# mpkuse/cerebro

Measured on AMD Instinct MI355X. Metric: loop-queries/sec (ticks of 3 descriptors vs 4096-D x 1M DB), higher is better.
Workload: dtype f64

## Files before the change

cerebro_amd/capi.py:

```python
from __future__ import annotations

import ctypes as C
import os
import sys
from pathlib import Path

import numpy as np

_HERE = Path(__file__).resolve().parent
PRODUCT_LIB_PATH = _HERE / "lib" / "libcerebro_hip.so"
HOOKS_LIB_PATH = _HERE / "lib" / "hooks" / "libcerebro_hip.so"


def _lib_path() -> Path:
    override = os.environ.get("CHIP_LIB")
    if override:
        if os.environ.get("CHIP_ALLOW_LIB_OVERRIDE") == "1":
            return Path(override).resolve()
        sys.stderr.write(f"[cerebro_amd] CHIP_LIB={override} IGNORED: set CHIP_ALLOW_LIB_OVERRIDE=1 to load another build of the library\n")
    return PRODUCT_LIB_PATH


LIB_PATH = _lib_path()

CHIP_OK = 0
CHIP_ERR_INVALID_ARG = -1
CHIP_ERR_NO_DEVICE = -2
CHIP_ERR_HIP = -3
CHIP_ERR_OOM = -4
CHIP_ERR_NOT_F32 = -5
CHIP_ERR_NONFINITE = -6
CHIP_ERR_RANGE = -7
CHIP_ERR_UNSUPPORTED = -8
CHIP_ERR_TOO_FEW_POINTS = -9
CHIP_ERR_BUSY = -10
CHIP_ERR_COMM = -11
CHIP_ERR_SHARD_FAILED = -12
CHIP_ERR_GROUP_BROKEN = -13

CHIP_MAX_TOPK = 16
CHIP_MAX_NQ = 4
CHIP_DEFAULT_TOPK = 8
CHIP_RING_ROWS = 4096
CHIP_MAX_INFLIGHT = 64
CHIP_APPEND_ALLOW_ROUNDING = 1
CHIP_CREATE_STORE_F32 = 1
CHIP_CREATE_STORE_F64 = 2
CHIP_MULTI_EXCHANGE_COPY = 4
CHIP_COMM_ID_BYTES = 128
CHIP_EXCHANGE_NONE, CHIP_EXCHANGE_RCCL, CHIP_EXCHANGE_COPY = 0, 1, 2
CHIP_SCAN_FORM_ONE_ROW, CHIP_SCAN_FORM_ROWS = 1, 2
CHIP_SAMPLER_FRESH, CHIP_SAMPLER_THEIA_PERSISTENT = 0, 1
CHIP_RANSAC_LEG_PNP, CHIP_RANSAC_LEG_ICP = 0, 1
CHIP_SCAN_FAMILY_NONE, CHIP_SCAN_FAMILY_ONE_ROW, CHIP_SCAN_FAMILY_WIDE, CHIP_SCAN_FAMILY_ROWS, CHIP_SCAN_FAMILY_MULTI = 0, 1, 2, 3, 4
CHIP_SCAN_CALL_QUERY, CHIP_SCAN_CALL_TICK, CHIP_SCAN_CALL_TICK_SYNC = 0, 1, 2
SCAN_FAMILY_NAMES = {0: "none", 1: "one_row", 2: "wide", 3: "rows", 4: "multi", 5: "prefilter", 6: "halfq"}

CHIP_TICK_SKIPPED, CHIP_TICK_TOO_SHORT, CHIP_TICK_SCANNED = 0, 1, 2
CHIP_MATCH_MAX_KEYPOINTS = 16384
CHIP_MATCH_MAX_BATCH = 16
CHIP_MATCH_MAX_PAIRS = CHIP_MATCH_MAX_BATCH
CHIP_ICP_MAX_BATCH = 16
CHIP_ORB_DESC_BYTES = 32
CHIP_SET_AB, CHIP_SET_BA = 0, 1
CHIP_DISP_S16, CHIP_DISP_F32 = 0, 1
CHIP_STEREO_BM_NUM_DISPARITIES, CHIP_STEREO_BM_BLOCK_SIZE, CHIP_STEREO_BM_PREFILTER_CAP = 64, 21, 31
CHIP_STEREO_BM_TEXTURE_THRESHOLD, CHIP_STEREO_BM_UNIQUENESS_RATIO = 10, 15
CHIP_ORB_MAX_LEVELS, CHIP_ORB_MAX_SIDE = 8, 4096
CHIP_ORB_BINS = 32
CHIP_ORB_N_FEATURES, CHIP_ORB_N_LEVELS, CHIP_ORB_FAST_THRESHOLD, CHIP_ORB_BORDER = 5000, 8, 0, 31
CHIP_RECTIFY_FRACTION_BITS, CHIP_RECTIFY_MAP_MIN, CHIP_RECTIFY_MAP_MAX, CHIP_RECTIFY_NAN_Q = 5, -2.0, 32768.0, -64
CHIP_PROJ_F32, CHIP_PROJ_F64, CHIP_PROJ_MAX_IN_DIM = 1, 2, 32768
CHIP_VLAD_NHWC, CHIP_VLAD_NCHW, CHIP_VLAD_BLOCK, CHIP_VLAD_MAX_POSITIONS = 1, 2, 64, 16384


class ChipError(RuntimeError):
    def __init__(self, status: int, where: str, detail: str = ""):
        self.status = status
        super().__init__(f"{where}: status {status} ({_strerror(status)}){' -- ' + detail if detail else ''}")


class DotParams(C.Structure):
    _fields_ = [("locality", C.c_int32), ("lag", C.c_int32), ("min_new", C.c_int32), ("min_k", C.c_int32),
                ("thresh", C.c_double)]


class TickResult(C.Structure):
    _fields_ = [("status", C.c_int32), ("found", C.c_int32), ("idx_curr", C.c_int64), ("idx_prev", C.c_int64),
                ("score", C.c_double), ("argmax", C.c_int64 * 3), ("maxv", C.c_double * 3)]

    def as_dict(self):
        return dict(status=self.status, found=self.found, idx_curr=self.idx_curr, idx_prev=self.idx_prev,
                    score=self.score, argmax=list(self.argmax), maxv=list(self.maxv))


class TopkEntry(C.Structure):
    _fields_ = [("score", C.c_double), ("idx", C.c_int64)]


class RansacParams(C.Structure):
    _fields_ = [("error_thresh", C.c_double), ("min_inlier_ratio", C.c_double), ("max_iterations", C.c_int32),
                ("min_iterations", C.c_int32), ("use_mle", C.c_int32), ("sample_size", C.c_int32),
                ("failure_probability", C.c_double), ("seed", C.c_uint64), ("n_hypotheses", C.c_int32),
                ("sampler", C.c_int32)]


class RansacSummary(C.Structure):
    _fields_ = [("n_iterations", C.c_int32), ("n_inliers", C.c_int32), ("best_hypothesis", C.c_int32),
                ("n_models", C.c_int32), ("best_cost", C.c_double)]


class StereoBmParams(C.Structure):
    _fields_ = [("num_disparities", C.c_int32), ("block_size", C.c_int32), ("prefilter_cap", C.c_int32),
                ("texture_threshold", C.c_int32), ("uniqueness_ratio", C.c_int32)]


class OrbParams(C.Structure):
    _fields_ = [("n_features", C.c_int32), ("n_levels", C.c_int32), ("fast_threshold", C.c_int32), ("border", C.c_int32)]


class OrbKeypoint(C.Structure):
    _fields_ = [("response", C.c_int64), ("x", C.c_float), ("y", C.c_float), ("m10", C.c_int32), ("m01", C.c_int32),
                ("x_level", C.c_uint16), ("y_level", C.c_uint16), ("level", C.c_uint16), ("zero", C.c_uint16)]


class OrbLevel(C.Structure):
    _fields_ = [("width", C.c_int32), ("height", C.c_int32), ("quota", C.c_int32), ("x0", C.c_int32), ("y0", C.c_int32),
                ("x1", C.c_int32), ("y1", C.c_int32), ("scale", C.c_double)]

    def as_dict(self):
        return {k: getattr(self, k) for k, _ in self._fields_}


ORB_KEYPOINT_DTYPE = np.dtype([("response", "<i8"), ("x", "<f4"), ("y", "<f4"), ("m10", "<i4"), ("m01", "<i4"), ("x_level", "<u2"),
                               ("y_level", "<u2"), ("level", "<u2"), ("zero", "<u2")])


class MatchFrame(C.Structure):
    _fields_ = [("desc", C.c_void_p), ("kp_xy", C.c_void_p), ("n", C.c_int32), ("width", C.c_int32), ("height", C.c_int32),
                ("xyz", C.c_void_p)]


class MatchSummary(C.Structure):
    _fields_ = [("n_matches_all", C.c_int32), ("n_matches_gms", C.c_int32), ("n_3d2d_ab", C.c_int32), ("n_3d2d_ba", C.c_int32),
                ("n_3d3d", C.c_int32), ("n_out_of_image", C.c_int32)]

    def as_dict(self):
        return {k: getattr(self, k) for k, _ in self._fields_}


CHIP_GMS_WITH_SCALE, CHIP_GMS_WITH_ROTATION = 1, 2


class GmsChoice(C.Structure):
    _fields_ = [("scale", C.c_int32), ("rotation", C.c_int32), ("n_inliers", C.c_int32), ("counts", (C.c_int32 * 8) * 5)]

    def as_dict(self):
        return dict(scale=self.scale, rotation=self.rotation, n_inliers=self.n_inliers,
                    counts=np.array([list(row) for row in self.counts], dtype=np.int32))


class MatchSetsOut(C.Structure):
    _fields_ = [(k, C.c_void_p) for k in ("uv", "uv_d", "X_ab", "uvn_ab", "X_ba", "uvn_ba", "A_3d3d", "B_3d3d",
                                          "match_query_idx", "match_train_idx")]


class ScanLaunch(C.Structure):
    _fields_ = [(n, C.c_int32) for n in ("family", "elem", "nq", "K", "U", "NT", "FULL", "NG", "R", "NTL", "ticks", "q64", "claimed", "fused",
                                         "grid", "block", "wg_per_cu", "lds_bytes")] + [("n_rows", C.c_int64), ("launches", C.c_int64)]

    def as_dict(self):
        d = {k: int(getattr(self, k)) for k, _ in self._fields_}
        d["family"] = SCAN_FAMILY_NAMES[d["family"]]
        return d


class PassInfo(C.Structure):
    _fields_ = [(n, C.c_int32) for n in ("family", "ticks", "grid", "wpb", "K", "e")] + [("k", C.c_int64 * 5), ("E", C.c_double)]


class RansacShape(C.Structure):
    _fields_ = [(n, C.c_int32) for n in ("P", "H", "N", "words", "S", "sampler")]


class Info(C.Structure):
    _fields_ = [("abi_version", C.c_int32), ("D", C.c_int32), ("device", C.c_int32), ("shard_rank", C.c_int32),
                ("shard_count", C.c_int32), ("n_cus", C.c_int32), ("rows_global", C.c_int64),
                ("rows_local", C.c_int64), ("capacity_local", C.c_int64), ("lossy_rows", C.c_int64),
                ("arch", C.c_char * 32), ("storage_bytes", C.c_int32), ("n_devices", C.c_int32), ("exchange", C.c_int32),
                ("comm_ranks", C.c_int32), ("comm_init_abandoned", C.c_int32), ("scan_forms", C.c_int32), ("test_hooks", C.c_int32),
                ("row_norm_max", C.c_double)]


_P = C.c_void_p
_SIGS = {
    "chip_strerror": (C.c_char_p, [C.c_int]),
    "chip_abi_version": (C.c_int, []),
    "chip_build_scan_forms": (C.c_int, []),
    "chip_build_test_hooks": (C.c_int, []),
    "chip_last_hip_error": (C.c_int, [_P, C.POINTER(C.c_char_p)]),
    "chip_last_comm_error": (C.c_int, [_P, C.POINTER(C.c_char_p)]),
    "chip_create": (C.c_int, [C.POINTER(_P), C.c_int32, C.c_int64, C.c_int32, C.c_int32, C.c_int32]),
    "chip_create_ex": (C.c_int, [C.POINTER(_P), C.c_int32, C.c_int64, C.c_int32, C.c_int32, C.c_int32, C.c_uint32]),
    "chip_create_multi": (C.c_int, [C.POINTER(_P), C.c_int32, C.c_int64, _P, C.c_int32, C.c_uint32]),
    "chip_comm_unique_id": (C.c_int, [_P]),
    "chip_comm_init_rank": (C.c_int, [_P, _P, C.c_int32, C.c_int32]),
    "chip_destroy": (None, [_P]),
    "chip_set_stream": (C.c_int, [_P, _P]),
    "chip_reset_stream": (C.c_int, [_P]),
    "chip_synchronize": (C.c_int, [_P]),
    "chip_db_append_f64": (C.c_int, [_P, _P, C.c_int64, C.c_uint32, C.POINTER(C.c_int64)]),
    "chip_db_append_f32": (C.c_int, [_P, _P, C.c_int64, C.POINTER(C.c_int64)]),
    "chip_db_size": (C.c_int64, [_P]),
    "chip_db_read_rows_f32": (C.c_int, [_P, _P, C.c_int64, _P]),
    "chip_db_read_rows_f64": (C.c_int, [_P, _P, C.c_int64, _P]),
    "chip_db_append_synthetic": (C.c_int, [_P, C.c_int64, C.c_uint64, _P, _P, _P, C.c_int64]),
    "chip_db_append_synthetic_unit": (C.c_int, [_P, C.c_int64, C.c_uint64, _P, _P, _P, C.c_int64]),
    "chip_query_rows": (C.c_int, [_P, C.c_int64, _P, C.c_int32, C.c_int32, _P, _P]),
    "chip_query_vectors_f32": (C.c_int, [_P, C.c_int64, _P, C.c_int32, C.c_int32, _P, _P]),
    "chip_query_vectors_f64": (C.c_int, [_P, C.c_int64, _P, C.c_int32, C.c_int32, _P, _P]),
    "chip_query_scores": (C.c_int, [_P, C.c_int64, C.c_int64, _P]),
    "chip_query_batch_f32": (C.c_int, [_P, C.c_int64, _P, C.c_int32, C.c_int32, _P, _P]),
    "chip_query_batch_cast_f32": (C.c_int, [_P, C.c_int64, _P, C.c_int32, C.c_int32, _P, _P]),
    "chip_build_has_query_prefix": (C.c_int, []),
    "chip_query_batch_rows_f32": (C.c_int, [_P, _P, _P, C.c_int32, C.c_int32, _P, _P]),
    "chip_query_batch_rows_cast_f32": (C.c_int, [_P, _P, _P, C.c_int32, C.c_int32, _P, _P]),
    "chip_query_batch_prefix_f32": (C.c_int, [_P, _P, _P, C.c_int32, C.c_int32, _P, _P]),
    "chip_query_batch_prefix_cast_f32": (C.c_int, [_P, _P, _P, C.c_int32, C.c_int32, _P, _P]),
    "chip_query_prefix_plan": (C.c_int, [_P, C.c_int32, C.c_int32, C.c_int32, _P, _P]),
    "chip_debug_query_prefix_last": (C.c_int, [_P, _P]),
    "chip_build_has_bulk_ticks": (C.c_int, []),
    "chip_loop_ticks_bulk": (C.c_int, [_P, _P, C.c_int32, _P, C.c_int64, C.c_int32, _P, _P, _P, _P]),
    "chip_bulk_ticks_plan": (C.c_int, [_P, C.c_int32, _P, C.c_int64, C.c_int64, _P, _P, _P]),
    "chip_debug_bulk_ticks_last": (C.c_int, [_P, _P]),
    "chip_dot_params_default": (None, [C.POINTER(DotParams)]),
    "chip_loop_tick": (C.c_int, [_P, C.c_int64, C.POINTER(DotParams), C.POINTER(TickResult)]),
    "chip_resident_pause": (C.c_int, [_P]),
    "chip_resident_resume": (C.c_int, [_P]),
    "chip_loop_tick_enqueue": (C.c_int, [_P, C.c_int64, C.POINTER(DotParams), C.c_int32]),
    "chip_loop_tick_collect": (C.c_int, [_P, C.c_int32, C.POINTER(TickResult)]),
    "chip_loop_last_l": (C.c_int64, [_P]),
    "chip_loop_reset": (None, [_P]),
    "chip_scan_local": (C.c_int, [_P, C.c_int64, C.POINTER(DotParams), C.c_int32, _P, C.POINTER(C.c_int32)]),
    "chip_merge_decide": (C.c_int, [_P, C.c_int64, C.POINTER(DotParams), _P, C.c_int32, C.c_int32, C.POINTER(TickResult)]),
    "chip_merge_decide_enqueue": (C.c_int, [_P, C.c_int64, C.POINTER(DotParams), _P, C.c_int32, C.c_int32, C.c_int32]),
    "chip_debug_merge_lists": (C.c_int, [_P, C.c_int32, _P, C.c_int32, C.c_int32, C.c_int32, _P, C.c_int64, C.POINTER(DotParams),
                                         C.POINTER(TickResult)]),
    "chip_debug_last_pass": (C.c_int, [_P, C.POINTER(PassInfo), _P, _P, _P]),
    "chip_ransac_params_default": (None, [C.POINTER(RansacParams)]),
    "chip_pnp_ransac": (C.c_int, [_P, _P, _P, C.c_int32, C.POINTER(RansacParams), _P, C.POINTER(C.c_float), _P,
                                  C.POINTER(RansacSummary)]),
    "chip_pnp_ransac_batch": (C.c_int, [_P, C.c_int32, _P, _P, _P, C.POINTER(RansacParams), _P, _P, _P, _P, _P]),
    "chip_icp_params_default": (None, [C.POINTER(RansacParams)]),
    "chip_icp_ransac": (C.c_int, [_P, _P, _P, C.c_int32, C.POINTER(RansacParams), _P, C.POINTER(C.c_float), _P,
                                  C.POINTER(RansacSummary)]),
    "chip_icp_ransac_enqueue": (C.c_int, [_P, _P, _P, C.c_int32, C.POINTER(RansacParams)]),
    "chip_icp_ransac_collect": (C.c_int, [_P, _P, C.POINTER(C.c_float), _P, C.POINTER(RansacSummary)]),
    "chip_build_has_icp_batch": (C.c_int, []),
    "chip_icp_ransac_batch": (C.c_int, [_P, C.c_int32, _P, _P, _P, C.POINTER(RansacParams), _P, _P, _P, _P, _P]),
    "chip_debug_ransac_record": (C.c_int, [_P, C.c_int32, C.c_int32, C.POINTER(RansacShape), _P, _P, _P, _P, _P, _P, _P]),
    "chip_debug_pnp_stage": (C.c_int, [_P, C.c_int32, _P, _P, _P]),
    "chip_debug_pnp_keep_stage": (C.c_int, [_P, C.c_int32]),
    "chip_build_has_match": (C.c_int, []),
    "chip_build_has_tick_coalesce": (C.c_int, []),
    "chip_debug_coalesce_stats": (C.c_int, [_P, C.POINTER(C.c_int64), C.POINTER(C.c_int64)]),
    "chip_debug_coalesce_force": (C.c_int, [_P, C.c_int32]),
    "chip_debug_coalesce_decide": (C.c_int, [C.c_int32, C.c_int32, C.c_int32]),
    "chip_debug_last_scan": (C.c_int, [_P, C.POINTER(ScanLaunch)]),
    "chip_debug_scan_plan": (C.c_int, [C.c_int32, C.c_int32, C.c_int32, C.c_int32, C.c_int64, C.c_int32, C.c_int32, C.POINTER(ScanLaunch)]),
    "chip_debug_multi_plan": (C.c_int, [C.c_int32, C.c_int32, C.c_int32, C.c_int32, C.c_int32, C.POINTER(ScanLaunch)]),
    "chip_debug_prefilter_plan": (C.c_int, [C.c_int32, C.c_int32, C.c_int32, C.c_int32, C.POINTER(ScanLaunch)]),
    "chip_debug_halfq_plan": (C.c_int, [C.c_int32, C.c_int32, C.c_int32, C.c_int32, C.POINTER(ScanLaunch)]),
    "chip_debug_halfq_bound": (C.c_int, [C.c_int32, C.c_double, C.POINTER(C.c_int32), C.POINTER(C.c_double)]),
    "chip_debug_prefilter_stats": (C.c_int, [_P, C.POINTER(C.c_int64), C.POINTER(C.c_int64), C.POINTER(C.c_int64)]),
    "chip_orb_match": (C.c_int, [_P, _P, C.c_int32, _P, C.c_int32, _P, _P]),
    "chip_gms_filter": (C.c_int, [_P, _P, C.c_int32, C.c_int32, C.c_int32, _P, C.c_int32, C.c_int32, C.c_int32, _P, _P, C.c_int32, _P,
                                  C.POINTER(C.c_int32)]),
    "chip_match_pair": (C.c_int, [_P, C.POINTER(MatchFrame), C.POINTER(MatchFrame), _P, C.POINTER(MatchSummary)]),
    "chip_match_read_sets": (C.c_int, [_P, C.POINTER(MatchSetsOut)]),
    "chip_pnp_ransac_matched": (C.c_int, [_P, C.c_int32, C.POINTER(RansacParams), _P, C.POINTER(C.c_float), _P, C.POINTER(RansacSummary)]),
    "chip_icp_ransac_matched": (C.c_int, [_P, C.POINTER(RansacParams), _P, C.POINTER(C.c_float), _P, C.POINTER(RansacSummary)]),
    "chip_build_has_gms_modes": (C.c_int, []),
    "chip_gms_filter_modes": (C.c_int, [_P, _P, C.c_int32, C.c_int32, C.c_int32, _P, C.c_int32, C.c_int32, C.c_int32, _P, _P, C.c_int32,
                                        C.c_uint32, _P, C.POINTER(C.c_int32), C.POINTER(GmsChoice)]),
    "chip_match_batch_modes": (C.c_int, [_P, C.POINTER(MatchFrame), C.POINTER(MatchFrame), C.c_int32, _P, C.c_uint32, C.POINTER(MatchSummary),
                                         C.POINTER(GmsChoice)]),
    "chip_match_batch_stored_modes": (C.c_int, [_P, C.c_int64, _P, C.c_int32, _P, C.c_uint32, C.POINTER(MatchSummary), C.POINTER(GmsChoice)]),
    "chip_build_has_match_batch": (C.c_int, []),
    "chip_match_batch": (C.c_int, [_P, C.POINTER(MatchFrame), C.POINTER(MatchFrame), C.c_int32, _P, C.POINTER(MatchSummary)]),
    "chip_match_select": (C.c_int, [_P, C.c_int32]),
    "chip_match_batch_read_matches": (C.c_int, [_P, C.c_int32, _P, _P]),
    "chip_pnp_ransac_matched_batch": (C.c_int, [_P, C.c_int32, _P, _P, C.POINTER(RansacParams), _P, _P, _P, _P, _P, _P]),
    "chip_icp_ransac_matched_batch_enqueue": (C.c_int, [_P, C.c_int32, _P, C.POINTER(RansacParams), _P, _P]),
    "chip_icp_ransac_matched_batch_collect": (C.c_int, [_P, _P, _P, _P, _P]),
    "chip_icp_ransac_matched_batch": (C.c_int, [_P, C.c_int32, _P, C.POINTER(RansacParams), _P, _P, _P, _P, _P, _P]),
    "chip_build_has_frame_store": (C.c_int, []),
    "chip_frame_store_reserve": (C.c_int, [_P, C.c_int32, C.c_int32]),
    "chip_frame_store_info": (C.c_int, [_P, C.POINTER(C.c_int32), C.POINTER(C.c_int32), C.POINTER(C.c_int32)]),
    "chip_frame_put": (C.c_int, [_P, C.c_int64, C.POINTER(MatchFrame)]),
    "chip_frame_drop": (C.c_int, [_P, C.c_int64]),
    "chip_frame_read": (C.c_int, [_P, C.c_int64, C.POINTER(C.c_int32), C.POINTER(C.c_int32), C.POINTER(C.c_int32), _P, _P, _P]),
    "chip_match_batch_stored": (C.c_int, [_P, C.c_int64, _P, C.c_int32, _P, C.POINTER(MatchSummary)]),
    "chip_build_has_match_pairs": (C.c_int, []),
    "chip_match_pairs_stored": (C.c_int, [_P, _P, _P, C.c_int32, _P, C.c_uint32, C.POINTER(MatchSummary), C.POINTER(GmsChoice)]),
    "chip_build_has_disparity": (C.c_int, []),
    "chip_frame_put_disparity": (C.c_int, [_P, C.c_int64, _P, _P, C.c_int32, C.c_int32, C.c_int32, _P, C.c_int32, _P]),
    "chip_disparity_to_xyz": (C.c_int, [_P, _P, C.c_int32, C.c_int32, C.c_int32, _P, _P]),
    "chip_stereo_bm_params_default": (None, [C.POINTER(StereoBmParams)]),
    "chip_build_has_stereo_bm": (C.c_int, []),
    "chip_stereo_bm": (C.c_int, [_P, _P, _P, C.c_int32, C.c_int32, C.POINTER(StereoBmParams), _P]),
    "chip_frame_put_stereo": (C.c_int, [_P, C.c_int64, _P, _P, C.c_int32, C.c_int32, C.c_int32, _P, _P, C.POINTER(StereoBmParams), _P]),
    "chip_orb_params_default": (None, [C.POINTER(OrbParams)]),
    "chip_build_has_orb_detect": (C.c_int, []),
    "chip_orb_plan": (C.c_int, [C.c_int32, C.c_int32, C.POINTER(OrbParams), C.POINTER(OrbLevel)]),
    "chip_orb_detect": (C.c_int, [_P, _P, C.c_int32, C.c_int32, C.POINTER(OrbParams), _P, C.c_int32, C.POINTER(C.c_int32), C.POINTER(C.c_int32)]),
    "chip_debug_orb_level": (C.c_int, [_P, C.c_int32, _P, _P]),
    "chip_build_has_orb_describe": (C.c_int, []),
    "chip_orb_bin": (C.c_int, [C.c_int32, C.c_int32]),
    "chip_orb_pattern": (C.c_int, [_P, _P]),
    "chip_orb_detect_describe": (C.c_int, [_P, _P, C.c_int32, C.c_int32, C.POINTER(OrbParams), _P, C.c_int32, C.POINTER(C.c_int32), C.POINTER(C.c_int32),
                                           _P]),
    "chip_debug_orb_blur": (C.c_int, [_P, C.c_int32, _P]),
    "chip_frame_put_orb_stereo": (C.c_int, [_P, C.c_int64, C.c_int32, C.c_int32, _P, _P, C.POINTER(OrbParams), C.POINTER(StereoBmParams), _P,
                                            C.POINTER(C.c_int32)]),
    "chip_build_has_rectify": (C.c_int, []),
    "chip_rectify_quantize": (C.c_int, [_P, C.c_int64, _P]),
    "chip_remap": (C.c_int, [_P, _P, C.c_int32, C.c_int32, _P, _P, _P]),
    "chip_rectify_set_maps": (C.c_int, [_P, C.c_int32, C.c_int32, _P, _P, _P, _P, _P, _P, _P, _P]),
    "chip_rectify_pair": (C.c_int, [_P, _P, _P, C.c_int32, C.c_int32, _P, _P]),
    "chip_frame_put_raw_orb_stereo": (C.c_int, [_P, C.c_int64, C.c_int32, C.c_int32, _P, _P, C.POINTER(OrbParams), C.POINTER(StereoBmParams), _P,
                                                C.POINTER(C.c_int32)]),
    "chip_build_has_frame_put_batch": (C.c_int, []),
    "chip_frame_put_plan": (C.c_int, [C.c_int32, C.c_int32, C.POINTER(OrbParams), C.c_int32, C.c_int32, C.POINTER(C.c_int32), C.POINTER(C.c_int32)]),
    "chip_frame_put_orb_stereo_batch": (C.c_int, [_P, _P, C.c_int32, C.c_int32, C.c_int32, _P, _P, C.POINTER(OrbParams), C.POINTER(StereoBmParams), _P,
                                                  _P]),
    "chip_frame_put_raw_orb_stereo_batch": (C.c_int, [_P, _P, C.c_int32, C.c_int32, C.c_int32, _P, _P, C.POINTER(OrbParams),
                                                      C.POINTER(StereoBmParams), _P, _P]),
    "chip_frame_put_records": (C.c_int, [_P, C.c_int64, _P, _P, _P, C.c_int32, C.c_int32, C.c_int32]),
    "chip_debug_frame_put_last": (C.c_int, [_P, C.POINTER(C.c_int32), C.POINTER(C.c_int32), C.POINTER(C.c_int32)]),
    "chip_build_has_project": (C.c_int, []),
    "chip_project_set": (C.c_int, [_P, C.c_int32, _P, C.c_int32, _P]),
    "chip_project_clear": (C.c_int, [_P]),
    "chip_project_info": (C.c_int, [_P, C.POINTER(C.c_int32), C.POINTER(C.c_int32), C.POINTER(C.c_int32)]),
    "chip_project": (C.c_int, [_P, _P, C.c_int64, _P]),
    "chip_db_append_projected_f32": (C.c_int, [_P, _P, C.c_int64, C.c_uint32, C.POINTER(C.c_int64)]),
    "chip_build_has_vlad": (C.c_int, []),
    "chip_vlad_set": (C.c_int, [_P, C.c_int32, C.c_int32, C.c_int32, _P, _P, _P]),
    "chip_vlad_clear": (C.c_int, [_P]),
    "chip_vlad_info": (C.c_int, [_P, C.POINTER(C.c_int32), C.POINTER(C.c_int32), C.POINTER(C.c_int32)]),
    "chip_vlad": (C.c_int, [_P, _P, C.c_int32, C.c_int32, _P]),
    "chip_db_append_vlad_f32": (C.c_int, [_P, _P, C.c_int32, C.c_int32, C.c_uint32, C.POINTER(C.c_int64)]),
    "chip_debug_vlad_stage": (C.c_int, [_P, _P, _P, _P]),
    "chip_project_plan": (C.c_int, [C.c_int32, C.c_int32, C.c_int64, _P]),
    "chip_debug_project_last": (C.c_int, [_P, C.POINTER(C.c_int64), C.POINTER(C.c_int64), C.POINTER(C.c_int32)]),
    "chip_vlad_batch": (C.c_int, [_P, _P, C.c_int32, C.c_int32, C.c_int32, _P]),
    "chip_db_append_vlad_batch_f32": (C.c_int, [_P, _P, C.c_int32, C.c_int32, C.c_int32, C.c_uint32, C.POINTER(C.c_int64)]),
    "chip_get_info": (C.c_int, [_P, C.POINTER(Info)]),
    "chip_profile_enable": (C.c_int, [_P, C.c_int32]),
    "chip_profile_reset": (C.c_int, [_P]),
    "chip_profile_scan": (C.c_int, [_P, C.POINTER(C.c_double), C.POINTER(C.c_int64), C.POINTER(C.c_double), C.POINTER(C.c_double)]),
}

_lib = None


def load_library(path: os.PathLike | None = None) -> C.CDLL:
    global _lib
    if _lib is not None and path is None:
        return _lib
    p = Path(path) if path else LIB_PATH
    if p.exists() and "torch" not in sys.modules:
        try:
            import torch
        except Exception:
            pass
    if not p.exists():
        raise FileNotFoundError(
            f"{p} not found: the HIP extension is not built. Run `make lib` (or __graft_entry__.build()). "
            "cerebro_amd has no CPU fallback.")
    lib = C.CDLL(str(p))
    for name, (res, args) in _SIGS.items():
        fn = getattr(lib, name)
        fn.restype = res
        fn.argtypes = args
    if path is None:
        _lib = lib
    return lib


class use_hooks_library:

    def __enter__(self):
        global _lib
        self.saved = _lib
        lib = load_library(HOOKS_LIB_PATH)
        if lib.chip_build_test_hooks() != 1:
            raise RuntimeError(f"{HOOKS_LIB_PATH} is not a -DCHIP_TEST_HOOKS build")
        _lib = lib
        return lib

    def __exit__(self, *exc):
        global _lib
        _lib = self.saved
        return False


def declared_symbols():
    return sorted(_SIGS)


def _strerror(status: int) -> str:
    try:
        return load_library().chip_strerror(status).decode()
    except Exception:
        return "?"


def _ptr(a: np.ndarray):
    return a.ctypes.data_as(C.c_void_p)

# ... 39 lines not shown
        raise ChipError(rc, "chip_orb_pattern")
    return pattern, steered


def rectify_quantize(map) -> np.ndarray:
    m = np.ascontiguousarray(map, dtype=np.float32)
    q = np.zeros(m.shape, dtype=np.int32)
    rc = load_library().chip_rectify_quantize(_ptr(m), m.size, _ptr(q))
    if rc != CHIP_OK:
        raise ChipError(rc, "chip_rectify_quantize")
    return q


def frame_put_plan(width: int, height: int, F: int, params=None, raw: bool = False) -> dict:
    _, o = _orb_params(params)
    g, n = C.c_int32(), C.c_int32()
    rc = load_library().chip_frame_put_plan(width, height, o, int(raw), F, C.byref(g), C.byref(n))
    if rc != CHIP_OK:
        raise ChipError(rc, "chip_frame_put_plan")
    return dict(group=g.value, n_groups=n.value)


def orb_plan(width: int, height: int, params=None) -> list:
    params, p = _orb_params(params)
    lv = (OrbLevel * CHIP_ORB_MAX_LEVELS)()
    rc = load_library().chip_orb_plan(width, height, p, lv)
    if rc != CHIP_OK:
        raise ChipError(rc, "chip_orb_plan")
    n = CHIP_ORB_N_LEVELS if params is None else params.n_levels
    return [lv[l].as_dict() for l in range(n)]


class ProjectPlan(C.Structure):
    _fields_ = [("width", C.c_int32), ("slab", C.c_int32), ("lds_bytes", C.c_int32), ("single_lds_bytes", C.c_int32), ("block", C.c_int32),
                ("reserved", C.c_int32), ("passes", C.c_int64), ("shared_passes", C.c_int64), ("single_launches", C.c_int64)]


def project_plan(in_dim: int, matrix_type: int, n: int) -> dict:
    out = ProjectPlan()
    rc = load_library().chip_project_plan(in_dim, matrix_type, n, C.byref(out))
    if rc != CHIP_OK:
        raise ChipError(rc, "chip_project_plan")
    return {name: getattr(out, name) for name, _ in ProjectPlan._fields_ if name != "reserved"}


CHIP_QUERY_PREFIX_GROUP = 4096


class QueryPrefixPlan(C.Structure):
    _fields_ = [("group_size", C.c_int32), ("groups", C.c_int32), ("tile_full", C.c_int32), ("tile_last", C.c_int32),
                ("qtiles", C.c_int64), ("units", C.c_int64), ("units_rect", C.c_int64)]


class QueryPrefixLast(C.Structure):
    _fields_ = [("groups", C.c_int32), ("launches", C.c_int32), ("waits", C.c_int32), ("reserved", C.c_int32),
                ("units_claimed", C.c_int64), ("units_planned", C.c_int64)]


def query_prefix_plan(k, elem: int = 4, topk: int = 5) -> dict:
    k = np.ascontiguousarray(k, dtype=np.int64).reshape(-1)
    order = np.empty(k.shape[0], dtype=np.int32)
    out = QueryPrefixPlan()
    rc = load_library().chip_query_prefix_plan(_ptr(k), k.shape[0], elem, topk, _ptr(order), C.byref(out))
    if rc != CHIP_OK:
        raise ChipError(rc, "chip_query_prefix_plan")
    d = {name: getattr(out, name) for name, _ in QueryPrefixPlan._fields_}
    d["order"] = order
    return d


CHIP_BULK_TICKS_GROUP, CHIP_BULK_TICKS_MAX_TOPK = 1365, 8


class BulkTicksPlan(C.Structure):
    _fields_ = [("group_ticks", C.c_int32), ("groups", C.c_int32), ("tile_full", C.c_int32), ("tile_last", C.c_int32),
                ("ticks_scanned", C.c_int64), ("ticks_skipped", C.c_int64), ("ticks_too_short", C.c_int64),
                ("units", C.c_int64), ("units_rect", C.c_int64), ("last_l", C.c_int64)]


class BulkTicksLast(C.Structure):
    _fields_ = [("groups", C.c_int32), ("launches", C.c_int32), ("waits", C.c_int32), ("list_len", C.c_int32),
                ("certified", C.c_int64), ("uncertified", C.c_int64), ("rescored_rows", C.c_int64),
                ("exact_reruns", C.c_int64), ("E", C.c_double)]


def bulk_ticks_plan(ls, n_rows: int, params: DotParams | None = None, last_l: int = 0) -> dict:
    ls = np.ascontiguousarray(ls, dtype=np.int64).reshape(-1)
    T = ls.shape[0]
    status = np.empty(T, dtype=np.int32)
    k = np.empty(T, dtype=np.int64)
    out = BulkTicksPlan()
    rc = load_library().chip_bulk_ticks_plan(_ptr(ls) if T else None, T, C.byref(params) if params is not None else None, last_l, n_rows,
                                             _ptr(status), _ptr(k), C.byref(out))
    if rc != CHIP_OK:
        raise ChipError(rc, "chip_bulk_ticks_plan")
    d = {name: getattr(out, name) for name, _ in BulkTicksPlan._fields_}
    d["status"] = status
    d["k"] = k
    return d


def default_ransac_params() -> RansacParams:
    p = RansacParams()
    load_library().chip_ransac_params_default(C.byref(p))
    return p


def default_icp_params() -> RansacParams:
    p = RansacParams()
    load_library().chip_icp_params_default(C.byref(p))
    return p


def scan_plan(D: int, elem: int, nq: int, K: int, n_rows: int, call: int = CHIP_SCAN_CALL_QUERY, n_cus: int = 256, check: bool = True):
    out = ScanLaunch()
    rc = load_library().chip_debug_scan_plan(D, elem, nq, K, n_rows, call, n_cus, C.byref(out))
    if not check:
        return rc, out.as_dict()
    if rc != CHIP_OK:
        raise ChipError(rc, "chip_debug_scan_plan")
    return out.as_dict()


def multi_plan(D: int, elem: int, n_ticks: int, K: int = CHIP_DEFAULT_TOPK, n_cus: int = 256, check: bool = True):
    out = ScanLaunch()
    rc = load_library().chip_debug_multi_plan(D, elem, n_ticks, K, n_cus, C.byref(out))
    if not check:
        return rc, out.as_dict()
    if rc != CHIP_OK:
        raise ChipError(rc, "chip_debug_multi_plan")
    return out.as_dict()


def prefilter_plan(D: int, elem: int = 4, K: int = CHIP_DEFAULT_TOPK, n_cus: int = 256, check: bool = True):
    out = ScanLaunch()
    rc = load_library().chip_debug_prefilter_plan(D, elem, K, n_cus, C.byref(out))
    if not check:
        return rc, out.as_dict()
    if rc != CHIP_OK:
        raise ChipError(rc, "chip_debug_prefilter_plan")
    return out.as_dict()


def halfq_plan(D: int, elem: int = 4, K: int = CHIP_DEFAULT_TOPK, n_cus: int = 256, check: bool = True):
    out = ScanLaunch()
    rc = load_library().chip_debug_halfq_plan(D, elem, K, n_cus, C.byref(out))
    if not check:
        return rc, out.as_dict()
    if rc != CHIP_OK:
        raise ChipError(rc, "chip_debug_halfq_plan")
    return out.as_dict()


def halfq_bound(D: int, row_norm_max: float) -> tuple[int, float]:
    e, E = C.c_int32(), C.c_double()
    rc = load_library().chip_debug_halfq_bound(D, row_norm_max, C.byref(e), C.byref(E))
    if rc != CHIP_OK:
        raise ChipError(rc, "chip_debug_halfq_bound")
    return e.value, E.value


def comm_unique_id() -> bytes:
    buf = C.create_string_buffer(CHIP_COMM_ID_BYTES)
    st = load_library().chip_comm_unique_id(buf)
    if st != CHIP_OK:
        raise ChipError(st, "chip_comm_unique_id")
    return buf.raw


class Chip:

    def __init__(self, D: int, capacity_hint: int = 0, device: int = 0, shard_rank: int = 0, shard_count: int = 1,
                 storage: str | None = None, devices=None, copy_exchange: bool = False):
        self.lib = load_library()
        self.D = int(D)
        self.shard_rank, self.shard_count = shard_rank, shard_count
        flags = {None: 0, "f32": CHIP_CREATE_STORE_F32, "f64": CHIP_CREATE_STORE_F64}[storage]
        h = C.c_void_p()
        if devices is not None:
            dev = np.ascontiguousarray(devices, dtype=np.int32)
            st = self.lib.chip_create_multi(C.byref(h), D, capacity_hint, _ptr(dev), dev.size,
                                            flags | (CHIP_MULTI_EXCHANGE_COPY if copy_exchange else 0))
            where = "chip_create_multi"
        elif flags:
            st = self.lib.chip_create_ex(C.byref(h), D, capacity_hint, device, shard_rank, shard_count, flags)
            where = "chip_create_ex"
        else:
            st = self.lib.chip_create(C.byref(h), D, capacity_hint, device, shard_rank, shard_count)
            where = "chip_create"
        if st != CHIP_OK:
            raise ChipError(st, where)
        self.h = h

    def comm_init_rank(self, unique_id: bytes, n_ranks: int, rank: int):
        assert len(unique_id) == CHIP_COMM_ID_BYTES
        self._chk(self.lib.chip_comm_init_rank(self.h, C.c_char_p(unique_id), n_ranks, rank), "chip_comm_init_rank")

    def close(self):
        if getattr(self, "h", None):
            self.lib.chip_destroy(self.h)
            self.h = None

    def __del__(self):
        try:
            self.close()
        except Exception:
            pass

    def __enter__(self):
        return self

    def __exit__(self, *a):
        self.close()

    def _chk(self, st: int, where: str):
        if st != CHIP_OK:
            txt = C.c_char_p()
            if st == CHIP_ERR_COMM:
                r = self.lib.chip_last_comm_error(self.h, C.byref(txt))
                raise ChipError(st, where, f"ncclResult {r}: {txt.value.decode() if txt.value else ''}")
            hip = self.lib.chip_last_hip_error(self.h, C.byref(txt)) if st in (CHIP_ERR_HIP, CHIP_ERR_OOM) else 0
            raise ChipError(st, where, f"hipError {hip}: {txt.value.decode() if txt.value else ''}" if hip else "")

    def last_comm_error(self) -> str:
        txt = C.c_char_p()
        r = self.lib.chip_last_comm_error(self.h, C.byref(txt))
        return f"{r}: {txt.value.decode() if txt.value else ''}"

    def set_stream(self, stream_ptr: int | None):
        if stream_ptr is None:
            self._chk(self.lib.chip_reset_stream(self.h), "chip_reset_stream")
        else:
            self._chk(self.lib.chip_set_stream(self.h, C.c_void_p(stream_ptr)), "chip_set_stream")

    def synchronize(self):
        self._chk(self.lib.chip_synchronize(self.h), "chip_synchronize")

    def append_f64(self, desc: np.ndarray, allow_rounding: bool = False) -> int:
        desc = np.ascontiguousarray(desc, dtype=np.float64).reshape(-1, self.D)
        first = C.c_int64()
        self._chk(self.lib.chip_db_append_f64(self.h, _ptr(desc), desc.shape[0],
                                              CHIP_APPEND_ALLOW_ROUNDING if allow_rounding else 0, C.byref(first)),
                  "chip_db_append_f64")
        return first.value

    def append_f32(self, desc: np.ndarray) -> int:
        desc = np.ascontiguousarray(desc, dtype=np.float32).reshape(-1, self.D)
        first = C.c_int64()
        self._chk(self.lib.chip_db_append_f32(self.h, _ptr(desc), desc.shape[0], C.byref(first)), "chip_db_append_f32")
        return first.value

    def project_set(self, Mt: np.ndarray, bias=None):
        Mt = np.asarray(Mt)
        if Mt.dtype not in (np.float32, np.float64) or Mt.ndim != 2 or Mt.shape[0] != self.D:
            raise ValueError("project_set: Mt must be a (D, in_dim) float32 or float64 array")
        Mt = np.ascontiguousarray(Mt)
        b = None if bias is None else np.ascontiguousarray(bias, dtype=np.float64).reshape(self.D)
        self._chk(self.lib.chip_project_set(self.h, Mt.shape[1], _ptr(Mt), CHIP_PROJ_F32 if Mt.dtype == np.float32 else CHIP_PROJ_F64,
                                            None if b is None else _ptr(b)), "chip_project_set")

    def project_clear(self):
        self._chk(self.lib.chip_project_clear(self.h), "chip_project_clear")

    def project_info(self) -> dict:
        v = [C.c_int32(), C.c_int32(), C.c_int32()]
        self._chk(self.lib.chip_project_info(self.h, *(C.byref(x) for x in v)), "chip_project_info")
        return dict(in_dim=v[0].value, matrix_type=v[1].value, has_bias=bool(v[2].value))

    def _raw_descriptors(self, x, n):
        if isinstance(x, (int, np.integer)):
            if n is None:
                raise ValueError("a device address needs n")
            return C.c_void_p(int(x)), int(n), None
        in_dim = self.project_info()["in_dim"]
        a = np.ascontiguousarray(x, dtype=np.float32)
        a = a.reshape(-1, in_dim) if in_dim else a.reshape(1, -1)
        return _ptr(a), a.shape[0], a

    def project(self, x, n: int | None = None) -> np.ndarray:
        p, n, keep = self._raw_descriptors(x, n)
        z = np.empty((n, self.D), dtype=np.float64)
        self._chk(self.lib.chip_project(self.h, p, n, _ptr(z)), "chip_project")
        return z

    def append_projected(self, x, flags: int = 0, n: int | None = None) -> int:
        p, n, keep = self._raw_descriptors(x, n)
        first = C.c_int64()
        self._chk(self.lib.chip_db_append_projected_f32(self.h, p, n, flags, C.byref(first)), "chip_db_append_projected_f32")
        return first.value

    def debug_project_last(self) -> dict:
        passes, descs, width = (C.c_int64 * 2)(), (C.c_int64 * 2)(), C.c_int32()
        self._chk(self.lib.chip_debug_project_last(self.h, passes, descs, C.byref(width)), "chip_debug_project_last")
        return dict(shared_passes=passes[0], single_launches=passes[1], shared_descriptors=descs[0], single_descriptors=descs[1],
                    width=width.value)

    def vlad_set(self, Wt, bias, centres):
        Wt = np.ascontiguousarray(Wt, dtype=np.float32)
        centres = np.ascontiguousarray(centres, dtype=np.float32)
        bias = np.ascontiguousarray(bias, dtype=np.float32).reshape(-1)
        if Wt.ndim != 2 or centres.ndim != 2 or centres.shape[1] != Wt.shape[1] or bias.size != Wt.shape[0] or centres.shape[0] > Wt.shape[0]:
            raise ValueError("vlad_set: Wt (K+G, C), bias (K+G), centres (K, C)")
        K, G = centres.shape[0], Wt.shape[0] - centres.shape[0]
        self._chk(self.lib.chip_vlad_set(self.h, Wt.shape[1], K, G, _ptr(Wt), _ptr(bias), _ptr(centres)), "chip_vlad_set")

    def vlad_clear(self):
# ... 86 lines not shown
        return out

    def read_rows_f64(self, rows) -> np.ndarray:
        rows = np.ascontiguousarray(rows, dtype=np.int64)
        out = np.empty((rows.size, self.D), dtype=np.float64)
        self._chk(self.lib.chip_db_read_rows_f64(self.h, _ptr(rows), rows.size, _ptr(out)), "chip_db_read_rows_f64")
        return out

    def query_scores(self, k: int, row: int) -> np.ndarray:
        u = np.full(max(k, 1), np.nan, dtype=np.float64)
        self._chk(self.lib.chip_query_scores(self.h, k, row, _ptr(u)), "chip_query_scores")
        return u[:k]

    def query_vectors_f64(self, k: int, q: np.ndarray, topk: int = CHIP_DEFAULT_TOPK):
        q = np.ascontiguousarray(q, dtype=np.float64).reshape(-1, self.D)
        nq = q.shape[0]
        sc = np.empty((nq, topk), dtype=np.float64)
        ix = np.empty((nq, topk), dtype=np.int64)
        self._chk(self.lib.chip_query_vectors_f64(self.h, k, _ptr(q), nq, topk, _ptr(sc), _ptr(ix)), "chip_query_vectors_f64")
        return sc, ix

    def query_rows(self, k: int, rows, topk: int = CHIP_DEFAULT_TOPK):
        rows = np.ascontiguousarray(rows, dtype=np.int64)
        nq = rows.size
        sc = np.empty((nq, topk), dtype=np.float64)
        ix = np.empty((nq, topk), dtype=np.int64)
        self._chk(self.lib.chip_query_rows(self.h, k, _ptr(rows), nq, topk, _ptr(sc), _ptr(ix)), "chip_query_rows")
        return sc, ix

    def query_vectors(self, k: int, q: np.ndarray, topk: int = CHIP_DEFAULT_TOPK):
        q = np.ascontiguousarray(q, dtype=np.float32).reshape(-1, self.D)
        nq = q.shape[0]
        sc = np.empty((nq, topk), dtype=np.float64)
        ix = np.empty((nq, topk), dtype=np.int64)
        self._chk(self.lib.chip_query_vectors_f32(self.h, k, _ptr(q), nq, topk, _ptr(sc), _ptr(ix)),
                  "chip_query_vectors_f32")
        return sc, ix

    def query_batch(self, k: int, q: np.ndarray, topk: int = CHIP_DEFAULT_TOPK, cast_rows: bool = False):
        q = np.ascontiguousarray(q, dtype=np.float32).reshape(-1, self.D)
        Q = q.shape[0]
        sc = np.empty((Q, topk), dtype=np.float32)
        ix = np.empty((Q, topk), dtype=np.int64)
        name = "chip_query_batch_cast_f32" if cast_rows else "chip_query_batch_f32"
        self._chk(getattr(self.lib, name)(self.h, k, _ptr(q), Q, topk, _ptr(sc), _ptr(ix)), name)
        return sc, ix

    def query_batch_rows(self, rows, k, topk: int = CHIP_DEFAULT_TOPK, cast_rows: bool = False):
        rows = np.ascontiguousarray(rows, dtype=np.int64).reshape(-1)
        k = np.ascontiguousarray(k, dtype=np.int64).reshape(-1)
        if rows.shape != k.shape:
            raise ValueError("rows and k must have the same length")
        Q = rows.shape[0]
        sc = np.empty((Q, topk), dtype=np.float32)
        ix = np.empty((Q, topk), dtype=np.int64)
        name = "chip_query_batch_rows_cast_f32" if cast_rows else "chip_query_batch_rows_f32"
        self._chk(getattr(self.lib, name)(self.h, _ptr(rows), _ptr(k), Q, topk, _ptr(sc), _ptr(ix)), name)
        return sc, ix

    def query_batch_prefix(self, k, q: np.ndarray, topk: int = CHIP_DEFAULT_TOPK, cast_rows: bool = False):
        q = np.ascontiguousarray(q, dtype=np.float32).reshape(-1, self.D)
        k = np.ascontiguousarray(k, dtype=np.int64).reshape(-1)
        Q = q.shape[0]
        if k.shape[0] != Q:
            raise ValueError("k must have one entry per query")
        sc = np.empty((Q, topk), dtype=np.float32)
        ix = np.empty((Q, topk), dtype=np.int64)
        name = "chip_query_batch_prefix_cast_f32" if cast_rows else "chip_query_batch_prefix_f32"
        self._chk(getattr(self.lib, name)(self.h, _ptr(k), _ptr(q), Q, topk, _ptr(sc), _ptr(ix)), name)
        return sc, ix

    def self_join(self, first: int, count: int, lag: int, topk: int = CHIP_DEFAULT_TOPK, cast_rows: bool = False):
        rows = first + np.arange(count, dtype=np.int64)
        return self.query_batch_rows(rows, np.maximum(0, rows - lag), topk, cast_rows)

    def debug_query_prefix_last(self) -> dict:
        out = QueryPrefixLast()
        self._chk(self.lib.chip_debug_query_prefix_last(self.h, C.byref(out)), "chip_debug_query_prefix_last")
        return {name: getattr(out, name) for name, _ in QueryPrefixLast._fields_ if name != "reserved"}

    def loop_tick(self, l: int, params: DotParams | None = None) -> TickResult:
        p = params or default_dot_params()
        r = TickResult()
        self._chk(self.lib.chip_loop_tick(self.h, l, C.byref(p), C.byref(r)), "chip_loop_tick")
        return r

    def loop_ticks_bulk(self, ls, params: DotParams | None = None, last_l: int = 0, topk: int = 1):
        ls = np.ascontiguousarray(ls, dtype=np.int64).reshape(-1)
        T = ls.shape[0]
        recs = (TickResult * max(T, 1))()
        sc = np.empty((T, 3, topk), dtype=np.float64)
        ix = np.empty((T, 3, topk), dtype=np.int64)
        last = C.c_int64(last_l)
        self._chk(self.lib.chip_loop_ticks_bulk(self.h, _ptr(ls) if T else None, T, C.byref(params) if params is not None else None, last_l, topk,
                                                C.byref(recs), _ptr(sc), _ptr(ix), C.byref(last)), "chip_loop_ticks_bulk")
        return [recs[t] for t in range(T)], sc, ix, last.value

    def debug_bulk_ticks_last(self) -> dict:
        out = BulkTicksLast()
        self._chk(self.lib.chip_debug_bulk_ticks_last(self.h, C.byref(out)), "chip_debug_bulk_ticks_last")
        return {name: getattr(out, name) for name, _ in BulkTicksLast._fields_}

    def resident_pause(self):
        self._chk(self.lib.chip_resident_pause(self.h), "chip_resident_pause")

    def resident_resume(self):
        self._chk(self.lib.chip_resident_resume(self.h), "chip_resident_resume")

    def loop_tick_enqueue(self, l: int, slot: int, params: DotParams | None = None):
        p = params or default_dot_params()
        self._chk(self.lib.chip_loop_tick_enqueue(self.h, l, C.byref(p), slot), "chip_loop_tick_enqueue")

    def loop_tick_collect(self, slot: int) -> TickResult:
        r = TickResult()
        self._chk(self.lib.chip_loop_tick_collect(self.h, slot, C.byref(r)), "chip_loop_tick_collect")
        return r

    def loop_reset(self):
        self.lib.chip_loop_reset(self.h)

    def last_l(self) -> int:
        return int(self.lib.chip_loop_last_l(self.h))

    def coalesce_stats(self) -> tuple[int, int]:
        passes, ticks = C.c_int64(), C.c_int64()
        self._chk(self.lib.chip_debug_coalesce_stats(self.h, C.byref(passes), C.byref(ticks)), "chip_debug_coalesce_stats")
        return passes.value, ticks.value

    def prefilter_stats(self) -> tuple[int, int, int]:
        passes, ticks, unc = C.c_int64(), C.c_int64(), C.c_int64()
        self._chk(self.lib.chip_debug_prefilter_stats(self.h, C.byref(passes), C.byref(ticks), C.byref(unc)), "chip_debug_prefilter_stats")
        return passes.value, ticks.value, unc.value

    def coalesce_force(self, on: bool):
        self._chk(self.lib.chip_debug_coalesce_force(self.h, 1 if on else 0), "chip_debug_coalesce_force")

    def last_scan(self) -> dict:
        out = ScanLaunch()
        self._chk(self.lib.chip_debug_last_scan(self.h, C.byref(out)), "chip_debug_last_scan")
        return out.as_dict()

    def last_pass(self) -> dict:
        info = PassInfo()
        self._chk(self.lib.chip_debug_last_pass(self.h, C.byref(info), None, None, None), "chip_debug_last_pass")
        T, grid, K = info.ticks, info.grid, info.K
        cand = np.empty((T, grid, 3, K, 2), dtype=np.float64)
        exact = np.empty((T, 3, K, 2), dtype=np.float64)
        cert = np.zeros((T, 3), dtype=np.uint32)
        self._chk(self.lib.chip_debug_last_pass(self.h, C.byref(info), _ptr(cand), _ptr(exact), _ptr(cert)), "chip_debug_last_pass")
        return dict(family=SCAN_FAMILY_NAMES[info.family], ticks=T, grid=grid, wpb=int(info.wpb), K=K, k=[int(x) for x in info.k[:T]],
                    E=float(info.E), e=int(info.e), cand_s=cand[..., 0].copy(), cand_i=cand[..., 1].copy().view(np.int64),
                    exact_s=exact[..., 0].copy(), exact_i=exact[..., 1].copy().view(np.int64), cert=cert)

    def scan_local(self, l: int, dev_out_ptr: int, topk: int = CHIP_DEFAULT_TOPK, params: DotParams | None = None) -> int:
        p = params or default_dot_params()
        status = C.c_int32()
        self._chk(self.lib.chip_scan_local(self.h, l, C.byref(p), topk, C.c_void_p(dev_out_ptr), C.byref(status)),
                  "chip_scan_local")
        return status.value

    def merge_decide(self, l: int, dev_gathered_ptr: int, n_lists: int, topk: int = CHIP_DEFAULT_TOPK,
                     params: DotParams | None = None) -> TickResult:
        p = params or default_dot_params()
        r = TickResult()
        self._chk(self.lib.chip_merge_decide(self.h, l, C.byref(p), C.c_void_p(dev_gathered_ptr), n_lists, topk,
                                             C.byref(r)), "chip_merge_decide")
        return r

    def merge_decide_enqueue(self, l: int, dev_gathered_ptr: int, n_lists: int, slot: int, topk: int = CHIP_DEFAULT_TOPK,
                             params: DotParams | None = None):
        p = params or default_dot_params()
        self._chk(self.lib.chip_merge_decide_enqueue(self.h, l, C.byref(p), C.c_void_p(dev_gathered_ptr), n_lists, topk, slot),
                  "chip_merge_decide_enqueue")

    def debug_merge_lists(self, form: int, scores: np.ndarray, idx: np.ndarray, l: int = 0, params: DotParams | None = None,
                          record: bool = False):
        scores = np.ascontiguousarray(scores, dtype=np.float64)
        idx = np.ascontiguousarray(idx, dtype=np.int64)
        assert scores.ndim == 3 and scores.shape == idx.shape
        n_lists, nq, K = scores.shape
        lists = np.empty((n_lists, nq, K, 2), dtype=np.float64)
        lists[..., 0] = scores
        lists[..., 1] = idx.view(np.float64)
        out = np.empty((nq, K, 2), dtype=np.float64)
        r = TickResult() if record else None
        p = params or default_dot_params()
        self._chk(self.lib.chip_debug_merge_lists(self.h, form, _ptr(lists), n_lists, nq, K, _ptr(out), l, C.byref(p),
                                                  C.byref(r) if record else None), "chip_debug_merge_lists")
        return out[..., 0].copy(), out[..., 1].copy().view(np.int64), r

    def pnp_ransac(self, X: np.ndarray, uv: np.ndarray, params: RansacParams | None = None):
        X = np.ascontiguousarray(X, dtype=np.float64).reshape(-1, 3)
        uv = np.ascontiguousarray(uv, dtype=np.float64).reshape(-1, 2)
        N = X.shape[0]
        assert uv.shape[0] == N
        p = params or default_ransac_params()
        T = np.empty(16, dtype=np.float64)
        conf = C.c_float()
        mask = np.zeros(max(N, 1), dtype=np.uint8)
        summ = RansacSummary()
        st = self.lib.chip_pnp_ransac(self.h, _ptr(X), _ptr(uv), N, C.byref(p), _ptr(T), C.byref(conf), _ptr(mask),
                                      C.byref(summ))
        if st == CHIP_ERR_TOO_FEW_POINTS:
            return dict(status=st, confidence=-1.0, T=None, mask=None, summary=None)
        self._chk(st, "chip_pnp_ransac")
        return dict(status=st, confidence=float(conf.value), T=T.reshape(4, 4).T.copy(), mask=mask[:N].copy(),
                    summary=dict(n_iterations=summ.n_iterations, n_inliers=summ.n_inliers,
                                 best_hypothesis=summ.best_hypothesis, n_models=summ.n_models,
                                 best_cost=summ.best_cost))

    def pnp_ransac_batch(self, problems, params: RansacParams | None = None, seeds=None):
        P = len(problems)
        Xs = [np.ascontiguousarray(X, dtype=np.float64).reshape(-1, 3) for X, _ in problems]
        uvs = [np.ascontiguousarray(uv, dtype=np.float64).reshape(-1, 2) for _, uv in problems]
        Ns = np.array([x.shape[0] for x in Xs], dtype=np.int32)
        p = params or default_ransac_params()
        T = np.empty((P, 16), dtype=np.float64)
        conf = np.zeros(P, dtype=np.float32)
        masks = [np.zeros(max(int(n), 1), dtype=np.uint8) for n in Ns]
        summ = (RansacSummary * max(P, 1))()
        Xp = (C.c_void_p * max(P, 1))(*[x.ctypes.data for x in Xs])
        uvp = (C.c_void_p * max(P, 1))(*[u.ctypes.data for u in uvs])
        mp = (C.c_void_p * max(P, 1))(*[m.ctypes.data for m in masks])
        sd = None if seeds is None else np.asarray(seeds, dtype=np.uint64)
        st = self.lib.chip_pnp_ransac_batch(self.h, P, Xp, uvp, _ptr(Ns), C.byref(p), None if sd is None else _ptr(sd),
                                            _ptr(T), _ptr(conf), mp, summ)
        self._chk(st, "chip_pnp_ransac_batch")
        return [dict(status=st, confidence=float(conf[i]), T=T[i].reshape(4, 4).T.copy(), mask=masks[i][:Ns[i]].copy(),
                     summary=dict(n_iterations=summ[i].n_iterations, n_inliers=summ[i].n_inliers,
                                  best_hypothesis=summ[i].best_hypothesis, n_models=summ[i].n_models,
                                  best_cost=summ[i].best_cost)) for i in range(P)]

    def icp_ransac_enqueue(self, A: np.ndarray, B: np.ndarray, params: RansacParams | None = None):
        A = np.ascontiguousarray(A, dtype=np.float64).reshape(-1, 3)
        B = np.ascontiguousarray(B, dtype=np.float64).reshape(-1, 3)
        p = params or default_icp_params()
        self._chk(self.lib.chip_icp_ransac_enqueue(self.h, _ptr(A), _ptr(B), A.shape[0], C.byref(p)), "chip_icp_ransac_enqueue")
        return A.shape[0]

    def icp_ransac_collect(self, N: int):
        T = np.empty(16, dtype=np.float64)
        conf = C.c_float()
        mask = np.zeros(max(N, 1), dtype=np.uint8)
        summ = RansacSummary()
        self._chk(self.lib.chip_icp_ransac_collect(self.h, _ptr(T), C.byref(conf), _ptr(mask), C.byref(summ)), "chip_icp_ransac_collect")
        return dict(status=0, confidence=float(conf.value), T=T.reshape(4, 4).T.copy(), mask=mask[:N].copy(),
                    summary=dict(n_iterations=summ.n_iterations, n_inliers=summ.n_inliers, best_hypothesis=summ.best_hypothesis,
                                 n_models=summ.n_models, best_cost=summ.best_cost))

    def icp_ransac(self, A: np.ndarray, B: np.ndarray, params: RansacParams | None = None):
        A = np.ascontiguousarray(A, dtype=np.float64).reshape(-1, 3)
        B = np.ascontiguousarray(B, dtype=np.float64).reshape(-1, 3)
        N = A.shape[0]
        assert B.shape[0] == N
        p = params or default_icp_params()
        T = np.empty(16, dtype=np.float64)
        conf = C.c_float()
        mask = np.zeros(max(N, 1), dtype=np.uint8)
        summ = RansacSummary()
        st = self.lib.chip_icp_ransac(self.h, _ptr(A), _ptr(B), N, C.byref(p), _ptr(T), C.byref(conf), _ptr(mask), C.byref(summ))
        if st == CHIP_ERR_TOO_FEW_POINTS:
            return dict(status=st, confidence=-1.0, T=None, mask=None, summary=None)
        self._chk(st, "chip_icp_ransac")
        return dict(status=st, confidence=float(conf.value), T=T.reshape(4, 4).T.copy(), mask=mask[:N].copy(),
                    summary=dict(n_iterations=summ.n_iterations, n_inliers=summ.n_inliers,
                                 best_hypothesis=summ.best_hypothesis, n_models=summ.n_models, best_cost=summ.best_cost))

    def icp_ransac_batch(self, problems, params: RansacParams | None = None, seeds=None):
        P = len(problems)
        As = [np.ascontiguousarray(A, dtype=np.float64).reshape(-1, 3) for A, _ in problems]
        Bs = [np.ascontiguousarray(B, dtype=np.float64).reshape(-1, 3) for _, B in problems]
        Ns = np.array([a.shape[0] for a in As], dtype=np.int32)
        p = params or default_icp_params()
        T = np.empty((max(P, 1), 16), dtype=np.float64)
        conf = np.zeros(max(P, 1), dtype=np.float32)
        masks = [np.zeros(max(int(n), 1), dtype=np.uint8) for n in Ns]
        summ = (RansacSummary * max(P, 1))()
        Ap = (C.c_void_p * max(P, 1))(*[a.ctypes.data for a in As])
        Bp = (C.c_void_p * max(P, 1))(*[b.ctypes.data for b in Bs])
        mp = (C.c_void_p * max(P, 1))(*[m.ctypes.data for m in masks])
        sd = None if seeds is None else np.ascontiguousarray(seeds, dtype=np.uint64)
        st = self.lib.chip_icp_ransac_batch(self.h, P, Ap, Bp, _ptr(Ns), C.byref(p), None if sd is None else _ptr(sd), _ptr(T), _ptr(conf), mp, summ)
        self._chk(st, "chip_icp_ransac_batch")
        return [dict(status=st, confidence=float(conf[i]), T=T[i].reshape(4, 4).T.copy(), mask=masks[i][:Ns[i]].copy(),
                     summary=dict(n_iterations=summ[i].n_iterations, n_inliers=summ[i].n_inliers, best_hypothesis=summ[i].best_hypothesis,
                                  n_models=summ[i].n_models, best_cost=summ[i].best_cost)) for i in range(P)]

    def ransac_record(self, leg: int = CHIP_RANSAC_LEG_PNP, problem: int = 0) -> dict:
        sh = self.ransac_record_shape(leg, problem)
        H, W, S = sh["H"], sh["words"], sh["S"]
        r = dict(valid=np.empty(H, np.int32), cost=np.empty(H, np.float64), nin=np.empty(H, np.int32), T=np.empty((H, 16), np.float64),
                 mask=np.empty((H, W), np.uint64))
        if leg == CHIP_RANSAC_LEG_PNP:
            r.update(nsol=np.empty(H, np.int32), sample=np.empty((H, S), np.int32))
        ptrs = [_ptr(r[k]) if k in r else None for k in ("valid", "cost", "nin", "T", "mask", "nsol", "sample")]
        self._chk(self.lib.chip_debug_ransac_record(self.h, leg, problem, None, *ptrs), "chip_debug_ransac_record")
        r.update(sh)
        return r

    def pnp_stage(self, problem: int = 0) -> dict:
        H = self.ransac_record_shape(CHIP_RANSAC_LEG_PNP, problem)["H"]
        r = dict(ok=np.empty(H, np.int32), Tg=np.empty((H, 27), np.float64), Sg=np.empty((H, 27, 27), np.float64))
        self._chk(self.lib.chip_debug_pnp_stage(self.h, problem, _ptr(r["ok"]), _ptr(r["Tg"]), _ptr(r["Sg"])), "chip_debug_pnp_stage")
        return r

    def ransac_record_shape(self, leg: int = CHIP_RANSAC_LEG_PNP, problem: int = 0) -> dict:
# ... 434 lines not shown
```

cerebro_amd/csrc/chip_api.hip:

```cpp
#include "chip_internal.h"
#include <cmath>
#include <cstdlib>
#include <cstring>
#include <memory>
#include <new>

using namespace chip;

extern "C" {

const char *chip_strerror(int status)
{
    switch (status) {
        case CHIP_OK: return "ok";
        case CHIP_ERR_INVALID_ARG: return "invalid argument";
        case CHIP_ERR_NO_DEVICE: return "no usable HIP device";
        case CHIP_ERR_HIP: return "HIP runtime error (see chip_last_hip_error)";
        case CHIP_ERR_OOM: return "out of device memory";
        case CHIP_ERR_NOT_F32: return "descriptor value not exactly representable as float32";
        case CHIP_ERR_NONFINITE: return "NaN/Inf in descriptor";
        case CHIP_ERR_RANGE: return "index / length out of range";
        case CHIP_ERR_UNSUPPORTED: return "unsupported configuration";
        case CHIP_ERR_TOO_FEW_POINTS: return "fewer than 20 correspondences";
        case CHIP_ERR_BUSY: return "async slot busy or empty";
        case CHIP_ERR_COMM: return "RCCL error (see chip_last_comm_error)";
        case CHIP_ERR_SHARD_FAILED: return "a shard could not take part in this tick / query (all ranks see this status); retry";
        case CHIP_ERR_GROUP_BROKEN: return "multi-GPU ctx is broken by an earlier partial failure; destroy it";
    }
    return "unknown status";
}

int chip_abi_version(void) { return CHIP_ABI_VERSION; }
int chip_build_scan_forms(void) { return scan_forms_built(); }
int chip_build_has_tick_coalesce(void) { return 1; }
int chip_build_test_hooks(void)
{
#ifdef CHIP_TEST_HOOKS
    return 1;
#else
    return 0;
#endif
}

int chip_last_hip_error(const chip_ctx *ctx, const char **text)
{
    if (!ctx) return (int)hipErrorInvalidValue;
    const Ctx *c = ctx->group ? group_root(const_cast<chip_ctx *>(ctx)) : ctx;
    if (text) *text = hipGetErrorString(c->last_hip);
    return (int)c->last_hip;
}

void chip_dot_params_default(chip_dot_params *p)
{
    if (!p) return;
    p->locality = 12;
    p->thresh = (double)(float)0.85;
    p->lag = 50;
    p->min_new = 3;
    p->min_k = 5;
}

void chip_ransac_params_default(chip_ransac_params *p)
{
    if (!p) return;
    p->error_thresh = 0.03;
    p->min_inlier_ratio = 0.7;
    p->max_iterations = 50;
    p->min_iterations = 5;
    p->use_mle = 1;
    p->sample_size = 15;
    p->failure_probability = 0.01;
    p->seed = 0x5EEDCE7EB80ULL;
    p->n_hypotheses = 0;
    p->sampler = CHIP_SAMPLER_FRESH;
}

}

namespace chip {

int env_int(const char *name, int dflt)
{
    const char *v = std::getenv(name);
    return v && *v ? std::atoi(v) : dflt;
}

static int ensure_capacity(Ctx *c, int64_t local_rows)
{
    const int64_t need = (local_rows + c->seg_rows - 1) >> c->seg_shift;
    if (need > kMaxSegs) return CHIP_ERR_OOM;
    bool grew = false;
    ResidentPause paused(c, (int64_t)c->segs.size() < need);
    while ((int64_t)c->segs.size() < need) {
        void *p = nullptr;
        CHIP_HIP(c, hipMalloc(&p, (size_t)c->seg_rows * c->D * c->elem));
        {
            std::lock_guard<std::mutex> lk(c->mu);
            c->segs.push_back(p);
        }
        grew = true;
    }
    if (grew) {
        CHIP_HIP(c, hipMemcpyAsync(c->seg_table_dev, c->segs.data(), c->segs.size() * sizeof(void *), hipMemcpyHostToDevice, c->s_append));
        CHIP_HIP(c, hipStreamSynchronize(c->s_append));
    }
    return CHIP_OK;
}

static int configure_storage(Ctx *c, int elem)
{
    ResidentPause paused(c);
    for (void *p : c->segs) (void)hipFree(p);
    {
        std::lock_guard<std::mutex> lk(c->mu);
        c->segs.clear();
    }
    c->ring_dev.release();
    c->qvec_dev.release();
    c->elem = elem;
    int64_t rows = kSegBytesTarget / ((int64_t)c->D * 4);
    int shift = 0;
    while ((2ll << shift) <= rows) shift++;
    if (shift < 6) shift = 6;
    c->seg_shift = shift;
    c->seg_rows = 1ll << shift;
    CHIP_HIP(c, hipMemset(c->seg_table_dev, 0, kMaxSegs * sizeof(void *)));
    if (c->nranks > 1) {
        const int rc = c->ring_dev.reserve(c, (size_t)CHIP_RING_ROWS * c->D * elem);
        if (rc != CHIP_OK) return rc;
        CHIP_HIP(c, hipMemset(c->ring_dev, 0, (size_t)CHIP_RING_ROWS * c->D * elem));
    }
    return c->qvec_dev.reserve(c, (size_t)CHIP_MAX_NQ * c->D * elem);
}

void ctx_destroy(chip_ctx *c)
{
    if (!c) return;
    if (c->group) { group_destroy(c); delete c; return; }
    (void)hipSetDevice(c->device);
    { std::lock_guard<std::mutex> qlk(c->query_mu); (void)coalesce_flush(c); }
    resident_stop(c);
    (void)hipDeviceSynchronize();
    resident_destroy(c);
    exchange_destroy(c);
    pnp_destroy(c);
    icp_destroy(c);
    batch_destroy(c);
    match_destroy(c);
    frame_store_destroy(c);
    orb_destroy(c);
    for (void *p : c->segs) (void)hipFree(p);
    for (int i = 0; i < Ctx::kRing; i++) {
        if (c->ev_scan[i]) (void)hipEventDestroy(c->ev_scan[i]);
        if (c->ev_merged[i]) (void)hipEventDestroy(c->ev_merged[i]);
    }
    if (c->s_scan) (void)hipStreamDestroy(c->s_scan);
    if (c->s_scan2) (void)hipStreamDestroy(c->s_scan2);
    for (hipStream_t x : c->s_scan_x)
        if (x) (void)hipStreamDestroy(x);
    for (Slot &s : c->slots)
        if (s.done) (void)hipEventDestroy(s.done);
    for (hipEvent_t e : c->prof_ev) (void)hipEventDestroy(e);
    if (c->own_query_stream && c->s_query) (void)hipStreamDestroy(c->s_query);
    if (c->s_append) (void)hipStreamDestroy(c->s_append);
    if (c->s_pnp) (void)hipStreamDestroy(c->s_pnp);
    delete c;
}

void scan_read_knobs(Ctx *c)
{
    c->scan_block = env_int("CHIP_SCAN_BLOCK", 0);
    if (c->scan_block != 256 && c->scan_block != 512 && c->scan_block != 768 && c->scan_block != 1024) c->scan_block = 0;
    c->scan_blocks_per_cu = env_int("CHIP_SCAN_BPC", 2);
    if (c->scan_blocks_per_cu < 1) c->scan_blocks_per_cu = 1;
    c->scan_variant = env_int("CHIP_SCAN_VARIANT", 0);
    c->scan_rows = env_int("CHIP_SCAN_ROWS", 0);
    c->scan_claim = env_int("CHIP_SCAN_CLAIM", -1);
    c->tick_same_stream = env_int("CHIP_TICK_SAME_STREAM", 1) != 0;
    c->scan_short_bpc = env_int("CHIP_SCAN_SHORT_BPC", 1);
    c->scan_plain_bytes = (double)env_int("CHIP_SCAN_PLAIN_MIB", 768) * 1024 * 1024;
    c->scan_half_bytes = (double)env_int("CHIP_SCAN_HALF_MIB", 192) * 1024 * 1024;
    c->scan_sync_plain_bytes = (double)env_int("CHIP_SCAN_SYNC_PLAIN_MIB", 4096) * 1024 * 1024;
    c->scan_overlap_bytes = (double)env_int("CHIP_SCAN_OVERLAP_GIB", 8) * 1024 * 1024 * 1024;
    c->scan_reserve = env_int("CHIP_SCAN_RESERVE", c->nranks > 1 ? 4 : 0);
    c->max_grid = 512;
    c->scan_streams = env_int("CHIP_SCAN_STREAMS", c->nranks > 1 ? 2 : 4);
    c->tick_fused = env_int("CHIP_TICK_FUSED", 1) != 0;
}

static int create_impl(chip_ctx *c, int64_t capacity_hint, int elem)
{
    hipDeviceProp_t prop;
    CHIP_HIP(c, hipGetDeviceProperties(&prop, c->device));
    c->n_cus = prop.multiProcessorCount;
    std::strncpy(c->arch, prop.gcnArchName, sizeof(c->arch) - 1);
    if (std::strncmp(c->arch, "gfx950", 6) != 0 && !std::getenv("CHIP_ALLOW_ANY_ARCH")) return CHIP_ERR_NO_DEVICE;

    c->segs.reserve(kMaxSegs);

    CHIP_HIP(c, hipStreamCreateWithFlags(&c->s_query, hipStreamNonBlocking));
    CHIP_HIP(c, hipStreamCreateWithFlags(&c->s_append, hipStreamNonBlocking));
    CHIP_HIP(c, hipStreamCreateWithFlags(&c->s_pnp, hipStreamNonBlocking));
    int rc = c->seg_table_dev.alloc(c, kMaxSegs);
    if (rc == CHIP_OK) rc = configure_storage(c, elem);
    if (rc != CHIP_OK) return rc;
    c->stage_bytes = 64ull << 20;
    if (c->stage_bytes < (size_t)c->D * 8 * 64) c->stage_bytes = (size_t)c->D * 8 * 64;
    rc = c->stage_dev.alloc(c, c->stage_bytes);
    if (rc == CHIP_OK) rc = c->flags_dev.alloc(c, 1);
    if (rc == CHIP_OK) rc = c->flags_host.alloc(c, 1);
    if (rc == CHIP_OK) rc = c->norm2_dev.alloc(c, 1);
    if (rc == CHIP_OK) rc = c->norm2_host.alloc(c, 1);
    if (rc != CHIP_OK) return rc;
    CHIP_HIP(c, hipMemset(c->norm2_dev, 0, sizeof(unsigned long long)));
    *c->norm2_host.host() = 0;

    scan_read_knobs(c);
    CHIP_HIP(c, hipStreamCreateWithFlags(&c->s_scan, hipStreamNonBlocking));
    {
        const int ns = c->scan_streams;
        if (ns >= 2) CHIP_HIP(c, hipStreamCreateWithFlags(&c->s_scan2, hipStreamNonBlocking));
        for (int i = 0; i < 2; i++)
            if (ns >= 3 + i) CHIP_HIP(c, hipStreamCreateWithFlags(&c->s_scan_x[i], hipStreamNonBlocking));
    }
    for (int i = 0; i < Ctx::kRing; i++) {
        constexpr size_t kListsPerGroup = 3 * kPassMaxTicks > CHIP_MAX_NQ ? 3 * kPassMaxTicks : CHIP_MAX_NQ;
        static_assert(kPassMaxTicks >= kMultiMaxTicks && kPassMaxTicks >= kPrefilterTicks, "the list buffers are sized for the deepest pass");
        rc = c->partial_dev[i].alloc(c, ((size_t)c->max_grid + 1) * kListsPerGroup * CHIP_MAX_TOPK);
        if (rc != CHIP_OK) return rc;
        CHIP_HIP(c, hipEventCreateWithFlags(&c->ev_scan[i], hipEventDisableTiming));
        CHIP_HIP(c, hipEventCreateWithFlags(&c->ev_merged[i], hipEventDisableTiming));
    }
    rc = c->tickets_dev.alloc(c, Ctx::kRing);
    if (rc != CHIP_OK) return rc;
    CHIP_HIP(c, hipMemset(c->tickets_dev, 0, Ctx::kRing * sizeof(int32_t)));
    c->coalesce_max = env_int("CHIP_TICK_COALESCE", kPassMaxTicks);
    if (c->coalesce_max < 2) c->coalesce_max = 0;
    if (c->coalesce_max > kPassMaxTicks) c->coalesce_max = kPassMaxTicks;
    c->tick_poll = env_int("CHIP_TICK_POLL", 1) != 0;
    resident_read_knobs(c);
    rc = c->seq_all.alloc(c, CHIP_MAX_INFLIGHT);
    if (rc != CHIP_OK) return rc;
    std::memset(c->seq_all.host(), 0, sizeof(unsigned long long) * CHIP_MAX_INFLIGHT);
    rc = c->cert_all.alloc(c, CHIP_MAX_INFLIGHT * 4);
    if (rc != CHIP_OK) return rc;
    std::memset(c->cert_all.host(), 0, sizeof(uint32_t) * CHIP_MAX_INFLIGHT * 4);
    rc = c->topk.alloc(c, (size_t)CHIP_MAX_NQ * CHIP_MAX_TOPK);
    if (rc != CHIP_OK) return rc;
    for (Slot &s : c->slots) {
        CHIP_HIP(c, hipEventCreateWithFlags(&s.done, hipEventDisableTiming));
        rc = s.rec.alloc(c, 1);
        if (rc != CHIP_OK) return rc;
        s.seq_host = c->seq_all.host() + (&s - c->slots);
        s.seq_dev = c->seq_all.dev() + (&s - c->slots);
        s.cert_host = c->cert_all.host() + 4 * (&s - c->slots);
        s.cert_dev = c->cert_all.dev() + 4 * (&s - c->slots);
    }
    if (env_int("CHIP_SCAN_STAMPS", 0)) {
        rc = c->stamps_dev.alloc(c, (size_t)c->max_grid * 16 * 4 + 64);
        if (rc != CHIP_OK) return rc;
        CHIP_HIP(c, hipMemset(c->stamps_dev, 0, ((size_t)c->max_grid * 16 * 4 + 64) * sizeof(unsigned long long)));
    }
    rc = pnp_create(c);
    if (rc != CHIP_OK) return rc;
    c->cap_hint = capacity_hint;
    if (capacity_hint > 0) {
        std::lock_guard<std::mutex> lk(c->append_mu);
        rc = ensure_capacity(c, local_count(c, capacity_hint));
        if (rc != CHIP_OK) return rc;
    }
    return CHIP_OK;
}

int ctx_create(chip_ctx **out, int32_t D, int64_t capacity_hint, int32_t device, int32_t shard_rank, int32_t shard_count, uint32_t flags)
{
    if (!out) return CHIP_ERR_INVALID_ARG;
    *out = nullptr;
    if (D <= 0 || shard_count < 1 || shard_rank < 0 || shard_rank >= shard_count || capacity_hint < 0) return CHIP_ERR_INVALID_ARG;
    const uint32_t store = flags & kCreateStoreMask;
    if (store == kCreateStoreMask) return CHIP_ERR_INVALID_ARG;
    if (D % 4 != 0 || (size_t)D * 4 * CHIP_MAX_NQ > 160 * 1024) return CHIP_ERR_UNSUPPORTED;
    if (store == CHIP_CREATE_STORE_F64 && (size_t)D * 8 * 2 > 160 * 1024) return CHIP_ERR_UNSUPPORTED;
    int ndev = 0;
    if (hipGetDeviceCount(&ndev) != hipSuccess || ndev <= 0) return CHIP_ERR_NO_DEVICE;
    if (device < 0 || device >= ndev) return CHIP_ERR_NO_DEVICE;
    if (hipSetDevice(device) != hipSuccess) return CHIP_ERR_NO_DEVICE;
    chip_ctx *c = new (std::nothrow) chip_ctx();
    if (!c) return CHIP_ERR_OOM;
    c->D = D;
    c->device = device;
    c->rank = shard_rank;
    c->nranks = shard_count;
    c->store_auto = store == 0;
    int rc = create_impl(c, capacity_hint, store == CHIP_CREATE_STORE_F64 ? 8 : 4);
    if (rc != CHIP_OK) { ctx_destroy(c); return rc; }
    *out = c;
    return CHIP_OK;
}

bool scan_policy(const Ctx *c, int64_t n_local, int nq, bool sync_tick, ScanArgs *a, int *grid)
{
    const double bytes = (double)n_local * c->D * c->elem;
    const bool short_scan = bytes <= c->scan_overlap_bytes;
    a->q64 = scan_q64(c, nq, !short_scan) ? 1 : 0;
    *grid = scan_grid_for(c, n_local, nq, a->q64 != 0);
    a->rows_form = scan_rows_form(c, n_local, nq, *grid, a->q64 != 0, sync_tick);
    a->plain_loads = bytes <= c->scan_plain_bytes ? 1 : 0;
    a->dyn_claim = (a->rows_form == 1 && (c->scan_claim == 1 || (c->scan_claim < 0 && *grid > c->n_cus))) ? 1 : 0;
    return short_scan;
}

bool scan_tick_fused(const Ctx *c, bool same_stream, const ScanArgs &a, bool decision_only, int nq)
{
    return same_stream && a.rows_form > 0 && c->tick_fused && decision_only && nq == 3;
}

bool tick_merge_on_scan_stream(const Ctx *c, bool tick, bool short_scan, bool second_tick_stream, bool caller_accepts)
{
    return tick && short_scan && !c->prof_on && c->nranks == 1 && !c->xchg && !c->parent && c->own_query_stream && second_tick_stream &&
           caller_accepts && c->tick_same_stream;
}

MergeArgs merge_args(const chip_topk_entry *in, int32_t n_lists, int32_t K, chip_topk_entry *out, chip_tick_result *result, int64_t l, const chip_dot_params *p)
{
    MergeArgs m;
    m.in = in;
    m.n_lists = n_lists;
    m.K = K;
    m.out = out;
    m.result = result;
    m.l = l;
    m.locality = p ? p->locality : 0;
    m.thresh = p ? p->thresh : 0.0;
    return m;
}

int prof_begin(Ctx *c, hipStream_t s, double bytes, hipEvent_t *stop)
{
    while (c->prof_used + 2 > c->prof_ev.size()) {
        hipEvent_t e;
        CHIP_HIP(c, hipEventCreate(&e));
        c->prof_ev.push_back(e);
    }
    hipEvent_t start = c->prof_ev[c->prof_used];
    *stop = c->prof_ev[c->prof_used + 1];
    c->prof_used += 2;
    c->prof_bytes_last = bytes;
    CHIP_HIP(c, hipEventRecord(start, s));
    return CHIP_OK;
}

int enqueue_scan_merge(Ctx *c, const ScanRequest &rq, ScanReceipt *rcpt)
{
    const int b = (int)(c->n_enqueued++ % Ctx::kRing);
    ScanArgs a;
    int grid = 0;
    const int nq = rq.nq;
    const bool short_scan = scan_policy(c, local_count(c, rq.k), nq, rq.tick && rq.sync_tick, &a, &grid);
    hipStream_t s_scan = (rq.tick && short_scan && !c->prof_on && c->s_scan2 && (c->n_enqueued & 1)) ? c->s_scan2 : c->s_scan;
    const bool same_stream = tick_merge_on_scan_stream(c, rq.tick, short_scan, c->s_scan2 != nullptr, rq.merge_on_scan_stream);
    if (same_stream) {
        hipStream_t ring[4] = {c->s_scan, c->s_scan2, c->s_scan_x[0], c->s_scan_x[1]};
        int ns = 2;
        while (ns < 4 && ring[ns]) ns++;
        s_scan = ring[c->n_same_stream++ % (uint64_t)ns];
    }
    scan_args_db(c, &a);
    a.n_rows = local_count(c, rq.k);
    a.K = rq.K;
    for (int i = 0; i < CHIP_MAX_NQ; i++) a.q[i] = i < nq ? rq.q[i] : nullptr;
    a.idx_mul = c->nranks;
    a.idx_add = c->nranks == 1 ? 0 : c->rank;
    a.partial = c->partial_dev[b];
    a.stamps = c->stamps_dev;
    const bool fused = scan_tick_fused(c, same_stream, a, rq.res != nullptr && rq.out == nullptr && rq.p != nullptr, nq);
    if (fused) {
        a.K = 1;
        a.fused_result = rq.res;
        a.fused_ticket = c->tickets_dev + b;
        a.tick_l = rq.l;
        a.locality = rq.p->locality;
        a.thresh = rq.p->thresh;
        a.fused_seq = rq.seq_dev;
        a.fused_seq_val = rq.seq_val;
    }

    if (hipEventQuery(c->ev_merged[b]) != hipSuccess) CHIP_HIP(c, hipStreamWaitEvent(s_scan, c->ev_merged[b], 0));
    hipEvent_t e1 = nullptr;
    int rc = c->prof_on ? prof_begin(c, s_scan, (double)a.n_rows * c->D * c->elem, &e1) : CHIP_OK;
    if (rc == CHIP_OK) rc = launch_scan(c, s_scan, a, nq, grid);
    if (rc != CHIP_OK) return rc;
    if (e1) CHIP_HIP(c, hipEventRecord(e1, s_scan));
    hipStream_t s_merge = same_stream ? s_scan : c->s_query;
    if (rcpt) { rcpt->merge_stream = s_merge; rcpt->fused = fused; rcpt->done_ev = same_stream ? c->ev_merged[b] : nullptr; }
    if (!same_stream) {
        CHIP_HIP(c, hipEventRecord(c->ev_scan[b], s_scan));
        if (rq.tick && !short_scan) { c->pass_ev = c->ev_scan[b]; c->pass_shared = false; c->pass_no++; }
        if (c->ring_dev) c->last_scan_ev[s_scan == c->s_scan2 ? 1 : 0] = c->ev_scan[b];
        CHIP_HIP(c, hipStreamWaitEvent(c->s_query, c->ev_scan[b], 0));
    }

    if (fused) {
        CHIP_HIP(c, hipEventRecord(c->ev_merged[b], s_scan));
        return CHIP_OK;
    }
    rc = launch_merge(c, s_merge, merge_args(c->partial_dev[b], grid, rq.K, rq.out, rq.res, rq.l, rq.p), nq);
    if (rc != CHIP_OK) return rc;
    CHIP_HIP(c, hipEventRecord(c->ev_merged[b], s_merge));
    return CHIP_OK;
}

int query_row_ptrs(Ctx *c, const int64_t *rows, int nq, int64_t n_global, const void **q)
{
    int64_t total;
    {
        std::lock_guard<std::mutex> lk(c->mu);
        total = c->rows_global;
    }
    for (int i = 0; i < nq; i++) {
        const int64_t g = rows[i];
        if (g < 0 || g >= n_global || g >= total) return CHIP_ERR_RANGE;
        if (c->nranks == 1) {
            q[i] = row_ptr_host(c, g);
        } else {
            const int64_t horizon = c->rows_pending > total ? c->rows_pending : total;
            if (g < horizon - CHIP_RING_ROWS) return CHIP_ERR_RANGE;
            q[i] = ring_ptr(c, g);
        }
    }
    return CHIP_OK;
}

int upload_query_vectors(Ctx *c, const void *queries, int src_elem, int nq, const void **q)
{
    const size_t n = (size_t)nq * c->D;
    if (src_elem == c->elem) {
        CHIP_HIP(c, hipMemcpyAsync(c->qvec_dev, queries, n * c->elem, hipMemcpyHostToDevice, c->s_scan));
    } else {
        c->qconv.resize(n * c->elem);
        if (c->elem == 8) {
            double *d = reinterpret_cast<double *>(c->qconv.data());
            const float *s = static_cast<const float *>(queries);
            for (size_t i = 0; i < n; i++) d[i] = (double)s[i];
        } else {
            float *d = reinterpret_cast<float *>(c->qconv.data());
            const double *s = static_cast<const double *>(queries);
            for (size_t i = 0; i < n; i++) {
                d[i] = (float)s[i];
                if (!((double)d[i] == s[i])) return std::isfinite(s[i]) ? CHIP_ERR_NOT_F32 : CHIP_ERR_NONFINITE;
            }
        }
        CHIP_HIP(c, hipMemcpyAsync(c->qvec_dev, c->qconv.data(), n * c->elem, hipMemcpyHostToDevice, c->s_scan));
        CHIP_HIP(c, hipStreamSynchronize(c->s_scan));
    }
    for (int i = 0; i < nq; i++) q[i] = c->qvec_dev + (size_t)i * c->D * c->elem;
    return CHIP_OK;
}

int tick_prepare(int64_t n, int64_t last_l, int64_t l, const chip_dot_params *p, int32_t *status, int64_t *k_out)
{
    if (l < 0 || l > n) return CHIP_ERR_RANGE;
    if (l - last_l < p->min_new) { *status = CHIP_TICK_SKIPPED; return CHIP_OK; }
    if (l < 3) return CHIP_ERR_RANGE;
    const int64_t k = l - p->lag;
    *k_out = k;
    *status = (k > p->min_k) ? CHIP_TICK_SCANNED : CHIP_TICK_TOO_SHORT;
    return CHIP_OK;
}

void fill_immediate(chip_tick_result *r, int32_t status)
{
    std::memset(r, 0, sizeof *r);
    r->status = status;
    r->idx_curr = r->idx_prev = -1;
    for (int q = 0; q < 3; q++) { r->argmax[q] = -1; r->maxv[q] = -INFINITY; }
}

int64_t published_rows(const Ctx *c)
{
    std::lock_guard<std::mutex> lk(c->mu);
    return c->rows_global;
}

int tick_begin(Slot &s, int64_t n_rows, int64_t *last_l, int64_t l, const chip_dot_params *p, int32_t *status, int64_t *k)
{
    if (s.state != SlotState::Free) return CHIP_ERR_BUSY;
    const int rc = tick_prepare(n_rows, *last_l, l, p, status, k);
    if (rc != CHIP_OK) return rc;
    s.prev_last_l = *last_l;
    s.prefilter = false;
    s.tick_l = l;
    s.last_l_ptr = last_l;
    if (*status != CHIP_TICK_SCANNED) {
        if (*status == CHIP_TICK_TOO_SHORT) *last_l = l;
        fill_immediate(s.rec.host(), *status);
        s.state = SlotState::Immediate;
    }
    return CHIP_OK;
}

static int tick_submit(Ctx *c, int64_t k, int64_t l, const chip_dot_params *p, const void *const *q, bool sync_tick, Slot &s)
{
    ScanRequest rq;
    rq.k = k; rq.q = q; rq.nq = 3; rq.K = CHIP_DEFAULT_TOPK;
    rq.res = s.rec.dev(); rq.l = l; rq.p = p;
    rq.tick = true; rq.sync_tick = sync_tick; rq.merge_on_scan_stream = true;
    if (c->tick_poll) { s.seq_want = ++c->tick_seq; rq.seq_dev = s.seq_dev; rq.seq_val = s.seq_want; }
    ScanReceipt done;
    const int rc = enqueue_scan_merge(c, rq, &done);
    if (rc != CHIP_OK) return rc;
    if (done.done_ev) s.wait_ev = done.done_ev;
    else { CHIP_HIP(c, hipEventRecord(s.done, done.merge_stream)); s.wait_ev = s.done; }
    s.pass_no = c->pass_no;
    s.state = c->tick_poll && done.fused ? SlotState::Poll : SlotState::Event;
    return CHIP_OK;
}

int coalesce_decide(int n_parked, int t_max, bool scan_running)
{
    if (t_max < 2) return kCoalesceLaunch;
    if (!scan_running) return n_parked > 0 ? kCoalesceParkFlush : kCoalesceLaunch;
    return n_parked + 1 >= t_max ? kCoalesceParkFlush : kCoalescePark;
}

static int coalesce_ticks_max(const Ctx *c, int64_t k, bool sync_tick)
{
    if (c->coalesce_max < 2 || sync_tick || c->nranks != 1 || c->xchg || c->parent || c->group || !c->own_query_stream) return 0;
    if ((double)k * c->D * c->elem <= c->scan_overlap_bytes) return 0;
    int fit = scan_multi_max_ticks(c);
    if (c->coalesce_max >= kPrefilterTicks && scan_prefilter_usable(c)) fit = kPrefilterTicks;
    if (c->coalesce_max >= kHalfqTicks && scan_halfq_usable(c)) fit = kHalfqTicks;
    const int t = fit < c->coalesce_max ? fit : c->coalesce_max;
    return t >= 2 ? t : 0;
}

static int coalesce_submit(Ctx *c, int first, int T)
{
    const Ctx::ParkedTick *parked = c->parked + first;
    const int b = (int)(c->n_enqueued++ % Ctx::kRing);
    const int K = CHIP_DEFAULT_TOPK;
    const bool prefilter = T >= kPrefilterTicks, halfq = T == kHalfqTicks;
    static_assert(kPrefilterTicks > kMultiMaxTicks && kHalfqTicks == kPrefilterTicks + 1, "passes of four and five ticks are the prefilters'");
    PassArgs a{};
    scan_args_db(c, &a);
    a.K = K;
    a.partial = c->partial_dev[b];
    for (int t = 0; t < T; t++) {
        a.k[t] = parked[t].k;
        if (a.k[t] > a.n_rows) a.n_rows = a.k[t];
        for (int i = 0; i < 3; i++) a.q[3 * t + i] = parked[t].q[i];
    }
    const int grid = scan_multi_grid(c);
    double E = 0.0;
    int e = 0;
    if (prefilter) {
        std::lock_guard<std::mutex> lk(c->mu);
        if (halfq) {
            e = halfq_exponent(c->row_norm_max);
            a.q_up = std::ldexp(1.0f, e);
            a.s_up = std::ldexp(1.0, e);
            a.s_down = std::ldexp(1.0, -e);
            E = halfq_error_bound(c->D, c->row_norm_max, e);
        } else {
            E = prefilter_error_bound(c->D, c->row_norm_max);
        }
    }
    if (hipEventQuery(c->ev_merged[b]) != hipSuccess) CHIP_HIP(c, hipStreamWaitEvent(c->s_scan, c->ev_merged[b], 0));
    hipEvent_t e1 = nullptr;
    int rc = c->prof_on ? prof_begin(c, c->s_scan, (double)a.n_rows * c->D * c->elem, &e1) : CHIP_OK;
    if (rc == CHIP_OK)
        rc = halfq ? launch_scan_halfq(c, c->s_scan, a, grid) : prefilter ? launch_scan_prefilter(c, c->s_scan, a, grid) : launch_scan_multi(c, c->s_scan, a, T, grid);
    if (rc != CHIP_OK) return rc;
    if (e1) CHIP_HIP(c, hipEventRecord(e1, c->s_scan));
    CHIP_HIP(c, hipEventRecord(c->ev_scan[b], c->s_scan));
    c->pass_ev = c->ev_scan[b];
    c->pass_shared = true;
    c->pass_no++;
    CHIP_HIP(c, hipStreamWaitEvent(c->s_query, c->ev_scan[b], 0));
    chip_topk_entry *exact = c->partial_dev[b] + (size_t)kPassMaxTicks * grid * 3 * K;
    if (prefilter) {
        RescoreArgs ra{};
        ra.seg_table = a.seg_table; ra.seg_shift = a.seg_shift; ra.seg_mask = a.seg_mask; ra.D = a.D; ra.K = K;
        ra.in = c->partial_dev[b]; ra.n_lists = grid; ra.wpb = 8;
        ra.E = E;
        ra.out = exact;
        for (int t = 0; t < T; t++) {
            const Ctx::ParkedTick &pt = parked[t];
            Slot &s = *pt.slot;
            ra.k[t] = pt.k;
            for (int i = 0; i < 3; i++) { ra.q[3 * t + i] = s.pf_q[i] = pt.q[i]; s.cert_host[i] = 0; }
            ra.cert[t] = s.cert_dev;
            s.prefilter = true; s.pf_k = pt.k; s.pf_p = pt.p;
        }
        rc = launch_rescore(c, c->s_query, ra, T);
        if (rc != CHIP_OK) return rc;
        Ctx::LastPass &lp = c->last_pass;
        lp.family = halfq ? CHIP_SCAN_FAMILY_HALFQ : CHIP_SCAN_FAMILY_PREFILTER;
        lp.ticks = T; lp.grid = grid; lp.wpb = ra.wpb; lp.K = K; lp.e = e; lp.ring = b; lp.E = E;
        for (int t = 0; t < T; t++) { lp.k[t] = parked[t].k; lp.cert[t] = parked[t].slot->cert_host; }
    }
    if (halfq) {
        PassMergeArgs m{};
        m.in = exact;
        m.K = K;
        for (int t = 0; t < T; t++) {
            const MergeArgs mt = merge_args(exact + (size_t)t * 3 * K, 1, K, nullptr, parked[t].slot->rec.dev(), parked[t].l, &parked[t].p);
            m.result[t] = mt.result; m.l[t] = mt.l; m.locality[t] = mt.locality; m.thresh[t] = mt.thresh;
        }
        rc = launch_pass_merge(c, c->s_query, m, T);
        if (rc != CHIP_OK) return rc;
    }
    for (int t = 0; t < T; t++) {
        const Ctx::ParkedTick &pt = parked[t];
        if (halfq) rc = CHIP_OK;
        else if (prefilter) rc = launch_merge(c, c->s_query, merge_args(exact + (size_t)t * 3 * K, 1, K, nullptr, pt.slot->rec.dev(), pt.l, &pt.p), 3);
        else rc = launch_merge(c, c->s_query, merge_args(c->partial_dev[b] + (size_t)t * grid * 3 * K, grid, K, nullptr, pt.slot->rec.dev(), pt.l, &pt.p), 3);
        if (rc != CHIP_OK) return rc;
        CHIP_HIP(c, hipEventRecord(pt.slot->done, c->s_query));
        pt.slot->wait_ev = pt.slot->done;
        pt.slot->state = SlotState::Event;
        pt.slot->pass_no = c->pass_no;
    }
    CHIP_HIP(c, hipEventRecord(c->ev_merged[b], c->s_query));
    c->coalesce_passes++;
    c->coalesce_ticks += T;
    if (prefilter) { c->prefilter_passes++; c->prefilter_ticks += T; }
    return CHIP_OK;
}

int coalesce_flush(Ctx *c)
{
    const int T = c->n_parked;
    if (T == 0) return CHIP_OK;
    c->n_parked = 0;
    const Ctx::ParkedTick &p0 = c->parked[0];
    int rc;
    if (T == kHalfqTicks && !scan_halfq_usable(c)) {
        rc = coalesce_submit(c, 0, kMultiMaxTicks);
        if (rc == CHIP_OK) rc = coalesce_submit(c, kMultiMaxTicks, T - kMultiMaxTicks);
    } else if (T == kPrefilterTicks && !scan_prefilter_usable(c)) {
        const Ctx::ParkedTick &pl = c->parked[T - 1];
        rc = coalesce_submit(c, 0, T - 1);
        if (rc == CHIP_OK) rc = tick_submit(c, pl.k, pl.l, &pl.p, pl.q, false, *pl.slot);
    } else {
        rc = T == 1 ? tick_submit(c, p0.k, p0.l, &p0.p, p0.q, false, *p0.slot) : coalesce_submit(c, 0, T);
    }
    for (int t = 0; t < T && rc != CHIP_OK; t++) {
        c->parked[t].slot->state = SlotState::Failed;
        c->parked[t].slot->err = rc;
    }
    return rc;
}

static int tick_enqueue_slot(Ctx *c, int64_t l, const chip_dot_params *p, bool sync_tick, Slot &s)
{
    int32_t status = 0;
    int64_t k = 0;
    const int64_t n_pub = published_rows(c);
    int rc = tick_begin(s, c->xchg ? INT64_MAX : n_pub, &c->last_l, l, p, &status, &k);
    if (rc != CHIP_OK || status != CHIP_TICK_SCANNED) return rc;
    if (c->xchg) {
        rc = xchg_tick_enqueue(c, l, k, p, sync_tick, s, l > n_pub);
        if (rc != CHIP_OK) return rc;
    } else {
        const int64_t rows[3] = {l - 1, l - 2, l - 3};
        const void *q[3];
        RingGuard rg(c);
        rc = query_row_ptrs(c, rows, 3, l, q);
        if (rc != CHIP_OK) return rc;
        if (resident_eligible(c, k)) {
            (void)coalesce_flush(c);
            rc = resident_tick_enqueue(c, k, l, p, s);
            if (rc == CHIP_OK) { c->last_l = l; return CHIP_OK; }
            if (rc != CHIP_ERR_UNSUPPORTED && rc != kResidentPaused) return rc;
        }
        int t_max = coalesce_ticks_max(c, k, sync_tick);
        if (t_max == kHalfqTicks && !c->pass_shared && !c->coalesce_force) t_max = kPrefilterTicks;
        const int act = t_max < 2 ? kCoalesceLaunch
                                  : coalesce_decide(c->n_parked, t_max, c->coalesce_force || (c->pass_ev && hipEventQuery(c->pass_ev) == hipErrorNotReady));
        if (act == kCoalesceLaunch) {
            (void)coalesce_flush(c);
            rc = tick_submit(c, k, l, p, q, sync_tick, s);
            if (rc != CHIP_OK) return rc;
        } else {
            Ctx::ParkedTick &pt = c->parked[c->n_parked++];
            pt.slot = &s; pt.k = k; pt.l = l; pt.p = *p;
            for (int i = 0; i < 3; i++) pt.q[i] = q[i];
            s.state = SlotState::Parked;
            if (act == kCoalesceParkFlush) (void)coalesce_flush(c);
        }
    }
    c->last_l = l;
    return CHIP_OK;
}

int tick_collect_slot(Ctx *c, Slot &s, chip_tick_result *out)
{
    if (s.state == SlotState::Parked) (void)coalesce_flush(c);
    else if (c->n_parked > 0 && (s.state == SlotState::Event || s.state == SlotState::Poll) && s.pass_no == c->pass_no &&
             hipEventQuery(s.wait_ev) == hipErrorNotReady)
        (void)coalesce_flush(c);
    switch (s.state) {
    case SlotState::Free:
    case SlotState::Parked:
        return CHIP_ERR_BUSY;
    case SlotState::Failed:
        s.state = SlotState::Free;
        if (s.last_l_ptr && *s.last_l_ptr == s.tick_l) *s.last_l_ptr = s.prev_last_l;
        return s.err;
    case SlotState::Immediate:
        break;
    case SlotState::Resident: {
        const int rc = resident_collect(c, s);
        if (rc != CHIP_OK) { s.state = SlotState::Free; return rc; }
        break;
    }
    case SlotState::Poll: {
        bool done = false;
        const volatile unsigned long long *w = s.seq_host;
        for (long spin = 0; spin < (1L << 24) && !done; spin++) {
            done = __atomic_load_n(w, __ATOMIC_ACQUIRE) == s.seq_want;
            if (!done && (spin & 0x3fff) == 0x3fff && hipEventQuery(s.wait_ev) != hipErrorNotReady) break;
        }
        if (done) break;
    }
        [[fallthrough]];
    case SlotState::Event:
        CHIP_HIP(c, hipEventSynchronize(s.wait_ev));
        break;
    }
    if (s.prefilter) {
        s.prefilter = false;
        if (s.cert_host[0] != 1u || s.cert_host[1] != 1u || s.cert_host[2] != 1u) {
            c->prefilter_uncertified++;
            (void)coalesce_flush(c);
            const int rc = tick_submit(c, s.pf_k, s.tick_l, &s.pf_p, s.pf_q, false, s);
            if (rc != CHIP_OK) { s.state = SlotState::Free; return rc; }
            CHIP_HIP(c, hipEventSynchronize(s.wait_ev));
        }
    }
    *out = *s.rec.host();
    s.state = SlotState::Free;
    if (out->status == CHIP_TICK_FAILED) {
        if (s.last_l_ptr && *s.last_l_ptr == s.tick_l) *s.last_l_ptr = s.prev_last_l;
        else if (s.last_l_ptr) {
            for (Slot &o : c->slots)
                if (&o != &s && o.state != SlotState::Free && o.last_l_ptr == s.last_l_ptr && o.prev_last_l == s.tick_l) o.prev_last_l = s.prev_last_l;
        }
        fill_immediate(out, CHIP_TICK_FAILED);
        return CHIP_ERR_SHARD_FAILED;
    }
    return CHIP_OK;
}

int sync_topk_out(Ctx *c, int nq, int K, double *scores, int64_t *idx)
{
    CHIP_HIP(c, hipStreamSynchronize(c->s_query));
    if (c->topk.host()[0].idx == -2) return CHIP_ERR_SHARD_FAILED;
    for (int i = 0; i < nq * K; i++) {
        if (scores) scores[i] = c->topk.host()[i].score;
        if (idx) idx[i] = c->topk.host()[i].idx;
    }
    return CHIP_OK;
}

static int ring_begin_append(Ctx *c, int64_t new_total)
{
    if (!c->ring_dev) return CHIP_OK;
    hipEvent_t ev[2];
    {
        std::lock_guard<std::mutex> rl(c->ring_mu);
        c->rows_pending = new_total;
        ev[0] = c->last_scan_ev[0];
        ev[1] = c->last_scan_ev[1];
    }
    for (hipEvent_t e : ev)
        if (e) CHIP_HIP(c, hipStreamWaitEvent(c->s_append, e, 0));
    return CHIP_OK;
}

int append_reserve(Ctx *c, int64_t first, int64_t n) { return ensure_capacity(c, local_count(c, first + n)); }

static int append_pass(Ctx *c, const AppendSrc &src, int64_t first, int64_t from, int64_t count, int64_t step, bool ring)
{
    const int src_elem = src.elem;
    const size_t row_bytes = (size_t)c->D * src_elem;
    const int64_t chunk_rows = (int64_t)(c->stage_bytes / row_bytes);
    for (int64_t done = 0; done < count; done += chunk_rows) {
        const int64_t m = (count - done) < chunk_rows ? (count - done) : chunk_rows;
        if (src.raw) {
            const int r = project_chunk(c, from + done, m);
            if (r != CHIP_OK) return r;
        } else if (src.fmap) {
            const int r = vlad_chunk(c, src, from + done, m);
            if (r != CHIP_OK) return r;
        } else {
            const char *host = static_cast<const char *>(src.desc) + (size_t)(from + done * step) * row_bytes;
            if (step == 1)
                CHIP_HIP(c, hipMemcpyAsync(c->stage_dev, host, (size_t)m * row_bytes, hipMemcpyHostToDevice, c->s_append));
            else
                CHIP_HIP(c, hipMemcpy2DAsync(c->stage_dev, row_bytes, host, (size_t)step * row_bytes, row_bytes, (size_t)m, hipMemcpyHostToDevice, c->s_append));
        }
        const int r = launch_store_rows(c, c->s_append, c->stage_dev, src_elem, m, first + from + done * step, c->flags_dev, ring, step);
        if (r != CHIP_OK) return r;
    }
    return CHIP_OK;
}

int append_store_db(Ctx *c, const AppendSrc &src, int64_t first, int64_t n, bool owner_only, uint32_t *bad)
{
    *c->flags_host.host() = 0;
    CHIP_HIP(c, hipMemsetAsync(c->flags_dev, 0, sizeof(uint32_t), c->s_append));
    CHIP_HIP(c, hipMemsetAsync(c->norm2_dev, 0, sizeof(unsigned long long), c->s_append));
    int rc;
    if (owner_only && c->nranks > 1) {
        const int64_t G = c->nranks;
        const int64_t i0 = ((c->rank - first) % G + G) % G;
        const int64_t cnt = n > i0 ? (n - i0 + G - 1) / G : 0;
        rc = append_pass(c, src, first, i0, cnt, G, false);
    } else {
        rc = append_pass(c, src, first, 0, n, 1, false);
    }
    if (rc != CHIP_OK) return rc;
    CHIP_HIP(c, hipMemcpyAsync(c->flags_host.host(), c->flags_dev, sizeof(uint32_t), hipMemcpyDeviceToHost, c->s_append));
    CHIP_HIP(c, hipMemcpyAsync(c->norm2_host.host(), c->norm2_dev, sizeof(unsigned long long), hipMemcpyDeviceToHost, c->s_append));
    CHIP_HIP(c, hipStreamSynchronize(c->s_append));
    *bad = *c->flags_host.host();
    return CHIP_OK;
}

// ... 460 lines not shown
    std::lock_guard<std::mutex> qlk(c->query_mu);
    c->last_l = 0;
}

int chip_scan_local(chip_ctx *c, int64_t l, const chip_dot_params *p, int32_t topk, void *dev_out, int32_t *status)
{
    if (!c || !p || !dev_out || !status) return CHIP_ERR_INVALID_ARG;
    if (c->group) return CHIP_ERR_UNSUPPORTED;
    if (topk < 1 || topk > CHIP_MAX_TOPK) return CHIP_ERR_UNSUPPORTED;
    std::lock_guard<std::mutex> qlk(c->query_mu);
    CHIP_HIP(c, hipSetDevice(c->device));
    (void)coalesce_flush(c);
    int64_t k = 0;
    int rc = tick_prepare(published_rows(c), c->last_l, l, p, status, &k);
    if (rc == CHIP_OK && *status == CHIP_TICK_TOO_SHORT) c->last_l = l;
    if (rc != CHIP_OK || *status != CHIP_TICK_SCANNED) return rc;
    const int64_t rows[3] = {l - 1, l - 2, l - 3};
    const void *q[3];
    RingGuard rg(c);
    rc = query_row_ptrs(c, rows, 3, l, q);
    if (rc != CHIP_OK) return rc;
    ScanRequest rq;
    rq.k = k; rq.q = q; rq.nq = 3; rq.K = topk; rq.out = (chip_topk_entry *)dev_out;
    rq.l = l; rq.tick = true;
    rc = enqueue_scan_merge(c, rq);
    if (rc == CHIP_OK) c->last_l = l;
    return rc;
}

int chip_merge_decide(chip_ctx *c, int64_t l, const chip_dot_params *p, const void *dev_gathered, int32_t n_lists,
                      int32_t topk, chip_tick_result *out)
{
    if (!c || !p || !dev_gathered || !out || n_lists < 1) return CHIP_ERR_INVALID_ARG;
    if (c->group) return CHIP_ERR_UNSUPPORTED;
    if (topk < 1 || topk > CHIP_MAX_TOPK) return CHIP_ERR_UNSUPPORTED;
    std::lock_guard<std::mutex> qlk(c->query_mu);
    CHIP_HIP(c, hipSetDevice(c->device));
    (void)coalesce_flush(c);
    Slot &s = c->slots[CHIP_MAX_INFLIGHT - 1];
    int rc = merge_enqueue_slot(c, l, p, dev_gathered, n_lists, topk, s);
    if (rc != CHIP_OK) return rc;
    return tick_collect_slot(c, s, out);
}

int chip_merge_decide_enqueue(chip_ctx *c, int64_t l, const chip_dot_params *p, const void *dev_gathered, int32_t n_lists,
                              int32_t topk, int32_t slot)
{
    if (!c || !p || !dev_gathered || n_lists < 1 || slot < 0 || slot >= CHIP_MAX_INFLIGHT - 1) return CHIP_ERR_INVALID_ARG;
    if (c->group) return CHIP_ERR_UNSUPPORTED;
    if (topk < 1 || topk > CHIP_MAX_TOPK) return CHIP_ERR_UNSUPPORTED;
    std::lock_guard<std::mutex> qlk(c->query_mu);
    CHIP_HIP(c, hipSetDevice(c->device));
    (void)coalesce_flush(c);
    return merge_enqueue_slot(c, l, p, dev_gathered, n_lists, topk, c->slots[slot]);
}

int chip_debug_merge_lists(chip_ctx *c, int32_t form, const chip_topk_entry *lists, int32_t n_lists, int32_t nq, int32_t K, chip_topk_entry *out,
                           int64_t l, const chip_dot_params *p, chip_tick_result *result)
{
    if (!c || !lists || !out || n_lists < 1 || (result && !p)) return CHIP_ERR_INVALID_ARG;
    if (c->group) return CHIP_ERR_UNSUPPORTED;
    if (K < 1 || K > CHIP_MAX_TOPK || n_lists > 512) return CHIP_ERR_UNSUPPORTED;
    const bool form_ok = form == 0 ? nq >= 1 && nq <= CHIP_MAX_NQ
                                   : form == 1 && nq >= 4 && nq % 4 == 0 && nq <= 4096 && !result;
    if (!form_ok) return CHIP_ERR_UNSUPPORTED;
    std::lock_guard<std::mutex> qlk(c->query_mu);
    CHIP_HIP(c, hipSetDevice(c->device));
    (void)coalesce_flush(c);
    return debug_merge_lists(c, form, lists, n_lists, nq, K, out, l, p, result);
}

int chip_get_info(const chip_ctx *c, chip_info *info)
{
    if (!c || !info) return CHIP_ERR_INVALID_ARG;
    std::memset(info, 0, sizeof *info);
    const Ctx *r = c->group ? group_root(const_cast<chip_ctx *>(c)) : c;
    std::lock_guard<std::mutex> lk(r->mu);
    info->abi_version = CHIP_ABI_VERSION;
    info->D = r->D;
    info->device = r->device;
    info->shard_rank = r->rank;
    info->shard_count = r->nranks;
    info->n_cus = r->n_cus;
    info->rows_global = r->rows_global;
    info->rows_local = r->rows_local;
    info->capacity_local = (int64_t)r->segs.size() * r->seg_rows;
    info->lossy_rows = r->lossy_rows;
    std::strncpy(info->arch, r->arch, sizeof(info->arch) - 1);
    info->storage_bytes = r->elem;
    info->n_devices = c->group ? group_size(c) : 1;
    info->exchange = c->group ? c->group_transport : (c->xchg ? CHIP_EXCHANGE_RCCL : CHIP_EXCHANGE_NONE);
    info->comm_ranks = exchange_comm_ranks(c->group ? r : c);
    info->comm_init_abandoned = c->comm_init_abandoned;
    info->scan_forms = scan_forms_built();
    info->test_hooks = chip_build_test_hooks();
    info->row_norm_max = r->row_norm_max;
    return CHIP_OK;
}

int chip_debug_coalesce_stats(chip_ctx *c, int64_t *passes, int64_t *ticks)
{
    if (!c || !passes || !ticks || c->group) return CHIP_ERR_INVALID_ARG;
    std::lock_guard<std::mutex> qlk(c->query_mu);
    *passes = c->coalesce_passes;
    *ticks = c->coalesce_ticks;
    return CHIP_OK;
}

int chip_debug_prefilter_stats(chip_ctx *c, int64_t *passes, int64_t *ticks, int64_t *uncertified)
{
    if (!c || !passes || !ticks || !uncertified || c->group) return CHIP_ERR_INVALID_ARG;
    std::lock_guard<std::mutex> qlk(c->query_mu);
    *passes = c->prefilter_passes;
    *ticks = c->prefilter_ticks;
    *uncertified = c->prefilter_uncertified;
    return CHIP_OK;
}

int chip_debug_last_pass(chip_ctx *c, chip_debug_pass_info *info, chip_topk_entry *cand, chip_topk_entry *exact, uint32_t *cert)
{
    if (!c || c->group) return CHIP_ERR_INVALID_ARG;
    std::lock_guard<std::mutex> qlk(c->query_mu);
    const Ctx::LastPass &lp = c->last_pass;
    if (lp.family == 0) return CHIP_ERR_BUSY;
    CHIP_HIP(c, hipSetDevice(c->device));
    CHIP_HIP(c, hipStreamSynchronize(c->s_scan));
    CHIP_HIP(c, hipStreamSynchronize(c->s_query));
    if (info) {
        std::memset(info, 0, sizeof *info);
        info->family = lp.family; info->ticks = lp.ticks; info->grid = lp.grid; info->wpb = lp.wpb; info->K = lp.K; info->e = lp.e; info->E = lp.E;
        for (int t = 0; t < lp.ticks; t++) info->k[t] = lp.k[t];
    }
    const chip_topk_entry *lists = c->partial_dev[lp.ring];
    const size_t n_cand = (size_t)lp.ticks * lp.grid * 3 * lp.K, n_exact = (size_t)lp.ticks * 3 * lp.K;
    if (cand) CHIP_HIP(c, hipMemcpy(cand, lists, n_cand * sizeof(chip_topk_entry), hipMemcpyDeviceToHost));
    if (exact) CHIP_HIP(c, hipMemcpy(exact, lists + (size_t)kPassMaxTicks * lp.grid * 3 * lp.K, n_exact * sizeof(chip_topk_entry), hipMemcpyDeviceToHost));
    if (cert)
        for (int t = 0; t < lp.ticks; t++)
            for (int i = 0; i < 3; i++) cert[3 * t + i] = lp.cert[t][i];
    return CHIP_OK;
}

int chip_debug_coalesce_force(chip_ctx *c, int32_t on)
{
    if (!c || c->group) return CHIP_ERR_INVALID_ARG;
    std::lock_guard<std::mutex> qlk(c->query_mu);
    c->coalesce_force = on != 0;
    if (!on) { (void)hipSetDevice(c->device); (void)coalesce_flush(c); }
    return CHIP_OK;
}

int chip_debug_coalesce_decide(int32_t n_parked, int32_t t_max, int32_t scan_running) { return coalesce_decide(n_parked, t_max, scan_running != 0); }

int chip_debug_last_scan(chip_ctx *c, chip_debug_scan_launch *out)
{
    if (!c || !out || c->group) return CHIP_ERR_INVALID_ARG;
    std::lock_guard<std::mutex> qlk(c->query_mu);
    (void)hipSetDevice(c->device);
    (void)coalesce_flush(c);
    *out = c->last_scan;
    return CHIP_OK;
}

int chip_debug_scan_plan(int32_t D, int32_t elem, int32_t nq, int32_t K, int64_t n_rows, int32_t call, int32_t n_cus, chip_debug_scan_launch *out)
{
    if (!out || D <= 0 || (elem != 4 && elem != 8) || nq < 1 || nq > CHIP_MAX_NQ || K < 1 || K > CHIP_MAX_TOPK || n_rows < 0 || n_cus < 1 ||
        call < CHIP_SCAN_CALL_QUERY || call > CHIP_SCAN_CALL_TICK_SYNC)
        return CHIP_ERR_INVALID_ARG;
    if (D % 4 != 0 || (size_t)D * 4 * CHIP_MAX_NQ > 160 * 1024 || (elem == 8 && (size_t)D * 8 * 2 > 160 * 1024)) return CHIP_ERR_UNSUPPORTED;
    std::unique_ptr<Ctx> c(new (std::nothrow) Ctx());
    if (!c) return CHIP_ERR_OOM;
    c->D = D;
    c->elem = elem;
    c->n_cus = n_cus;
    scan_read_knobs(c.get());
    const bool tick = call != CHIP_SCAN_CALL_QUERY;
    ScanArgs a{};
    int grid = 0;
    const bool short_scan = scan_policy(c.get(), n_rows, nq, call == CHIP_SCAN_CALL_TICK_SYNC, &a, &grid);
    a.n_rows = n_rows;
    a.D = D;
    a.K = K;
    const bool same_stream = tick_merge_on_scan_stream(c.get(), tick, short_scan, c->scan_streams >= 2, tick);
    chip_tick_result dummy;
    if (scan_tick_fused(c.get(), same_stream, a, tick, nq)) { a.K = 1; a.fused_result = &dummy; }
    return scan_select(c.get(), a, nq, grid, out);
}

int chip_debug_multi_plan(int32_t D, int32_t elem, int32_t n_ticks, int32_t K, int32_t n_cus, chip_debug_scan_launch *out)
{
    if (!out || D <= 0 || (elem != 4 && elem != 8) || n_ticks < 1 || K < 1 || K > CHIP_MAX_TOPK || n_cus < 1) return CHIP_ERR_INVALID_ARG;
    if (D % 4 != 0 || (size_t)D * 4 * CHIP_MAX_NQ > 160 * 1024 || (elem == 8 && (size_t)D * 8 * 2 > 160 * 1024)) return CHIP_ERR_UNSUPPORTED;
    return scan_multi_plan(D, elem, n_ticks, K, n_cus < 512 ? n_cus : 512, out);
}

int chip_debug_prefilter_plan(int32_t D, int32_t elem, int32_t K, int32_t n_cus, chip_debug_scan_launch *out)
{
    if (!out || D <= 0 || (elem != 4 && elem != 8) || K < 1 || K > CHIP_MAX_TOPK || n_cus < 1) return CHIP_ERR_INVALID_ARG;
    if (D % 4 != 0 || (size_t)D * 4 * CHIP_MAX_NQ > 160 * 1024 || (elem == 8 && (size_t)D * 8 * 2 > 160 * 1024)) return CHIP_ERR_UNSUPPORTED;
    return scan_prefilter_plan(D, elem, K, n_cus < 512 ? n_cus : 512, out);
}

int chip_debug_halfq_plan(int32_t D, int32_t elem, int32_t K, int32_t n_cus, chip_debug_scan_launch *out)
{
    if (!out || D <= 0 || (elem != 4 && elem != 8) || K < 1 || K > CHIP_MAX_TOPK || n_cus < 1) return CHIP_ERR_INVALID_ARG;
    if (D % 4 != 0 || (size_t)D * 4 * CHIP_MAX_NQ > 160 * 1024 || (elem == 8 && (size_t)D * 8 * 2 > 160 * 1024)) return CHIP_ERR_UNSUPPORTED;
    return scan_halfq_plan(D, elem, K, n_cus < 512 ? n_cus : 512, out);
}

int chip_debug_halfq_bound(int32_t D, double row_norm_max, int32_t *e, double *E)
{
    if (!e || !E || D <= 0 || !(row_norm_max >= 0.0)) return CHIP_ERR_INVALID_ARG;
    *e = halfq_exponent(row_norm_max);
    *E = halfq_error_bound(D, row_norm_max, *e);
    return CHIP_OK;
}

int chip_debug_scan_stamps(chip_ctx *c, unsigned long long *out, int64_t n_waves)
{
    if (!c || !out || c->group || !c->stamps_dev || n_waves > (int64_t)c->max_grid * 16 + 16) return CHIP_ERR_INVALID_ARG;
    std::lock_guard<std::mutex> qlk(c->query_mu);
    CHIP_HIP(c, hipSetDevice(c->device));
    (void)coalesce_flush(c);
    resident_stop(c);
    CHIP_HIP(c, hipDeviceSynchronize());
    CHIP_HIP(c, hipMemcpy(out, c->stamps_dev, (size_t)n_waves * 4 * sizeof(unsigned long long), hipMemcpyDeviceToHost));
    return CHIP_OK;
}

int chip_profile_enable(chip_ctx *c, int32_t on)
{
    if (!c) return CHIP_ERR_INVALID_ARG;
    if (c->group) return group_profile_enable(c, on);
    std::lock_guard<std::mutex> qlk(c->query_mu);
    (void)hipSetDevice(c->device);
    (void)coalesce_flush(c);
    if (on) resident_stop(c);
    c->prof_on = on != 0;
    return CHIP_OK;
}

int chip_profile_reset(chip_ctx *c)
{
    if (!c) return CHIP_ERR_INVALID_ARG;
    if (c->group) c = static_cast<chip_ctx *>(group_root(c));
    std::lock_guard<std::mutex> qlk(c->query_mu);
    (void)hipSetDevice(c->device);
    (void)coalesce_flush(c);
    c->prof_used = 0;
    return CHIP_OK;
}

int chip_profile_scan(chip_ctx *c, double *total_ms, int64_t *n_launches, double *bytes_per_launch_last, double *span_ms)
{
    if (!c) return CHIP_ERR_INVALID_ARG;
    if (c->group) {
        const int rc = group_synchronize(c);
        if (rc != CHIP_OK) return rc;
        c = static_cast<chip_ctx *>(group_root(c));
    }
    std::lock_guard<std::mutex> qlk(c->query_mu);
    CHIP_HIP(c, hipSetDevice(c->device));
    (void)coalesce_flush(c);
    CHIP_HIP(c, hipStreamSynchronize(c->s_scan));
    if (c->s_scan2) CHIP_HIP(c, hipStreamSynchronize(c->s_scan2));
    CHIP_HIP(c, hipStreamSynchronize(c->s_query));
    double tot = 0.0, span = 0.0;
    for (size_t i = 0; i + 1 < c->prof_used; i += 2) {
        float ms = 0.f;
        CHIP_HIP(c, hipEventElapsedTime(&ms, c->prof_ev[i], c->prof_ev[i + 1]));
        tot += ms;
        CHIP_HIP(c, hipEventElapsedTime(&ms, c->prof_ev[0], c->prof_ev[i + 1]));
        if (ms > span) span = ms;
    }
    if (total_ms) *total_ms = tot;
    if (n_launches) *n_launches = (int64_t)(c->prof_used / 2);
    if (bytes_per_launch_last) *bytes_per_launch_last = c->prof_bytes_last;
    if (span_ms) *span_ms = span;
    return CHIP_OK;
}

}
```

cerebro_amd/csrc/chip_internal.h:

```cpp
#pragma once
#include <hip/hip_runtime.h>
#include <cstdint>
#include <mutex>
#include <utility>
#include <condition_variable>
#include <vector>
#include "../../include/cerebro_hip.h"

namespace chip {

constexpr int kWave = 64;
constexpr int kMaxSegs = 4096;
constexpr int64_t kSegBytesTarget = 512ll << 20;

struct ScanArgs {
    const void *const *seg_table;
    int32_t seg_shift;
    int64_t seg_mask;
    int64_t n_rows;
    int32_t D;
    int32_t K;
    const void *q[CHIP_MAX_NQ];
    int64_t idx_mul, idx_add;
    chip_topk_entry *partial;
    int32_t q64 = 0;
    int32_t rows_form = 0;
    int32_t plain_loads = 0;
    int32_t dyn_claim = 0;
    unsigned long long *stamps = nullptr;
    chip_tick_result *fused_result = nullptr;
    int32_t *fused_ticket = nullptr;
    unsigned long long *fused_seq = nullptr;
    unsigned long long fused_seq_val = 0;
    int64_t tick_l = 0;
    int32_t locality = 0;
    double thresh = 0.0;
};

struct ResidentCmd {
    uint32_t head;
    int32_t locality;
    int64_t n_rows;
    int64_t tick_l;
    double thresh;
    uint64_t result;
    uint64_t seq_ptr;
    uint64_t seq_val;
    uint32_t dyn_claim;
    uint32_t tail;
};
static_assert(sizeof(ResidentCmd) == 64, "one cache line, one PCIe read");
constexpr uint32_t kResidentLeave = 0xffffffffu;

struct ResidentArgs {
    ScanArgs base;
    const uint32_t *cmd_host;
    uint32_t *cmd_dev;
    unsigned long long *exit_host;
    unsigned long long instance;
    unsigned long long lease_ticks;
    uint32_t done;
    uint32_t direct;
};

constexpr int kMultiMaxTicks = 3;
constexpr int kPrefilterTicks = 4;
constexpr int kRescoreCap = 32;
constexpr int kHalfqTicks = 5;
constexpr int kPassMaxTicks = kHalfqTicks;
struct PassArgs {
    const void *const *seg_table;
    int32_t seg_shift;
    int64_t seg_mask;
    int64_t n_rows;
    int32_t D;
    int32_t K;
    int64_t k[kPassMaxTicks];
    const void *q[3 * kPassMaxTicks];
    chip_topk_entry *partial;
    float q_up;
    double s_down, s_up;
};
struct RescoreArgs {
    const void *const *seg_table;
    int32_t seg_shift;
    int64_t seg_mask;
    int32_t D;
    int32_t K;
    const chip_topk_entry *in;
    int32_t n_lists;
    int32_t wpb;
    int64_t k[kPassMaxTicks];
    const void *q[3 * kPassMaxTicks];
    double E;
    chip_topk_entry *out;
    uint32_t *cert[kPassMaxTicks];
};
struct PassMergeArgs {
    const chip_topk_entry *in;
    int32_t K;
    chip_tick_result *result[kPassMaxTicks];
    int64_t l[kPassMaxTicks];
    int32_t locality[kPassMaxTicks];
    double thresh[kPassMaxTicks];
};

struct MergeArgs {
    const chip_topk_entry *in;
    int32_t n_lists;
    int32_t K;
    chip_topk_entry *out;
    chip_tick_result *result;
    int64_t l;
    int32_t locality;
    double thresh;
};

struct BulkFinishArgs {
    const void *const *seg_table;
    int32_t seg_shift;
    int64_t seg_mask;
    int32_t D;
    int32_t KL;
    int32_t K;
    const chip_topk_entry *lists;
    const int64_t *rows;
    double E;
    int32_t locality;
    double thresh;
    chip_tick_result *rec;
    chip_topk_entry *out;
    uint32_t *words;
};

struct Ctx;

template <class T> class DevBuf {
public:
    DevBuf() = default;
    DevBuf(const DevBuf &) = delete;
    DevBuf &operator=(const DevBuf &) = delete;
    ~DevBuf() { release(); }
    int alloc(Ctx *c, size_t n);
    int reserve(Ctx *c, size_t n);
    void release() { if (p_) (void)hipFree(p_); p_ = nullptr; cap_ = 0; }
    void swap(DevBuf &o) { std::swap(p_, o.p_); std::swap(cap_, o.cap_); }
    T *get() const { return p_; }
    operator T *() const { return p_; }
    size_t capacity() const { return cap_; }
private:
    T *p_ = nullptr;
    size_t cap_ = 0;
};
template <class T> class PinnedBuf {
public:
    PinnedBuf() = default;
    PinnedBuf(const PinnedBuf &) = delete;
    PinnedBuf &operator=(const PinnedBuf &) = delete;
    ~PinnedBuf() { release(); }
    int alloc(Ctx *c, size_t n);
    int reserve(Ctx *c, size_t n);
    void release() { if (h_) (void)hipHostFree(h_); h_ = d_ = nullptr; cap_ = 0; }
    T *host() const { return h_; }
    T *dev() const { return d_; }
    size_t capacity() const { return cap_; }
private:
    T *h_ = nullptr, *d_ = nullptr;
    size_t cap_ = 0;
};

struct Projection {
    DevBuf<char> buf;
    DevBuf<float> x;
    size_t mat_bytes = 0;
    int32_t in_dim = 0;
    int32_t matrix_type = 0;
    int32_t D = 0;
    bool has_bias = false;
    int64_t last_passes = 0, last_singles = 0, last_pass_descriptors = 0;
    double *bias() const { return reinterpret_cast<double *>(buf.get() + mat_bytes); }
    double *y() const { return bias() + D; }
};
struct AppendSrc {
    const void *desc;
    int elem;
    const float *raw = nullptr;
    const float *fmap = nullptr;
    int32_t positions = 0;
    int32_t layout = 0;
    int32_t n_maps = 0;
};
int project_stage_input(Ctx *c, const float *x, int64_t n);
int project_chunk(Ctx *c, int64_t from, int64_t m);
void project_count_reset(Ctx *c);

struct Vlad {
    DevBuf<char> w;
    DevBuf<float> raw;
    DevBuf<float> x;
    DevBuf<double> a;
    DevBuf<double> part;
    DevBuf<double> vu;
    DevBuf<float> out;
    int32_t C = 0, K = 0, G = 0;
    int32_t last_n = 0;
    int32_t last_maps = 0;
    int bias_count() const { return (K + G + 1) & ~1; }
    double *bias() const { return reinterpret_cast<double *>(w.get()); }
    float *Wt() const { return reinterpret_cast<float *>(w.get() + (size_t)bias_count() * sizeof(double)); }
    float *centres() const { return Wt() + (size_t)(K + G) * C; }
};
int vlad_chunk(Ctx *c, const AppendSrc &src, int64_t from, int64_t m);

int launch_resident(Ctx *c, hipStream_t s, const ResidentArgs &ra, int grid);
int launch_scan(Ctx *c, hipStream_t s, const ScanArgs &a, int nq, int grid);
int launch_merge(Ctx *c, hipStream_t s, const MergeArgs &a, int nq);
int scan_multi_max_ticks(const Ctx *c);
int scan_multi_plan(int D, int elem, int n_ticks, int K, int grid, chip_debug_scan_launch *f);
int scan_multi_grid(const Ctx *c);
int launch_scan_multi(Ctx *c, hipStream_t s, const PassArgs &a, int n_ticks, int grid);
int scan_prefilter_plan(int D, int elem, int K, int grid, chip_debug_scan_launch *f);
bool scan_prefilter_usable(const Ctx *c);
double prefilter_error_bound(int D, double row_norm_max);
int launch_scan_prefilter(Ctx *c, hipStream_t s, const PassArgs &a, int grid);
int scan_halfq_plan(int D, int elem, int K, int grid, chip_debug_scan_launch *f);
bool scan_halfq_usable(const Ctx *c);
int halfq_exponent(double row_norm_max);
double halfq_error_bound(int D, double row_norm_max, int e);
int launch_scan_halfq(Ctx *c, hipStream_t s, const PassArgs &a, int grid);
int launch_rescore(Ctx *c, hipStream_t s, const RescoreArgs &a, int n_ticks);
int launch_pass_merge(Ctx *c, hipStream_t s, const PassMergeArgs &a, int n_ticks);
int launch_bulk_finish(Ctx *c, hipStream_t s, const BulkFinishArgs &a, int n_ticks);
int scan_grid_for(const Ctx *c, int64_t n_rows, int nq, bool q64);
bool scan_q64(const Ctx *c, int nq, bool long_scan);
int scan_rows_form(const Ctx *c, int64_t n_rows, int nq, int grid, bool q64, bool sync_tick = false);
int scan_select(const Ctx *c, const ScanArgs &a, int nq, int grid, chip_debug_scan_launch *f);
int scan_forms_built();
int launch_scores(Ctx *c, hipStream_t s, const ScanArgs &a, double *out_dev);
int launch_store_rows(Ctx *c, hipStream_t s, const void *src, int src_elem, int64_t n, int64_t first_global, uint32_t *flags_dev, bool write_ring,
                      int64_t row_stride = 1);
int launch_synth(Ctx *c, hipStream_t s, int64_t first_global, int64_t n, uint64_t seed,
                 const int64_t *plant_dst_dev, const int64_t *plant_src_dev, const int32_t *plant_kind_dev, int64_t n_plant, int unit);

enum class SlotState : uint8_t {
    Free,
    Immediate,
    Parked,
    Event,
    Poll,
    Resident,
    Failed,
};

struct Slot {
    hipEvent_t done = nullptr;
    hipEvent_t wait_ev = nullptr;
    PinnedBuf<chip_tick_result> rec;
    SlotState state = SlotState::Free;
    int64_t prev_last_l = 0;
    int64_t tick_l = 0;
    unsigned long long *seq_host = nullptr, *seq_dev = nullptr;
    unsigned long long seq_want = 0;
    uint64_t pass_no = 0;
    int32_t err = 0;
    bool prefilter = false;
    uint32_t *cert_host = nullptr, *cert_dev = nullptr;
    int64_t pf_k = 0;
    chip_dot_params pf_p{};
    const void *pf_q[3] = {};
    int64_t *last_l_ptr = nullptr;
};

struct Resident {
    bool enabled = false;
    double max_bytes = 512.0 * 1024 * 1024;
    int32_t lease_ms = 250;
    hipStream_t stream = nullptr;
    PinnedBuf<char> pinned;
    DevBuf<char> cmd_vram;
    bool cmd_in_vram = false;
    bool direct = false;
    ResidentCmd pending{};
    int64_t test_skip_master = 0;
    bool test_skipped = false;
    ResidentCmd *cmd_host = nullptr;
    uint32_t *cmd_hostdev = nullptr;
    DevBuf<uint32_t> cmd_dev;
    unsigned long long *exit_host = nullptr, *exit_hostdev = nullptr;
    DevBuf<chip_topk_entry> partial;
    DevBuf<int32_t> ticket;
    unsigned long long instance = 0;
    bool alive = false;
    bool ready = false;
    int32_t inhibit = 0;
    bool busy = false;
    uint32_t cmd_no = 0, done = 0;
    int32_t grid = 0;
    Slot *slot = nullptr;
    int64_t ticks = 0, launches = 0;
    std::mutex mu;
};

struct PnpState;
struct IcpState;
struct BatchState;
struct MatchState;
struct FrameStore;
struct OrbState;
struct Exchange;
struct Group;

struct Ctx {
    int32_t D = 0;
    int32_t device = 0;
    int32_t rank = 0, nranks = 1;
    int32_t n_cus = 0;
    char arch[32] = {0};

    int32_t elem = 4;
    bool store_auto = true;

    int32_t seg_shift = 0;
    int64_t seg_rows = 0;
    std::vector<void *> segs;
    DevBuf<void *> seg_table_dev;
    DevBuf<char> ring_dev;
    int64_t rows_global = 0;
    int64_t rows_local = 0;
    int64_t lossy_rows = 0;
    mutable std::mutex mu;
    std::mutex append_mu;
    mutable std::mutex query_mu;
    std::mutex ring_mu;
    int64_t rows_pending = 0;
    hipEvent_t last_scan_ev[2] = {};
    std::mutex pnp_mu;
    std::mutex icp_mu;

    hipStream_t s_query = nullptr, s_append = nullptr, s_pnp = nullptr;
    bool own_query_stream = true;

    DevBuf<char> stage_dev;
    size_t stage_bytes = 0;
    DevBuf<uint32_t> flags_dev;
    PinnedBuf<uint32_t> flags_host;
    DevBuf<unsigned long long> norm2_dev;
    PinnedBuf<unsigned long long> norm2_host;
    double row_norm_max = 0.0;

    static constexpr int kRing = 64;
    hipStream_t s_scan = nullptr;
    hipStream_t s_scan2 = nullptr;
    hipStream_t s_scan_x[2] = {};
    uint64_t n_same_stream = 0;
    DevBuf<chip_topk_entry> partial_dev[kRing];
    int32_t partial_lists[kRing] = {};
    hipEvent_t ev_scan[kRing] = {};
    hipEvent_t ev_merged[kRing] = {};
    DevBuf<int32_t> tickets_dev;
    PinnedBuf<unsigned long long> seq_all;
    unsigned long long tick_seq = 0;
    bool tick_poll = true;
    bool tick_fused = true;
    Resident res;
    uint64_t n_enqueued = 0;
    int32_t max_grid = 0;
    PinnedBuf<chip_topk_entry> topk;

    DevBuf<char> qvec_dev;
    DevBuf<double> scores_dev;
    DevBuf<unsigned long long> stamps_dev;

    std::vector<char> qconv;
    int64_t cap_hint = 0;
    int32_t group_transport = 0;
    mutable int last_comm = 0;
    int32_t comm_init_abandoned = 0;
    Exchange *xchg = nullptr;
    Group *group = nullptr;
    Ctx *parent = nullptr;
    Slot slots[CHIP_MAX_INFLIGHT];
    int64_t last_l = 0;

    struct ParkedTick { Slot *slot; int64_t k, l; chip_dot_params p; const void *q[3]; };
    int32_t coalesce_max = 5;
    bool coalesce_force = false;
    ParkedTick parked[kPassMaxTicks];
    int32_t n_parked = 0;
    hipEvent_t pass_ev = nullptr;
    bool pass_shared = false;
    uint64_t pass_no = 0;
    int64_t coalesce_passes = 0, coalesce_ticks = 0;
    int64_t prefilter_passes = 0, prefilter_ticks = 0, prefilter_uncertified = 0;
    PinnedBuf<uint32_t> cert_all;
    chip_debug_scan_launch last_scan{};
    struct LastPass { int32_t family = 0, ticks = 0, grid = 0, wpb = 0, K = 0, e = 0, ring = 0; double E = 0.0; int64_t k[kPassMaxTicks] = {}; const uint32_t *cert[kPassMaxTicks] = {}; } last_pass;

    int32_t scan_block = 0;
    int32_t scan_blocks_per_cu = 2;
    int32_t scan_reserve = 0;
    int32_t scan_variant = 0;
    int32_t scan_streams = 4;
    bool tick_same_stream = true;
    int32_t scan_claim = -1;
    int32_t scan_rows = 0;
    double scan_plain_bytes = 768.0 * 1024 * 1024;
    double scan_sync_plain_bytes = 4096.0 * 1024 * 1024;
    double scan_half_bytes = 192.0 * 1024 * 1024;
    int32_t scan_short_bpc = 1;
    double scan_overlap_bytes = 8.0 * 1024 * 1024 * 1024;

    bool prof_on = false;
    std::vector<hipEvent_t> prof_ev;
    size_t prof_used = 0;
    double prof_bytes_last = 0.0;

    PnpState *pnp_state = nullptr;
    IcpState *icp_state = nullptr;
    BatchState *batch_state = nullptr;
    MatchState *match_state = nullptr;
    FrameStore *frame_store = nullptr;
    OrbState *orb_state = nullptr;
    Projection proj;
    Vlad vlad;
    std::mutex match_mu;

    mutable hipError_t last_hip = hipSuccess;
};

#define CHIP_HIP(ctx, expr)                                  \
    do {                                                     \
        hipError_t _e = (expr);                              \
        if (_e != hipSuccess) {                              \
            (ctx)->last_hip = _e;                            \
            return _e == hipErrorOutOfMemory ? CHIP_ERR_OOM : CHIP_ERR_HIP; \
        }                                                    \
    } while (0)

inline bool owns_row(const Ctx *c, int64_t g) { return c->nranks == 1 || (g % c->nranks) == c->rank; }
inline int64_t local_of(const Ctx *c, int64_t g) { return c->nranks == 1 ? g : g / c->nranks; }
inline int64_t local_count(const Ctx *c, int64_t k) {
    if (c->nranks == 1) return k;
    return k > c->rank ? (k - c->rank + c->nranks - 1) / c->nranks : 0;
}
inline char *row_ptr_host(const Ctx *c, int64_t local) {
    return static_cast<char *>(c->segs[(size_t)(local >> c->seg_shift)]) + (local & (c->seg_rows - 1)) * (int64_t)c->D * c->elem;
}
inline char *ring_ptr(const Ctx *c, int64_t g) {
    return c->ring_dev + (g % CHIP_RING_ROWS) * (int64_t)c->D * c->elem;
}

struct RingGuard {
    std::unique_lock<std::mutex> lk;
    explicit RingGuard(Ctx *c) : lk(c->ring_mu, std::defer_lock) { if (c->ring_dev) lk.lock(); }
};
int ctx_create(chip_ctx **out, int32_t D, int64_t capacity_hint, int32_t device, int32_t rank, int32_t nranks, uint32_t flags);
void ctx_destroy(chip_ctx *c);
int ctx_append(Ctx *c, const AppendSrc &src, int64_t n, uint32_t flags, int64_t *first_index);
int append_reserve(Ctx *c, int64_t first, int64_t n);
int append_store_db(Ctx *c, const AppendSrc &src, int64_t first, int64_t n, bool owner_only, uint32_t *bad);
bool append_can_switch_to_double(const Ctx *c, int64_t first);
int append_switch_to_double(Ctx *c, int64_t n);
int append_ring_publish(Ctx *c, const AppendSrc &src, int64_t first, int64_t n, bool lossy);
int synth_generate(Ctx *c, int64_t first, int64_t n, uint64_t seed, const int64_t *plant_dst, const int64_t *plant_src, const int32_t *plant_kind, int64_t n_plant, int unit);
void append_publish(Ctx *c, int64_t new_total, bool lossy, int64_t n);
int64_t published_rows(const Ctx *c);
int ctx_append_synthetic(Ctx *c, int64_t n, uint64_t seed, const int64_t *plant_dst, const int64_t *plant_src, const int32_t *plant_kind, int64_t n_plant, int unit);
int ctx_read_row(Ctx *c, int64_t g, int64_t total, void *out);
int query_row_ptrs(Ctx *c, const int64_t *rows, int nq, int64_t n_global, const void **q);
int upload_query_vectors(Ctx *c, const void *queries, int src_elem, int nq, const void **q);
struct ScanRequest {
    int64_t k = 0;
    const void *const *q = nullptr;
    int nq = 0;
    int K = 0;
    chip_topk_entry *out = nullptr;
    chip_tick_result *res = nullptr;
    int64_t l = 0;
    const chip_dot_params *p = nullptr;
    bool tick = false;
    bool sync_tick = false;
    bool merge_on_scan_stream = false;
    unsigned long long *seq_dev = nullptr;
    unsigned long long seq_val = 0;
};
struct ScanReceipt {
    hipStream_t merge_stream = nullptr;
    hipEvent_t done_ev = nullptr;
    bool fused = false;
};
int enqueue_scan_merge(Ctx *c, const ScanRequest &rq, ScanReceipt *rcpt = nullptr);
bool tick_merge_on_scan_stream(const Ctx *c, bool tick, bool short_scan, bool second_tick_stream, bool caller_accepts);
template <class Args> inline void scan_args_db(const Ctx *c, Args *a)
{
    a->seg_table = c->seg_table_dev; a->seg_shift = c->seg_shift; a->seg_mask = c->seg_rows - 1; a->D = c->D;
}
MergeArgs merge_args(const chip_topk_entry *in, int32_t n_lists, int32_t K, chip_topk_entry *out, chip_tick_result *result, int64_t l, const chip_dot_params *p);
int prof_begin(Ctx *c, hipStream_t s, double bytes, hipEvent_t *stop);
int merge_enqueue_slot(Ctx *c, int64_t l, const chip_dot_params *p, const void *dev_gathered, int32_t n_lists, int32_t topk, Slot &s);
int merge_enqueue_out(Ctx *c, const void *dev_gathered, int32_t n_lists, int nq, int32_t topk, chip_topk_entry *out);
int tick_begin(Slot &s, int64_t n_rows, int64_t *last_l, int64_t l, const chip_dot_params *p, int32_t *status, int64_t *k);
int tick_prepare(int64_t n, int64_t last_l, int64_t l, const chip_dot_params *p, int32_t *status, int64_t *k_out);
void fill_immediate(chip_tick_result *r, int32_t status);
int tick_collect_slot(Ctx *c, Slot &s, chip_tick_result *out);
enum { kCoalesceLaunch = 0, kCoalescePark = 1, kCoalesceParkFlush = 2 };
int coalesce_decide(int n_parked, int t_max, bool scan_running);
int coalesce_flush(Ctx *c);
int sync_topk_out(Ctx *c, int nq, int K, double *scores, int64_t *idx);
int ctx_scores_local(Ctx *c, int64_t k, const void *q, double *u_global, int64_t stride_mul, int64_t stride_add);
int env_int(const char *name, int dflt);
void scan_read_knobs(Ctx *c);
bool scan_policy(const Ctx *c, int64_t n_local, int nq, bool sync_tick, ScanArgs *a, int *grid);
bool scan_tick_fused(const Ctx *c, bool same_stream, const ScanArgs &a, bool decision_only, int nq);
void resident_read_knobs(Ctx *c);
bool resident_eligible(Ctx *c, int64_t k);
constexpr int kResidentPaused = 1;
int resident_tick_enqueue(Ctx *c, int64_t k, int64_t l, const chip_dot_params *p, Slot &s);
int resident_collect(Ctx *c, Slot &s);
void resident_wait_command(Ctx *c);
void resident_destroy(Ctx *c);
void resident_stop(Ctx *c);
void resident_pause(Ctx *c);
void resident_resume(Ctx *c);
struct ResidentPause {
    Ctx *c;
    bool on;
    explicit ResidentPause(Ctx *ctx, bool cond = true) : c(ctx), on(cond) { if (on) resident_pause(c); }
    ~ResidentPause() { if (on) resident_resume(c); }
    ResidentPause(const ResidentPause &) = delete;
    ResidentPause &operator=(const ResidentPause &) = delete;
};
template <class T> int DevBuf<T>::alloc(Ctx *c, size_t n)
{
    const hipError_t e = hipMalloc((void **)&p_, n * sizeof(T));
    if (e != hipSuccess) p_ = nullptr;
    CHIP_HIP(c, e);
    cap_ = n;
    return CHIP_OK;
}
template <class T> int DevBuf<T>::reserve(Ctx *c, size_t n)
{
    if (n <= cap_) return CHIP_OK;
    ResidentPause paused(c);
    release();
    return alloc(c, n);
}
template <class T> int PinnedBuf<T>::alloc(Ctx *c, size_t n)
{
    hipError_t e = hipHostMalloc((void **)&h_, n * sizeof(T), hipHostMallocDefault);
    if (e != hipSuccess) h_ = nullptr;
    else if ((e = hipHostGetDevicePointer((void **)&d_, h_, 0)) != hipSuccess) release();
    CHIP_HIP(c, e);
    cap_ = n;
    return CHIP_OK;
}
template <class T> int PinnedBuf<T>::reserve(Ctx *c, size_t n)
{
    if (n <= cap_) return CHIP_OK;
    ResidentPause paused(c);
    release();
    return alloc(c, n);
}
constexpr uint32_t kCreateStoreMask = 3u;

constexpr int kXRing = 64;
constexpr int kListEntries = CHIP_MAX_NQ * CHIP_MAX_TOPK;
void exchange_destroy(Ctx *c);
int exchange_comm_ranks(const Ctx *c);
void group_destroy(Ctx *c);
int xchg_tick_enqueue(Ctx *c, int64_t l, int64_t k, const chip_dot_params *p, bool sync_tick, Slot &s, bool fail_local);
int xchg_query(Ctx *c, int64_t k, const void *const *q, int nq, int K, double *scores, int64_t *idx, bool fail_local);
int xchg_fetch_rows(Ctx *c, const int64_t *rows, int nq, int64_t n_local_published, const void **q, bool *fail_local);
int group_append(Ctx *gc, const void *desc, int src_elem, int64_t n, uint32_t flags, int64_t *first_index);
int group_append_synthetic(Ctx *gc, int64_t n, uint64_t seed, const int64_t *pd, const int64_t *ps, const int32_t *pk, int64_t n_plant, int unit);
int group_read_rows(Ctx *gc, const int64_t *rows, int64_t n, void *out, int out_elem);
int group_tick_enqueue(Ctx *gc, int64_t l, const chip_dot_params *p, int32_t slot);
int group_tick_collect(Ctx *gc, int32_t slot, chip_tick_result *out);
int group_query(Ctx *gc, int64_t k, const int64_t *rows, const void *vectors, int vec_elem, int nq, int K, double *scores, int64_t *idx);
int group_scores(Ctx *gc, int64_t k, int64_t query_row, double *u);
int group_synchronize(Ctx *gc);
int group_profile_enable(Ctx *gc, int on);
Ctx *group_root(Ctx *gc);
int group_size(const Ctx *gc);

int32_t batch_qpad(int32_t Q);
int batch_local_enqueue(Ctx *c, int64_t k, const float *queries, int32_t Q, int32_t topk, chip_topk_entry **out_dev, int32_t *Qpad_out);
int batch_deliver(Ctx *c, const chip_topk_entry *list_dev, int32_t Q, int32_t topk, float *scores, int64_t *idx);
int batch_exchange_buffers(Ctx *c, int n_lists, int32_t Qpad, int32_t topk, chip_topk_entry **gathered, chip_topk_entry **merged, hipEvent_t *ev_done);
int batch_merge_lists(Ctx *c, hipStream_t s, const chip_topk_entry *in, int n_lists, int32_t Qpad, int32_t Q, int32_t topk, chip_topk_entry *out);
int debug_merge_lists(Ctx *c, int form, const chip_topk_entry *lists, int32_t n_lists, int32_t nq, int32_t K, chip_topk_entry *out, int64_t l,
                      const chip_dot_params *p, chip_tick_result *result);
int group_query_batch(Ctx *gc, int64_t k, const float *queries, int32_t Q, int32_t topk, float *scores, int64_t *idx, bool cast_rows);
int xchg_query_batch(Ctx *c, int64_t k, const float *queries, int32_t Q, int32_t topk, float *scores, int64_t *idx, bool fail_local, bool cast_rows);

int pnp_create(Ctx *c);
void pnp_destroy(Ctx *c);
void icp_destroy(Ctx *c);
void batch_destroy(Ctx *c);
void match_destroy(Ctx *c);
void frame_store_destroy(Ctx *c);
void orb_destroy(Ctx *c);
int orb_check(int32_t width, int32_t height, const chip_orb_params *p, chip_orb_params *d);
int orb_enqueue(Ctx *c, hipStream_t s, const uint8_t *image, const uint8_t *image_dev, int32_t width, int32_t height, const chip_orb_params &d,
                bool describe, uint8_t *desc_dev, float2 *kp_dev, size_t back);
int orb_finished(Ctx *c, bool describe, int32_t n_features, int32_t *total, int32_t level_counts[8]);
constexpr int kFramePutGroup = 16;
int orb_batch_enqueue(Ctx *c, hipStream_t s, const uint8_t *pairs_dev, size_t pair_stride, int32_t G, int32_t width, int32_t height,
                      const chip_orb_params &d, uint8_t *desc_base, float2 *kp_base, int32_t slot_kp, const int32_t *slot, int32_t *launches,
                      const uint8_t **out_dev, size_t *out_stride);
int orb_batch_counts(Ctx *c, hipStream_t s, int32_t G, const int32_t **counts);
int orb_batch_reserve(Ctx *c, int32_t G, int32_t width, int32_t height, const chip_orb_params &d, bool probe);
int pnp_ransac_device(Ctx *c, const double *X_dev, const double *uv_dev, int32_t N, const chip_ransac_params *p, double *T_colmajor,
                      float *confidence, uint8_t *inlier_mask, chip_ransac_summary *summary);
int pnp_ransac_device_batch(Ctx *c, int32_t P, const double *const *X_dev, const double *const *uv_dev, const int32_t *N, const chip_ransac_params *p,
                            const uint64_t *seeds, double *T_colmajor, float *confidence, uint8_t *const *inlier_mask, chip_ransac_summary *summary);
int icp_ransac_device(Ctx *c, const double *A_dev, const double *B_dev, int32_t N, const chip_ransac_params *p, double *T_colmajor,
                      float *confidence, uint8_t *inlier_mask, chip_ransac_summary *summary);
int icp_enqueue_device_batch(Ctx *c, int32_t R, const double *const *A_dev, const double *const *B_dev, const int32_t *N, const chip_ransac_params *p,
                             const uint64_t *seeds, int32_t total, const int32_t *at);
int icp_wait_matched(Ctx *c);
int icp_debug_record(Ctx *c, int32_t problem, chip_debug_ransac_shape *shape, int32_t *valid, double *cost, int32_t *nin, double *T_colmajor,
                     unsigned long long *mask);

}

struct chip_ctx : chip::Ctx {};
```

include/cerebro_hip.h:

```cpp
#ifndef CEREBRO_HIP_H
#define CEREBRO_HIP_H
#include <stdint.h>

#ifdef __cplusplus
extern "C" {
#endif

#define CHIP_ABI_VERSION 7

enum {
    CHIP_OK = 0,
    CHIP_ERR_INVALID_ARG = -1,
    CHIP_ERR_NO_DEVICE = -2,
    CHIP_ERR_HIP = -3,
    CHIP_ERR_OOM = -4,
    CHIP_ERR_NOT_F32 = -5,
    CHIP_ERR_NONFINITE = -6,
    CHIP_ERR_RANGE = -7,
    CHIP_ERR_UNSUPPORTED = -8,
    CHIP_ERR_TOO_FEW_POINTS = -9,
    CHIP_ERR_BUSY = -10,
    CHIP_ERR_COMM = -11,
    CHIP_ERR_SHARD_FAILED = -12,
    CHIP_ERR_GROUP_BROKEN = -13
// ... 84 lines not shown
int chip_query_vectors_f32(chip_ctx *ctx, int64_t k, const float *queries, int32_t nq, int32_t topk,
                           double *scores, int64_t *idx);
int chip_query_vectors_f64(chip_ctx *ctx, int64_t k, const double *queries, int32_t nq, int32_t topk,
                           double *scores, int64_t *idx);
int chip_query_scores(chip_ctx *ctx, int64_t k, int64_t query_row, double *u);

int chip_query_batch_f32(chip_ctx *ctx, int64_t k, const float *queries, int32_t Q, int32_t topk,
                         float *scores , int64_t *idx );

int chip_query_batch_cast_f32(chip_ctx *ctx, int64_t k, const float *queries, int32_t Q, int32_t topk,
                              float *scores , int64_t *idx );

#define CHIP_QUERY_PREFIX_GROUP 4096
typedef struct chip_query_prefix_plan_out {
    int32_t group_size;
    int32_t groups;
    int32_t tile_full;
    int32_t tile_last;
    int64_t qtiles;
    int64_t units;
    int64_t units_rect;
} chip_query_prefix_plan_out;
typedef struct chip_query_prefix_last {
    int32_t groups, launches, waits, reserved;
    int64_t units_claimed, units_planned;
} chip_query_prefix_last;
int chip_build_has_query_prefix(void);
int chip_query_batch_rows_f32(chip_ctx *ctx, const int64_t *query_rows, const int64_t *k, int32_t Q, int32_t topk,
                              float *scores , int64_t *idx );
int chip_query_batch_rows_cast_f32(chip_ctx *ctx, const int64_t *query_rows, const int64_t *k, int32_t Q, int32_t topk,
                                   float *scores , int64_t *idx );
int chip_query_batch_prefix_f32(chip_ctx *ctx, const int64_t *k, const float *queries, int32_t Q, int32_t topk,
                                float *scores , int64_t *idx );
int chip_query_batch_prefix_cast_f32(chip_ctx *ctx, const int64_t *k, const float *queries, int32_t Q, int32_t topk,
                                     float *scores , int64_t *idx );
int chip_query_prefix_plan(const int64_t *k, int32_t Q, int32_t elem, int32_t topk, int32_t *order ,
                           chip_query_prefix_plan_out *out);
int chip_debug_query_prefix_last(chip_ctx *ctx, chip_query_prefix_last *out);

typedef struct {
    int32_t locality;
    int32_t lag;
    int32_t min_new;
    int32_t min_k;
    double  thresh;
} chip_dot_params;
void chip_dot_params_default(chip_dot_params *p);

enum { CHIP_TICK_SKIPPED = 0,
       CHIP_TICK_TOO_SHORT = 1,
       CHIP_TICK_SCANNED = 2,
       CHIP_TICK_FAILED = 3 };

typedef struct {
    int32_t status;
    int32_t found;
    int64_t idx_curr;
    int64_t idx_prev;
    double  score;
    int64_t argmax[3];
    double  maxv[3];
} chip_tick_result;

int chip_loop_tick(chip_ctx *ctx, int64_t l, const chip_dot_params *p, chip_tick_result *out);
int chip_resident_pause(chip_ctx *ctx);
int chip_resident_resume(chip_ctx *ctx);
#define CHIP_MAX_INFLIGHT 64
int chip_loop_tick_enqueue(chip_ctx *ctx, int64_t l, const chip_dot_params *p, int32_t slot);
int chip_loop_tick_collect(chip_ctx *ctx, int32_t slot, chip_tick_result *out);
int64_t chip_loop_last_l(const chip_ctx *ctx);
void chip_loop_reset(chip_ctx *ctx);
int chip_build_has_tick_coalesce(void);
int chip_debug_coalesce_stats(chip_ctx *ctx, int64_t *passes, int64_t *ticks);
int chip_debug_coalesce_force(chip_ctx *ctx, int32_t on);
int chip_debug_coalesce_decide(int32_t n_parked, int32_t t_max, int32_t scan_running);

#define CHIP_BULK_TICKS_GROUP 1365
#define CHIP_BULK_TICKS_MAX_TOPK 8
typedef struct chip_bulk_ticks_plan_out {
    int32_t group_ticks;
    int32_t groups;
    int32_t tile_full;
    int32_t tile_last;
    int64_t ticks_scanned, ticks_skipped, ticks_too_short;
    int64_t units, units_rect;
    int64_t last_l;
} chip_bulk_ticks_plan_out;
typedef struct chip_bulk_ticks_last {
    int32_t groups, launches, waits;
    int32_t list_len;
    int64_t certified, uncertified, rescored_rows, exact_reruns;
    double E;
} chip_bulk_ticks_last;
int chip_build_has_bulk_ticks(void);
int chip_loop_ticks_bulk(chip_ctx *ctx, const int64_t *l, int32_t T, const chip_dot_params *p ,
                         int64_t last_l, int32_t topk ,
                         chip_tick_result *out , double *scores ,
                         int64_t *idx , int64_t *last_l_out );
int chip_bulk_ticks_plan(const int64_t *l, int32_t T, const chip_dot_params *p , int64_t last_l, int64_t n_rows,
                         int32_t *status , int64_t *k , chip_bulk_ticks_plan_out *out);
int chip_debug_bulk_ticks_last(chip_ctx *ctx, chip_bulk_ticks_last *out);

#define CHIP_SCAN_FAMILY_NONE    0
#define CHIP_SCAN_FAMILY_ONE_ROW 1
#define CHIP_SCAN_FAMILY_WIDE    2
#define CHIP_SCAN_FAMILY_ROWS    3
#define CHIP_SCAN_FAMILY_MULTI   4
#define CHIP_SCAN_FAMILY_PREFILTER 5
#define CHIP_SCAN_FAMILY_HALFQ   6
#define CHIP_SCAN_CALL_QUERY      0
#define CHIP_SCAN_CALL_TICK       1
#define CHIP_SCAN_CALL_TICK_SYNC  2
typedef struct {
    int32_t family;
    int32_t elem;
    int32_t nq, K;
    int32_t U, NT, FULL;
    int32_t NG;
    int32_t R, NTL;
    int32_t ticks;
    int32_t q64;
    int32_t claimed;
    int32_t fused;
    int32_t grid, block;
    int32_t wg_per_cu;
    int32_t lds_bytes;
    int64_t n_rows;
    int64_t launches;
} chip_debug_scan_launch;
int chip_debug_last_scan(chip_ctx *ctx, chip_debug_scan_launch *out);
int chip_debug_scan_plan(int32_t D, int32_t elem, int32_t nq, int32_t K, int64_t n_rows, int32_t call, int32_t n_cus,
                         chip_debug_scan_launch *out);
int chip_debug_multi_plan(int32_t D, int32_t elem, int32_t n_ticks, int32_t K, int32_t n_cus, chip_debug_scan_launch *out);
int chip_debug_prefilter_plan(int32_t D, int32_t elem, int32_t K, int32_t n_cus, chip_debug_scan_launch *out);
int chip_debug_halfq_plan(int32_t D, int32_t elem, int32_t K, int32_t n_cus, chip_debug_scan_launch *out);
int chip_debug_halfq_bound(int32_t D, double row_norm_max, int32_t *e, double *E);
int chip_debug_prefilter_stats(chip_ctx *ctx, int64_t *passes, int64_t *ticks, int64_t *uncertified);

typedef struct { double score; int64_t idx; } chip_topk_entry;
int chip_scan_local(chip_ctx *ctx, int64_t l, const chip_dot_params *p, int32_t topk, void *dev_out, int32_t *status);
int chip_merge_decide(chip_ctx *ctx, int64_t l, const chip_dot_params *p, const void *dev_gathered, int32_t n_lists,
                      int32_t topk, chip_tick_result *out);
int chip_merge_decide_enqueue(chip_ctx *ctx, int64_t l, const chip_dot_params *p, const void *dev_gathered, int32_t n_lists,
                              int32_t topk, int32_t slot);
int chip_debug_merge_lists(chip_ctx *ctx, int32_t form, const chip_topk_entry *lists, int32_t n_lists, int32_t nq, int32_t K,
                           chip_topk_entry *out, int64_t l, const chip_dot_params *p, chip_tick_result *result);
typedef struct {
    int32_t family, ticks, grid, wpb, K;
    int32_t e;
    int64_t k[5];
    double E;
} chip_debug_pass_info;
int chip_debug_last_pass(chip_ctx *ctx, chip_debug_pass_info *info, chip_topk_entry *cand, chip_topk_entry *exact, uint32_t *cert);

typedef struct {
    double  error_thresh;
    double  min_inlier_ratio;
    int32_t max_iterations;
    int32_t min_iterations;
    int32_t use_mle;
    int32_t sample_size;
    double  failure_probability;
    uint64_t seed;
    int32_t n_hypotheses;
    int32_t sampler;
} chip_ransac_params;
enum { CHIP_SAMPLER_FRESH = 0, CHIP_SAMPLER_THEIA_PERSISTENT = 1 };
void chip_ransac_params_default(chip_ransac_params *p);

typedef struct {
    int32_t n_iterations;
    int32_t n_inliers;
    int32_t best_hypothesis;
    int32_t n_models;
    double  best_cost;
} chip_ransac_summary;

int chip_pnp_ransac(chip_ctx *ctx, const double *X, const double *uv, int32_t N, const chip_ransac_params *p,
                    double T_colmajor[16], float *confidence, uint8_t *inlier_mask ,
                    chip_ransac_summary *summary );

int chip_pnp_ransac_batch(chip_ctx *ctx, int32_t P, const double *const *X, const double *const *uv, const int32_t *N,
                          const chip_ransac_params *p, const uint64_t *seeds, double *T_colmajor ,
                          float *confidence , uint8_t *const *inlier_mask, chip_ransac_summary *summary );

void chip_icp_params_default(chip_ransac_params *p);
int chip_icp_ransac(chip_ctx *ctx, const double *A, const double *B, int32_t N, const chip_ransac_params *p,
                    double T_colmajor[16], float *confidence, uint8_t *inlier_mask ,
                    chip_ransac_summary *summary );
int chip_icp_ransac_enqueue(chip_ctx *ctx, const double *A, const double *B, int32_t N, const chip_ransac_params *p);
int chip_icp_ransac_collect(chip_ctx *ctx, double T_colmajor[16], float *confidence, uint8_t *inlier_mask ,
                            chip_ransac_summary *summary );

#define CHIP_ICP_MAX_BATCH 16
int chip_build_has_icp_batch(void);
int chip_icp_ransac_batch(chip_ctx *ctx, int32_t P, const double *const *A, const double *const *B, const int32_t *N,
                          const chip_ransac_params *p, const uint64_t *seeds, double *T_colmajor ,
                          float *confidence , uint8_t *const *inlier_mask, chip_ransac_summary *summary );

#define CHIP_RANSAC_LEG_PNP 0
#define CHIP_RANSAC_LEG_ICP 1
typedef struct {
    int32_t P;
    int32_t H;
    int32_t N;
    int32_t words;
    int32_t S;
    int32_t sampler;
} chip_debug_ransac_shape;
int chip_debug_ransac_record(chip_ctx *ctx, int32_t leg, int32_t problem, chip_debug_ransac_shape *shape, int32_t *valid, double *cost,
                             int32_t *nin, double *T_colmajor, uint64_t *mask, int32_t *nsol, int32_t *sample);
int chip_debug_pnp_stage(chip_ctx *ctx, int32_t problem, int32_t *ok, double *Tg, double *Sg);
int chip_debug_pnp_keep_stage(chip_ctx *ctx, int32_t on);


#define CHIP_MATCH_MAX_KEYPOINTS 16384
#define CHIP_ORB_DESC_BYTES 32
int chip_build_has_match(void);

int chip_orb_match(chip_ctx *ctx, const uint8_t *d1, int32_t n1, const uint8_t *d2, int32_t n2,
                   int32_t *train_idx , int32_t *distance );
int chip_gms_filter(chip_ctx *ctx, const float *kp1_xy, int32_t n1, int32_t w1, int32_t h1,
                    const float *kp2_xy, int32_t n2, int32_t w2, int32_t h2,
                    const int32_t *query_idx, const int32_t *train_idx, int32_t n_matches,
                    uint8_t *inlier , int32_t *n_inliers);

typedef struct {
    const uint8_t *desc;
    const float   *kp_xy;
    int32_t        n;
    int32_t        width, height;
    const float   *xyz;
} chip_match_frame;
typedef struct {
    int32_t n_matches_all;
    int32_t n_matches_gms;
    int32_t n_3d2d_ab;
    int32_t n_3d2d_ba;
    int32_t n_3d3d;
    int32_t n_out_of_image;
} chip_match_summary;
int chip_match_pair(chip_ctx *ctx, const chip_match_frame *a, const chip_match_frame *b, const double Kinv_rowmajor[9],
                    chip_match_summary *summary);
typedef struct {
    double  *uv, *uv_d;
    double  *X_ab, *uvn_ab;
    double  *X_ba, *uvn_ba;
    double  *A_3d3d, *B_3d3d;
    int32_t *match_query_idx, *match_train_idx;
} chip_match_sets_out;
int chip_match_read_sets(chip_ctx *ctx, chip_match_sets_out *out);
enum { CHIP_SET_AB = 0, CHIP_SET_BA = 1 };
int chip_pnp_ransac_matched(chip_ctx *ctx, int32_t which, const chip_ransac_params *p, double T_colmajor[16], float *confidence,
                            uint8_t *inlier_mask, chip_ransac_summary *summary );
int chip_icp_ransac_matched(chip_ctx *ctx, const chip_ransac_params *p, double T_colmajor[16], float *confidence,
                            uint8_t *inlier_mask, chip_ransac_summary *summary );

#define CHIP_MATCH_MAX_BATCH 16
int chip_build_has_match_batch(void);
int chip_match_batch(chip_ctx *ctx, const chip_match_frame *a, const chip_match_frame *b, int32_t B,
                     const double Kinv_rowmajor[9], chip_match_summary *summary );
int chip_match_select(chip_ctx *ctx, int32_t j);
int chip_match_batch_read_matches(chip_ctx *ctx, int32_t j, int32_t *train_idx, int32_t *distance);
int chip_pnp_ransac_matched_batch(chip_ctx *ctx, int32_t P, const int32_t *cand, const int32_t *which,
                                  const chip_ransac_params *p, const uint64_t *seeds, double *T_colmajor ,
                                  float *confidence , uint8_t *const *inlier_mask ,
                                  chip_ransac_summary *summary , int32_t *status );
int chip_icp_ransac_matched_batch_enqueue(chip_ctx *ctx, int32_t P, const int32_t *cand, const chip_ransac_params *p,
                                          const uint64_t *seeds, int32_t *status );
int chip_icp_ransac_matched_batch_collect(chip_ctx *ctx, double *T_colmajor , float *confidence ,
                                          uint8_t *const *inlier_mask , chip_ransac_summary *summary );
int chip_icp_ransac_matched_batch(chip_ctx *ctx, int32_t P, const int32_t *cand, const chip_ransac_params *p, const uint64_t *seeds,
                                  double *T_colmajor , float *confidence , uint8_t *const *inlier_mask ,
                                  chip_ransac_summary *summary , int32_t *status );

int chip_build_has_frame_store(void);
int chip_frame_store_reserve(chip_ctx *ctx, int32_t n_slots, int32_t slot_keypoints);
int chip_frame_store_info(chip_ctx *ctx, int32_t *n_slots, int32_t *slot_keypoints, int32_t *n_frames );
int chip_frame_put(chip_ctx *ctx, int64_t id, const chip_match_frame *f);
int chip_frame_drop(chip_ctx *ctx, int64_t id);
int chip_frame_read(chip_ctx *ctx, int64_t id, int32_t *n, int32_t *width, int32_t *height,
                    uint8_t *desc , float *kp_xy , float *pts );
int chip_match_batch_stored(chip_ctx *ctx, int64_t a_id, const int64_t *b_ids, int32_t B,
                            const double Kinv_rowmajor[9], chip_match_summary *summary );

enum { CHIP_GMS_WITH_SCALE = 1, CHIP_GMS_WITH_ROTATION = 2 };
typedef struct {
    int32_t scale;
    int32_t rotation;
    int32_t n_inliers;
    int32_t counts[5][8];
} chip_gms_choice;
int chip_build_has_gms_modes(void);
int chip_gms_filter_modes(chip_ctx *ctx, const float *kp1_xy, int32_t n1, int32_t w1, int32_t h1,
                          const float *kp2_xy, int32_t n2, int32_t w2, int32_t h2,
                          const int32_t *query_idx, const int32_t *train_idx, int32_t n_matches, uint32_t modes,
                          uint8_t *inlier , int32_t *n_inliers, chip_gms_choice *choice );
int chip_match_batch_modes(chip_ctx *ctx, const chip_match_frame *a, const chip_match_frame *b, int32_t B,
                           const double Kinv_rowmajor[9], uint32_t modes, chip_match_summary *summary ,
                           chip_gms_choice *choice );
int chip_match_batch_stored_modes(chip_ctx *ctx, int64_t a_id, const int64_t *b_ids, int32_t B, const double Kinv_rowmajor[9],
                                  uint32_t modes, chip_match_summary *summary , chip_gms_choice *choice );

#define CHIP_MATCH_MAX_PAIRS CHIP_MATCH_MAX_BATCH
int chip_build_has_match_pairs(void);
int chip_match_pairs_stored(chip_ctx *ctx, const int64_t *a_ids, const int64_t *b_ids, int32_t P, const double Kinv_rowmajor[9],
// ... 129 lines not shown
```

Measured before the change: 1373.

## Add deep coalesced MFMA scan covering up to ten parked ticks per DB pass

Adds a new 'deep' scan family that batches up to ten parked loop-query ticks (thirty descriptors) into one database pass. It uses an f32 MFMA 32x32 kernel with multi-stage LDS staging and per-wave top-K lists, followed by batched exact rescoring and merge on the query stream. Coalescing depth is also made adaptive to how many consecutive shared passes have run, and flush windows are split into chunks. The aim is to amortise streaming the large database across more queries, at the cost of extra latency from parking ticks and extra device buffers. The deep path only applies to f32 storage, so f64 stores fall back to the old families with the new depth and flush policy.

```diff
diff --git a/cerebro_amd/capi.py b/cerebro_amd/capi.py
--- a/cerebro_amd/capi.py
+++ b/cerebro_amd/capi.py
@@ -54,7 +54,8 @@
 CHIP_RANSAC_LEG_PNP, CHIP_RANSAC_LEG_ICP = 0, 1
 CHIP_SCAN_FAMILY_NONE, CHIP_SCAN_FAMILY_ONE_ROW, CHIP_SCAN_FAMILY_WIDE, CHIP_SCAN_FAMILY_ROWS, CHIP_SCAN_FAMILY_MULTI = 0, 1, 2, 3, 4
 CHIP_SCAN_CALL_QUERY, CHIP_SCAN_CALL_TICK, CHIP_SCAN_CALL_TICK_SYNC = 0, 1, 2
-SCAN_FAMILY_NAMES = {0: "none", 1: "one_row", 2: "wide", 3: "rows", 4: "multi", 5: "prefilter", 6: "halfq"}
+SCAN_FAMILY_NAMES = {0: "none", 1: "one_row", 2: "wide", 3: "rows", 4: "multi", 5: "prefilter", 6: "halfq", 7: "deep"}
+CHIP_SCAN_FAMILY_DEEP, CHIP_DEEP_MAX_TICKS = 7, 10
 
 CHIP_TICK_SKIPPED, CHIP_TICK_TOO_SHORT, CHIP_TICK_SCANNED = 0, 1, 2
 CHIP_MATCH_MAX_KEYPOINTS = 16384
@@ -177,6 +178,10 @@
 
 class PassInfo(C.Structure):
     _fields_ = [(n, C.c_int32) for n in ("family", "ticks", "grid", "wpb", "K", "e")] + [("k", C.c_int64 * 5), ("E", C.c_double)]
+
+
+class DeepInfo(C.Structure):
+    _fields_ = [(n, C.c_int32) for n in ("family", "ticks", "grid", "wpb", "K", "reserved")] + [("k", C.c_int64 * 10), ("E", C.c_double)]
 
 
 class RansacShape(C.Structure):
@@ -266,6 +271,10 @@
     "chip_debug_coalesce_stats": (C.c_int, [_P, C.POINTER(C.c_int64), C.POINTER(C.c_int64)]),
     "chip_debug_coalesce_force": (C.c_int, [_P, C.c_int32]),
     "chip_debug_coalesce_decide": (C.c_int, [C.c_int32, C.c_int32, C.c_int32]),
+    "chip_debug_coalesce_depth": (C.c_int, [C.c_int32, C.c_int32, C.c_int32]),
+    "chip_debug_deep_plan": (C.c_int, [C.c_int32, C.c_int32, C.c_int32, C.c_int32, C.c_int32, C.POINTER(ScanLaunch)]),
+    "chip_debug_last_deep_pass": (C.c_int, [_P, C.POINTER(DeepInfo), _P, _P, _P]),
+    "chip_debug_deep_stats": (C.c_int, [_P, C.POINTER(C.c_int64), C.POINTER(C.c_int64)]),
     "chip_debug_last_scan": (C.c_int, [_P, C.POINTER(ScanLaunch)]),
     "chip_debug_scan_plan": (C.c_int, [C.c_int32, C.c_int32, C.c_int32, C.c_int32, C.c_int64, C.c_int32, C.c_int32, C.POINTER(ScanLaunch)]),
     "chip_debug_multi_plan": (C.c_int, [C.c_int32, C.c_int32, C.c_int32, C.c_int32, C.c_int32, C.POINTER(ScanLaunch)]),
@@ -611,6 +620,20 @@
     return out.as_dict()
 
 
+def deep_plan(D: int, n_ticks: int, elem: int = 4, K: int = CHIP_DEFAULT_TOPK, n_cus: int = 256, check: bool = True):
+    out = ScanLaunch()
+    rc = load_library().chip_debug_deep_plan(D, elem, n_ticks, K, n_cus, C.byref(out))
+    if not check:
+        return rc, out.as_dict()
+    if rc != CHIP_OK:
+        raise ChipError(rc, "chip_debug_deep_plan")
+    return out.as_dict()
+
+
+def coalesce_depth(run: int, n_parked: int, t_max: int) -> int:
+    return int(load_library().chip_debug_coalesce_depth(run, n_parked, t_max))
+
+
 def halfq_bound(D: int, row_norm_max: float) -> tuple[int, float]:
     e, E = C.c_int32(), C.c_double()
     rc = load_library().chip_debug_halfq_bound(D, row_norm_max, C.byref(e), C.byref(E))
@@ -1003,6 +1026,23 @@
                     E=float(info.E), e=int(info.e), cand_s=cand[..., 0].copy(), cand_i=cand[..., 1].copy().view(np.int64),
                     exact_s=exact[..., 0].copy(), exact_i=exact[..., 1].copy().view(np.int64), cert=cert)
 
+    def deep_stats(self) -> tuple[int, int]:
+        passes, ticks = C.c_int64(), C.c_int64()
+        self._chk(self.lib.chip_debug_deep_stats(self.h, C.byref(passes), C.byref(ticks)), "chip_debug_deep_stats")
+        return passes.value, ticks.value
+
+    def last_deep_pass(self) -> dict:
+        info = DeepInfo()
+        self._chk(self.lib.chip_debug_last_deep_pass(self.h, C.byref(info), None, None, None), "chip_debug_last_deep_pass")
+        T, grid, K = info.ticks, info.grid, info.K
+        cand = np.empty((T, grid, 3, K, 2), dtype=np.float64)
+        exact = np.empty((T, 3, K, 2), dtype=np.float64)
+        cert = np.zeros((T, 3), dtype=np.uint32)
+        self._chk(self.lib.chip_debug_last_deep_pass(self.h, C.byref(info), _ptr(cand), _ptr(exact), _ptr(cert)), "chip_debug_last_deep_pass")
+        return dict(family=SCAN_FAMILY_NAMES[info.family], ticks=T, grid=grid, wpb=int(info.wpb), K=K, k=[int(x) for x in info.k[:T]],
+                    E=float(info.E), cand_s=cand[..., 0].copy(), cand_i=cand[..., 1].copy().view(np.int64),
+                    exact_s=exact[..., 0].copy(), exact_i=exact[..., 1].copy().view(np.int64), cert=cert)
+
     def scan_local(self, l: int, dev_out_ptr: int, topk: int = CHIP_DEFAULT_TOPK, params: DotParams | None = None) -> int:
         p = params or default_dot_params()
         status = C.c_int32()
diff --git a/cerebro_amd/csrc/chip_api.hip b/cerebro_amd/csrc/chip_api.hip
--- a/cerebro_amd/csrc/chip_api.hip
+++ b/cerebro_amd/csrc/chip_api.hip
@@ -154,6 +154,10 @@
         if (c->ev_scan[i]) (void)hipEventDestroy(c->ev_scan[i]);
         if (c->ev_merged[i]) (void)hipEventDestroy(c->ev_merged[i]);
     }
+    for (int i = 0; i < kDeepRing; i++) {
+        if (c->deep_ev_scan[i]) (void)hipEventDestroy(c->deep_ev_scan[i]);
+        if (c->deep_ev_merged[i]) (void)hipEventDestroy(c->deep_ev_merged[i]);
+    }
     if (c->s_scan) (void)hipStreamDestroy(c->s_scan);
     if (c->s_scan2) (void)hipStreamDestroy(c->s_scan2);
     for (hipStream_t x : c->s_scan_x)
@@ -234,9 +238,17 @@
     rc = c->tickets_dev.alloc(c, Ctx::kRing);
     if (rc != CHIP_OK) return rc;
     CHIP_HIP(c, hipMemset(c->tickets_dev, 0, Ctx::kRing * sizeof(int32_t)));
-    c->coalesce_max = env_int("CHIP_TICK_COALESCE", kPassMaxTicks);
+    c->coalesce_max = env_int("CHIP_TICK_COALESCE", kCoalesceDefault);
     if (c->coalesce_max < 2) c->coalesce_max = 0;
-    if (c->coalesce_max > kPassMaxTicks) c->coalesce_max = kPassMaxTicks;
+    if (c->coalesce_max > kDeepMaxTicks) c->coalesce_max = kDeepMaxTicks;
+    if (c->coalesce_max > kPassMaxTicks) {
+        for (int i = 0; i < kDeepRing; i++) {
+            rc = c->deep_dev[i].alloc(c, ((size_t)c->max_grid + 1) * 3 * kDeepMaxTicks * CHIP_DEFAULT_TOPK);
+            if (rc != CHIP_OK) return rc;
+            CHIP_HIP(c, hipEventCreateWithFlags(&c->deep_ev_scan[i], hipEventDisableTiming));
+            CHIP_HIP(c, hipEventCreateWithFlags(&c->deep_ev_merged[i], hipEventDisableTiming));
+        }
+    }
     c->tick_poll = env_int("CHIP_TICK_POLL", 1) != 0;
     resident_read_knobs(c);
     rc = c->seq_all.alloc(c, CHIP_MAX_INFLIGHT);
@@ -395,7 +407,7 @@
     if (rcpt) { rcpt->merge_stream = s_merge; rcpt->fused = fused; rcpt->done_ev = same_stream ? c->ev_merged[b] : nullptr; }
     if (!same_stream) {
         CHIP_HIP(c, hipEventRecord(c->ev_scan[b], s_scan));
-        if (rq.tick && !short_scan) { c->pass_ev = c->ev_scan[b]; c->pass_shared = false; c->pass_no++; }
+        if (rq.tick && !short_scan) { c->pass_ev = c->ev_scan[b]; c->pass_shared = false; c->run_shared = 0; c->pass_no++; }
         if (c->ring_dev) c->last_scan_ev[s_scan == c->s_scan2 ? 1 : 0] = c->ev_scan[b];
         CHIP_HIP(c, hipStreamWaitEvent(c->s_query, c->ev_scan[b], 0));
     }
@@ -523,14 +535,28 @@
     return n_parked + 1 >= t_max ? kCoalesceParkFlush : kCoalescePark;
 }
 
-static int coalesce_ticks_max(const Ctx *c, int64_t k, bool sync_tick)
-{
+int coalesce_depth(int run, int n_parked, int t_max)
+{
+    int cap = t_max;
+    if (t_max >= kHalfqTicks) {
+        if (run <= 0) cap = kPrefilterTicks;
+        else if (run <= 2) cap = kHalfqTicks;
+    }
+    if (cap < n_parked + 1) cap = n_parked + 1 < t_max ? n_parked + 1 : t_max;
+    return cap;
+}
+
+static int coalesce_ticks_max(const Ctx *c, int64_t k, bool sync_tick, int *shallow)
+{
+    *shallow = 0;
     if (c->coalesce_max < 2 || sync_tick || c->nranks != 1 || c->xchg || c->parent || c->group || !c->own_query_stream) return 0;
     if ((double)k * c->D * c->elem <= c->scan_overlap_bytes) return 0;
     int fit = scan_multi_max_ticks(c);
     if (c->coalesce_max >= kPrefilterTicks && scan_prefilter_usable(c)) fit = kPrefilterTicks;
     if (c->coalesce_max >= kHalfqTicks && scan_halfq_usable(c)) fit = kHalfqTicks;
-    const int t = fit < c->coalesce_max ? fit : c->coalesce_max;
+    int t = fit < c->coalesce_max ? fit : c->coalesce_max;
+    *shallow = t >= 2 ? t : 0;
+    if (c->coalesce_max > kPassMaxTicks && c->deep_dev[0] && scan_deep_usable(c)) t = c->coalesce_max;
     return t >= 2 ? t : 0;
 }
 
@@ -575,6 +601,7 @@
     CHIP_HIP(c, hipEventRecord(c->ev_scan[b], c->s_scan));
     c->pass_ev = c->ev_scan[b];
     c->pass_shared = true;
+    c->run_shared++;
     c->pass_no++;
     CHIP_HIP(c, hipStreamWaitEvent(c->s_query, c->ev_scan[b], 0));
     chip_topk_entry *exact = c->partial_dev[b] + (size_t)kPassMaxTicks * grid * 3 * K;
@@ -628,22 +655,106 @@
     return CHIP_OK;
 }
 
+static int coalesce_submit_deep(Ctx *c, int T)
+{
+    const Ctx::ParkedTick *parked = c->parked;
+    const int d = (int)(c->n_deep++ % kDeepRing);
+    const int K = CHIP_DEFAULT_TOPK;
+    if (T <= kPassMaxTicks || T > kDeepMaxTicks || !c->deep_dev[d]) return CHIP_ERR_UNSUPPORTED;
+    DeepArgs a{};
+    scan_args_db(c, &a);
+    a.K = K;
+    a.n_ticks = T;
+    a.partial = c->deep_dev[d];
+    for (int t = 0; t < T; t++) {
+        a.k[t] = parked[t].k;
+        if (a.k[t] > a.n_rows) a.n_rows = a.k[t];
+        for (int i = 0; i < 3; i++) a.q[3 * t + i] = parked[t].q[i];
+    }
+    const int grid = scan_multi_grid(c);
+    double E;
+    { std::lock_guard<std::mutex> lk(c->mu); E = prefilter_error_bound(c->D, c->row_norm_max); }
+    if (hipEventQuery(c->deep_ev_merged[d]) != hipSuccess) CHIP_HIP(c, hipStreamWaitEvent(c->s_scan, c->deep_ev_merged[d], 0));
+    hipEvent_t e1 = nullptr;
+    int rc = c->prof_on ? prof_begin(c, c->s_scan, (double)a.n_rows * c->D * c->elem, &e1) : CHIP_OK;
+    if (rc == CHIP_OK) rc = launch_scan_deep(c, c->s_scan, a, grid);
+    if (rc != CHIP_OK) return rc;
+    if (e1) CHIP_HIP(c, hipEventRecord(e1, c->s_scan));
+    CHIP_HIP(c, hipEventRecord(c->deep_ev_scan[d], c->s_scan));
+    c->pass_ev = c->deep_ev_scan[d];
+    c->pass_shared = true;
+    c->run_shared++;
+    c->pass_no++;
+    CHIP_HIP(c, hipStreamWaitEvent(c->s_query, c->deep_ev_scan[d], 0));
+    chip_topk_entry *exact = c->deep_dev[d] + (size_t)kDeepMaxTicks * grid * 3 * K;
+    for (int t0 = 0; t0 < T; t0 += kPassMaxTicks) {
+        const int n = T - t0 < kPassMaxTicks ? T - t0 : kPassMaxTicks;
+        RescoreArgs ra{};
+        ra.seg_table = a.seg_table; ra.seg_shift = a.seg_shift; ra.seg_mask = a.seg_mask; ra.D = a.D; ra.K = K;
+        ra.in = c->deep_dev[d] + (size_t)t0 * grid * 3 * K; ra.n_lists = grid; ra.wpb = 32;
+        ra.E = E;
+        ra.out = exact + (size_t)t0 * 3 * K;
+        PassMergeArgs m{};
+        m.in = ra.out;
+        m.K = K;
+        for (int t = 0; t < n; t++) {
+            const Ctx::ParkedTick &pt = parked[t0 + t];
+            Slot &s = *pt.slot;
+            ra.k[t] = pt.k;
+            for (int i = 0; i < 3; i++) { ra.q[3 * t + i] = s.pf_q[i] = pt.q[i]; s.cert_host[i] = 0; }
+            ra.cert[t] = s.cert_dev;
+            s.prefilter = true; s.pf_k = pt.k; s.pf_p = pt.p;
+            const MergeArgs mt = merge_args(m.in + (size_t)t * 3 * K, 1, K, nullptr, s.rec.dev(), pt.l, &pt.p);
+            m.result[t] = mt.result; m.l[t] = mt.l; m.locality[t] = mt.locality; m.thresh[t] = mt.thresh;
+        }
+        rc = launch_rescore(c, c->s_query, ra, n);
+        if (rc == CHIP_OK) rc = launch_pass_merge(c, c->s_query, m, n);
+        if (rc != CHIP_OK) return rc;
+        for (int t = 0; t < n; t++) {
+            Slot &s = *parked[t0 + t].slot;
+            CHIP_HIP(c, hipEventRecord(s.done, c->s_query));
+            s.wait_ev = s.done;
+            s.state = SlotState::Event;
+            s.pass_no = c->pass_no;
+        }
+    }
+    CHIP_HIP(c, hipEventRecord(c->deep_ev_merged[d], c->s_query));
+    Ctx::LastDeep &lp = c->last_deep;
+    lp.ticks = T; lp.grid = grid; lp.wpb = 32; lp.K = K; lp.ring = d; lp.E = E;
+    for (int t = 0; t < T; t++) { lp.k[t] = parked[t].k; lp.cert[t] = parked[t].slot->cert_host; }
+    c->coalesce_passes++;
+    c->coalesce_ticks += T;
+    c->prefilter_passes++; c->prefilter_ticks += T;
+    c->deep_passes++; c->deep_ticks += T;
+    return CHIP_OK;
+}
+
+static int coalesce_flush_window(Ctx *c, int first, int T)
+{
+    if ((T == kHalfqTicks && scan_halfq_usable(c)) || (T == kPrefilterTicks && scan_prefilter_usable(c))) return coalesce_submit(c, first, T);
+    const int m = scan_multi_max_ticks(c);
+    int rc = CHIP_OK;
+    for (int at = first; at < first + T && rc == CHIP_OK;) {
+        const int n = first + T - at < m ? first + T - at : m;
+        const Ctx::ParkedTick &p = c->parked[at];
+        if (n >= 2) rc = coalesce_submit(c, at, n);
+        else rc = tick_submit(c, p.k, p.l, &p.p, p.q, false, *p.slot);
+        at += n >= 2 ? n : 1;
+    }
+    return rc;
+}
+
 int coalesce_flush(Ctx *c)
 {
     const int T = c->n_parked;
     if (T == 0) return CHIP_OK;
     c->n_parked = 0;
-    const Ctx::ParkedTick &p0 = c->parked[0];
-    int rc;
-    if (T == kHalfqTicks && !scan_halfq_usable(c)) {
-        rc = coalesce_submit(c, 0, kMultiMaxTicks);
-        if (rc == CHIP_OK) rc = coalesce_submit(c, kMultiMaxTicks, T - kMultiMaxTicks);
-    } else if (T == kPrefilterTicks && !scan_prefilter_usable(c)) {
-        const Ctx::ParkedTick &pl = c->parked[T - 1];
-        rc = coalesce_submit(c, 0, T - 1);
-        if (rc == CHIP_OK) rc = tick_submit(c, pl.k, pl.l, &pl.p, pl.q, false, *pl.slot);
+    int rc = CHIP_OK;
+    if (T > kPassMaxTicks && scan_deep_usable(c)) {
+        rc = coalesce_submit_deep(c, T);
     } else {
-        rc = T == 1 ? tick_submit(c, p0.k, p0.l, &p0.p, p0.q, false, *p0.slot) : coalesce_submit(c, 0, T);
+        for (int first = 0; first < T && rc == CHIP_OK; first += kPassMaxTicks)
+            rc = coalesce_flush_window(c, first, T - first < kPassMaxTicks ? T - first : kPassMaxTicks);
     }
     for (int t = 0; t < T && rc != CHIP_OK; t++) {
         c->parked[t].slot->state = SlotState::Failed;
@@ -674,8 +785,9 @@
             if (rc == CHIP_OK) { c->last_l = l; return CHIP_OK; }
             if (rc != CHIP_ERR_UNSUPPORTED && rc != kResidentPaused) return rc;
         }
-        int t_max = coalesce_ticks_max(c, k, sync_tick);
-        if (t_max == kHalfqTicks && !c->pass_shared && !c->coalesce_force) t_max = kPrefilterTicks;
+        int shallow = 0;
+        int t_max = coalesce_ticks_max(c, k, sync_tick, &shallow);
+        if (!c->coalesce_force && (t_max <= kPassMaxTicks || shallow == kHalfqTicks)) t_max = coalesce_depth(c->run_shared, c->n_parked, t_max);
         const int act = t_max < 2 ? kCoalesceLaunch
                                   : coalesce_decide(c->n_parked, t_max, c->coalesce_force || (c->pass_ev && hipEventQuery(c->pass_ev) == hipErrorNotReady));
         if (act == kCoalesceLaunch) {
@@ -1442,6 +1554,48 @@
 
 int chip_debug_coalesce_decide(int32_t n_parked, int32_t t_max, int32_t scan_running) { return coalesce_decide(n_parked, t_max, scan_running != 0); }
 
+int chip_debug_coalesce_depth(int32_t run, int32_t n_parked, int32_t t_max) { return coalesce_depth(run, n_parked, t_max); }
+
+int chip_debug_deep_plan(int32_t D, int32_t elem, int32_t n_ticks, int32_t K, int32_t n_cus, chip_debug_scan_launch *out)
+{
+    if (!out || D <= 0 || (elem != 4 && elem != 8) || n_ticks < 1 || K < 1 || K > CHIP_MAX_TOPK || n_cus < 1) return CHIP_ERR_INVALID_ARG;
+    if (D % 4 != 0 || (size_t)D * 4 * CHIP_MAX_NQ > 160 * 1024 || (elem == 8 && (size_t)D * 8 * 2 > 160 * 1024)) return CHIP_ERR_UNSUPPORTED;
+    return scan_deep_plan(D, elem, n_ticks, K, n_cus < 512 ? n_cus : 512, out);
+}
+
+int chip_debug_deep_stats(chip_ctx *c, int64_t *passes, int64_t *ticks)
+{
+    if (!c || !passes || !ticks || c->group) return CHIP_ERR_INVALID_ARG;
+    std::lock_guard<std::mutex> qlk(c->query_mu);
+    *passes = c->deep_passes;
+    *ticks = c->deep_ticks;
+    return CHIP_OK;
+}
+
+int chip_debug_last_deep_pass(chip_ctx *c, chip_debug_deep_info *info, chip_topk_entry *cand, chip_topk_entry *exact, uint32_t *cert)
+{
+    if (!c || c->group) return CHIP_ERR_INVALID_ARG;
+    std::lock_guard<std::mutex> qlk(c->query_mu);
+    const Ctx::LastDeep &lp = c->last_deep;
+    if (lp.ticks == 0) return CHIP_ERR_BUSY;
+    CHIP_HIP(c, hipSetDevice(c->device));
+    CHIP_HIP(c, hipStreamSynchronize(c->s_scan));
+    CHIP_HIP(c, hipStreamSynchronize(c->s_query));
+    if (info) {
+        std::memset(info, 0, sizeof *info);
+        info->family = CHIP_SCAN_FAMILY_DEEP; info->ticks = lp.ticks; info->grid = lp.grid; info->wpb = lp.wpb; info->K = lp.K; info->E = lp.E;
+        for (int t = 0; t < lp.ticks; t++) info->k[t] = lp.k[t];
+    }
+    const chip_topk_entry *lists = c->deep_dev[lp.ring];
+    const size_t n_cand = (size_t)lp.ticks * lp.grid * 3 * lp.K, n_exact = (size_t)lp.ticks * 3 * lp.K;
+    if (cand) CHIP_HIP(c, hipMemcpy(cand, lists, n_cand * sizeof(chip_topk_entry), hipMemcpyDeviceToHost));
+    if (exact) CHIP_HIP(c, hipMemcpy(exact, lists + (size_t)kDeepMaxTicks * lp.grid * 3 * lp.K, n_exact * sizeof(chip_topk_entry), hipMemcpyDeviceToHost));
+    if (cert)
+        for (int t = 0; t < lp.ticks; t++)
+            for (int i = 0; i < 3; i++) cert[3 * t + i] = lp.cert[t][i];
+    return CHIP_OK;
+}
+
 int chip_debug_last_scan(chip_ctx *c, chip_debug_scan_launch *out)
 {
     if (!c || !out || c->group) return CHIP_ERR_INVALID_ARG;
diff --git a/cerebro_amd/csrc/chip_internal.h b/cerebro_amd/csrc/chip_internal.h
--- a/cerebro_amd/csrc/chip_internal.h
+++ b/cerebro_amd/csrc/chip_internal.h
@@ -105,6 +105,22 @@
     double thresh[kPassMaxTicks];
 };
 
+constexpr int kDeepMaxTicks = 10;
+constexpr int kCoalesceDefault = kPassMaxTicks;
+constexpr int kDeepRing = 8;
+struct DeepArgs {
+    const void *const *seg_table;
+    int32_t seg_shift;
+    int64_t seg_mask;
+    int64_t n_rows;
+    int32_t D;
+    int32_t K;
+    int32_t n_ticks;
+    int64_t k[kDeepMaxTicks];
+    const void *q[3 * kDeepMaxTicks];
+    chip_topk_entry *partial;
+};
+
 struct MergeArgs {
     const chip_topk_entry *in;
     int32_t n_lists;
@@ -228,6 +244,9 @@
 int halfq_exponent(double row_norm_max);
 double halfq_error_bound(int D, double row_norm_max, int e);
 int launch_scan_halfq(Ctx *c, hipStream_t s, const PassArgs &a, int grid);
+int scan_deep_plan(int D, int elem, int n_ticks, int K, int grid, chip_debug_scan_launch *f);
+bool scan_deep_usable(const Ctx *c);
+int launch_scan_deep(Ctx *c, hipStream_t s, const DeepArgs &a, int grid);
 int launch_rescore(Ctx *c, hipStream_t s, const RescoreArgs &a, int n_ticks);
 int launch_pass_merge(Ctx *c, hipStream_t s, const PassMergeArgs &a, int n_ticks);
 int launch_bulk_finish(Ctx *c, hipStream_t s, const BulkFinishArgs &a, int n_ticks);
@@ -385,16 +404,22 @@
     struct ParkedTick { Slot *slot; int64_t k, l; chip_dot_params p; const void *q[3]; };
     int32_t coalesce_max = 5;
     bool coalesce_force = false;
-    ParkedTick parked[kPassMaxTicks];
+    ParkedTick parked[kDeepMaxTicks];
     int32_t n_parked = 0;
     hipEvent_t pass_ev = nullptr;
     bool pass_shared = false;
+    int32_t run_shared = 0;
     uint64_t pass_no = 0;
     int64_t coalesce_passes = 0, coalesce_ticks = 0;
     int64_t prefilter_passes = 0, prefilter_ticks = 0, prefilter_uncertified = 0;
+    int64_t deep_passes = 0, deep_ticks = 0;
+    DevBuf<chip_topk_entry> deep_dev[kDeepRing];
+    hipEvent_t deep_ev_scan[kDeepRing] = {}, deep_ev_merged[kDeepRing] = {};
+    uint64_t n_deep = 0;
     PinnedBuf<uint32_t> cert_all;
     chip_debug_scan_launch last_scan{};
     struct LastPass { int32_t family = 0, ticks = 0, grid = 0, wpb = 0, K = 0, e = 0, ring = 0; double E = 0.0; int64_t k[kPassMaxTicks] = {}; const uint32_t *cert[kPassMaxTicks] = {}; } last_pass;
+    struct LastDeep { int32_t ticks = 0, grid = 0, wpb = 0, K = 0, ring = 0; double E = 0.0; int64_t k[kDeepMaxTicks] = {}; const uint32_t *cert[kDeepMaxTicks] = {}; } last_deep;
 
     int32_t scan_block = 0;
     int32_t scan_blocks_per_cu = 2;
@@ -505,6 +530,7 @@
 int tick_collect_slot(Ctx *c, Slot &s, chip_tick_result *out);
 enum { kCoalesceLaunch = 0, kCoalescePark = 1, kCoalesceParkFlush = 2 };
 int coalesce_decide(int n_parked, int t_max, bool scan_running);
+int coalesce_depth(int run, int n_parked, int t_max);
 int coalesce_flush(Ctx *c);
 int sync_topk_out(Ctx *c, int nq, int K, double *scores, int64_t *idx);
 int ctx_scores_local(Ctx *c, int64_t k, const void *q, double *u_global, int64_t stride_mul, int64_t stride_add);
diff --git a/cerebro_amd/csrc/db_scan_deep.hip b/cerebro_amd/csrc/db_scan_deep.hip
--- /dev/null
+++ b/cerebro_amd/csrc/db_scan_deep.hip
@@ -0,0 +1,286 @@
+#include "chip_internal.h"
+#include <cmath>
+
+namespace chip {
+
+typedef float f32x16 __attribute__((ext_vector_type(16)));
+
+constexpr int kDeepBlock = 512;
+constexpr int kDeepStages = 4;
+constexpr int kDeepKC = 32;
+constexpr int kDeepBBlock = 8 * 32 + 4;
+constexpr int kDeepQOff = 32 * kDeepBBlock;
+constexpr int kStageFloats = 36 * kDeepBBlock;
+constexpr int kDeepKL = 8;
+constexpr int kDeepLoads = 5;
+constexpr size_t kDeepLds = (size_t)kDeepStages * kStageFloats * sizeof(float);
+static_assert(kDeepLds <= 160 * 1024, "four stages fit the LDS");
+static_assert((size_t)8 * 2 * 32 * kDeepKL * 8 <= kDeepLds, "the fold's lists alias the stages");
+
+__device__ __forceinline__ constexpr int deep_row_off(int row) { return (row >> 3) * kDeepBBlock + ((row >> 3) & 3) + (row & 7) * 32; }
+__device__ __forceinline__ bool dkey_gt(float s, int32_t i, float s2, int32_t i2) { return s > s2 || (s == s2 && i > i2); }
+
+struct DeepList {
+    float s[kDeepKL];
+    int32_t r[kDeepKL];
+};
+__device__ __forceinline__ void deep_push(DeepList &L, int K, float s, int32_t row)
+{
+#pragma unroll
+    for (int j = kDeepKL - 1; j >= 1; j--) {
+        if (j < K) {
+            const bool above = dkey_gt(s, row, L.s[j - 1], L.r[j - 1]);
+            const bool here = dkey_gt(s, row, L.s[j], L.r[j]) && !above;
+            if (above) { L.s[j] = L.s[j - 1]; L.r[j] = L.r[j - 1]; }
+            else if (here) { L.s[j] = s; L.r[j] = row; }
+        }
+    }
+    if (dkey_gt(s, row, L.s[0], L.r[0])) { L.s[0] = s; L.r[0] = row; }
+}
+__device__ __forceinline__ void deep_kth(const DeepList &L, int K, float &ts, int32_t &tr)
+{
+    ts = L.s[0]; tr = L.r[0];
+#pragma unroll
+    for (int j = 1; j < kDeepKL; j++)
+        if (j < K) { ts = L.s[j]; tr = L.r[j]; }
+}
+
+__device__ __forceinline__ void deep_glds16(const float *gsrc, uint32_t lds_byte_addr_wave_uniform)
+{
+    unsigned keep;
+    asm volatile("s_mov_b32 %0, m0\n\ts_mov_b32 m0, %2\n\ts_nop 0\n\tglobal_load_lds_dwordx4 %1, off\n\ts_mov_b32 m0, %0"
+                 : "=&s"(keep)
+                 : "v"(gsrc), "s"(lds_byte_addr_wave_uniform)
+                 : "memory");
+}
+__device__ __forceinline__ void deep_glds16_s(const void *base_wave_uniform, uint32_t byte_off, uint32_t lds_byte_addr_wave_uniform)
+{
+    unsigned keep;
+    asm volatile("s_mov_b32 %0, m0\n\ts_mov_b32 m0, %3\n\ts_nop 0\n\tglobal_load_lds_dwordx4 %1, %2\n\ts_mov_b32 m0, %0"
+                 : "=&s"(keep)
+                 : "v"(byte_off), "s"(base_wave_uniform), "s"(lds_byte_addr_wave_uniform)
+                 : "memory");
+}
+__device__ __forceinline__ void deep_wait_barrier(int chunks)
+{
+    if (chunks >= 3) asm volatile("s_waitcnt vmcnt(15) lgkmcnt(0)\n\ts_barrier" ::: "memory");
+    else if (chunks == 2) asm volatile("s_waitcnt vmcnt(10) lgkmcnt(0)\n\ts_barrier" ::: "memory");
+    else if (chunks == 1) asm volatile("s_waitcnt vmcnt(5) lgkmcnt(0)\n\ts_barrier" ::: "memory");
+    else asm volatile("s_waitcnt vmcnt(0) lgkmcnt(0)\n\ts_barrier" ::: "memory");
+    static_assert(kDeepLoads == 5, "the counts above");
+}
+
+__global__ __launch_bounds__(kDeepBlock) void db_scan_deep(DeepArgs a)
+{
+    extern __shared__ __attribute__((aligned(16))) char smem[];
+    float *const S0 = reinterpret_cast<float *>(smem);
+    const int tid = threadIdx.x, lane = tid & 63;
+    const int wave = __builtin_amdgcn_readfirstlane(tid >> 6);
+    const int D = a.D, K = a.K, nq = 3 * a.n_ticks;
+    const int n_chunks = D / kDeepKC;
+    const int G = gridDim.x, b = blockIdx.x;
+    const int64_t n_rows = a.n_rows;
+    const int64_t S = (n_rows + 31) >> 5;
+    const int64_t nb = S > b ? (S - b + G - 1) / G : 0;
+    const int64_t nt = (nb + 7) >> 3;
+    const int64_t total = nt * n_chunks;
+    const uint32_t lds_base = __builtin_amdgcn_readfirstlane((uint32_t)(uintptr_t)(const __attribute__((address_space(3))) void *)S0);
+
+    const int col = lane & 31;
+    int32_t klim = 0;
+#pragma unroll
+    for (int t = 0; t < kDeepMaxTicks; t++)
+        if (col < nq && col / 3 == t) klim = (int32_t)a.k[t];
+    const int qrow = 4 * wave + ((lane >> 3) & 3);
+    const float *qsrc = static_cast<const float *>(a.q[0]);
+#pragma unroll
+    for (int j = 1; j < 3 * kDeepMaxTicks; j++)
+        if (j < nq && j == qrow) qsrc = static_cast<const float *>(a.q[j]);
+    qsrc += ((lane & 7) ^ (qrow & 7)) * 4;
+    const uint32_t q_dst = (uint32_t)(kDeepQOff + deep_row_off(4 * wave)) * 4u;
+    const int l_rr = lane >> 3, l_k4 = ((lane & 7) ^ (lane >> 3)) * 4;
+    const int fr = lane & 31, fk = lane >> 5, sw = fr & 7;
+    const int a_off = deep_row_off(wave * 32 + fr) + fk, b_off = kDeepQOff + deep_row_off(fr) + fk;
+
+    int64_t ltile = 0;
+    int lc = 0;
+    const char *rbase = nullptr;
+    uint32_t boff[4];
+    auto load_tile = [&]() {
+        const int64_t j = ltile * 8 + wave;
+        const int64_t r0 = j < nb ? ((int64_t)b + j * G) << 5 : 0;
+        const uint64_t ea = (uint64_t)(a.seg_table + (r0 >> a.seg_shift));
+        const uint32_t ea_hi = (uint32_t)__builtin_amdgcn_readfirstlane((int)(uint32_t)(ea >> 32)), ea_lo = (uint32_t)__builtin_amdgcn_readfirstlane((int)(uint32_t)ea);
+        uint64_t sp;
+        asm volatile("s_load_dwordx2 %0, %1, 0x0\n\ts_waitcnt lgkmcnt(0)" : "=s"(sp) : "s"(((uint64_t)ea_hi << 32) | ea_lo) : "memory");
+        rbase = (const char *)(sp + (uint64_t)((r0 & a.seg_mask) * (int64_t)D) * 4u);
+#pragma unroll
+        for (int u = 0; u < 4; u++) {
+            const int rr = 8 * u + l_rr;
+            boff[u] = (uint32_t)((r0 + rr < n_rows ? rr : 0) * D + l_k4) * 4u;
+        }
+    };
+    auto issue = [&](int stage) {
+        const uint32_t st = lds_base + (uint32_t)stage * (uint32_t)(kStageFloats * 4);
+        const char *src = rbase + (int64_t)lc * (kDeepKC * 4);
+#pragma unroll
+        for (int u = 0; u < 4; u++) deep_glds16_s(src, boff[u], st + (uint32_t)deep_row_off((4 * wave + u) * 8) * 4u);
+        if (lane < 32) deep_glds16(qsrc + lc * kDeepKC, st + q_dst);
+        if (++lc == n_chunks) { lc = 0; ltile++; load_tile(); }
+    };
+    float fa[2][16], fb[2][16];
+    auto read_frags = [&](int stage, float *da, float *db) {
+        const float *St = S0 + stage * kStageFloats;
+#pragma unroll
+        for (int k4 = 0; k4 < 8; k4++) {
+            const int p = (k4 ^ sw) << 2;
+            da[2 * k4] = St[a_off + p]; da[2 * k4 + 1] = St[a_off + p + 2];
+            db[2 * k4] = St[b_off + p]; db[2 * k4 + 1] = St[b_off + p + 2];
+        }
+    };
+
+    DeepList L;
+#pragma unroll
+    for (int j = 0; j < kDeepKL; j++) { L.s[j] = -INFINITY; L.r[j] = -1; }
+    float ts = -INFINITY;
+    int32_t tr = -1;
+
+    if (total > 0) {
+        load_tile();
+        const int first = total < 4 ? (int)total : 4;
+        for (int p = 0; p < first; p++) issue(p);
+        deep_wait_barrier(first - 1);
+        read_frags(0, fa[0], fb[0]);
+    }
+    f32x16 acc;
+#pragma unroll
+    for (int e = 0; e < 16; e++) acc[e] = 0.0f;
+    int64_t ctile = 0;
+    int cc = 0;
+    for (int64_t g = 0; g < total; g += 2) {
+#pragma unroll
+        for (int h = 0; h < 2; h++) {
+            const int64_t gg = g + h;
+            if (gg >= total) break;
+            const float *ca = fa[h], *cb = fb[h];
+#pragma unroll
+            for (int i = 0; i < 8; i++) acc = __builtin_amdgcn_mfma_f32_32x32x2f32(ca[i], cb[i], acc, 0, 0, 0);
+            if (gg + 1 < total) {
+                const int64_t ahead = total - 2 - gg;
+                deep_wait_barrier(ahead < 2 ? (int)ahead : 2);
+                if (gg + 4 < total) issue((int)(gg & 3));
+                read_frags((int)((gg + 1) & 3), fa[h ^ 1], fb[h ^ 1]);
+            }
+#pragma unroll
+            for (int i = 8; i < 16; i++) acc = __builtin_amdgcn_mfma_f32_32x32x2f32(ca[i], cb[i], acc, 0, 0, 0);
+            if (++cc == n_chunks) {
+                const int64_t j = ctile * 8 + wave;
+                if (j < nb) {
+                    const int32_t r0 = (int32_t)(((int64_t)b + j * G) << 5) + 4 * fk;
+                    if (r0 < klim) {
+#pragma unroll
+                        for (int e = 0; e < 16; e++) {
+                            const int32_t r = r0 + (e & 3) + 8 * (e >> 2);
+                            const float s = acc[e];
+                            if (r < klim && dkey_gt(s, r, ts, tr)) {
+                                deep_push(L, K, s, r);
+                                deep_kth(L, K, ts, tr);
+                            }
+                        }
+                    }
+                }
+#pragma unroll
+                for (int e = 0; e < 16; e++) acc[e] = 0.0f;
+                cc = 0;
+                ctile++;
+            }
+        }
+    }
+    asm volatile("s_waitcnt vmcnt(0) lgkmcnt(0)\n\ts_barrier" ::: "memory");
+    float *const Ls = S0;
+    int32_t *const Lr = reinterpret_cast<int32_t *>(S0 + 8 * 2 * 32 * kDeepKL);
+    {
+        const int at = ((wave * 2 + fk) * 32 + col) * kDeepKL;
+#pragma unroll
+        for (int j = 0; j < kDeepKL; j++) { Ls[at + j] = L.s[j]; Lr[at + j] = L.r[j]; }
+    }
+    __syncthreads();
+    if (tid < nq) {
+        DeepList M;
+#pragma unroll
+        for (int j = 0; j < kDeepKL; j++) { M.s[j] = -INFINITY; M.r[j] = -1; }
+        float ms = -INFINITY;
+        int32_t mr = -1;
+        for (int l = 0; l < 16; l++)
+            for (int j = 0; j < kDeepKL; j++) {
+                const float s = Ls[(l * 32 + tid) * kDeepKL + j];
+                const int32_t r = Lr[(l * 32 + tid) * kDeepKL + j];
+                if (r >= 0 && dkey_gt(s, r, ms, mr)) {
+                    deep_push(M, K, s, r);
+                    deep_kth(M, K, ms, mr);
+                }
+            }
+        chip_topk_entry *dst = a.partial + (((int64_t)(tid / 3) * G + b) * 3 + tid % 3) * K;
+#pragma unroll
+        for (int j = 0; j < kDeepKL; j++)
+            if (j < K) {
+                chip_topk_entry e;
+                e.score = (double)M.s[j];
+                e.idx = M.r[j] >= 0 ? (int64_t)M.r[j] : -1;
+                dst[j] = e;
+            }
+    }
+}
+
+int scan_deep_plan(int D, int elem, int n_ticks, int K, int grid, chip_debug_scan_launch *f)
+{
+    *f = chip_debug_scan_launch{};
+    if (D < kDeepKC || D % kDeepKC != 0 || D > 32768 || elem != 4 || n_ticks <= kPassMaxTicks || n_ticks > kDeepMaxTicks || K < 1 || K > kDeepKL || grid < 1 ||
+        grid > 512)
+        return CHIP_ERR_UNSUPPORTED;
+    f->family = CHIP_SCAN_FAMILY_DEEP;
+    f->elem = elem;
+    f->nq = 3 * n_ticks;
+    f->K = K;
+    f->U = 1;
+    f->FULL = 1;
+    f->R = 32;
+    f->NTL = 0;
+    f->ticks = n_ticks;
+    f->NG = 3 * n_ticks;
+    f->grid = grid;
+    f->block = kDeepBlock;
+    f->wg_per_cu = 1;
+    f->lds_bytes = (int32_t)kDeepLds;
+    return CHIP_OK;
+}
+
+bool scan_deep_usable(const Ctx *c)
+{
+    if (c->elem != 4 || c->nranks != 1 || c->scan_variant != 0 || c->scan_rows > 0 || c->seg_rows < 32) return false;
+    chip_debug_scan_launch f;
+    if (scan_deep_plan(c->D, c->elem, kDeepMaxTicks, CHIP_DEFAULT_TOPK, scan_multi_grid(c), &f) != CHIP_OK) return false;
+    double n;
+    { std::lock_guard<std::mutex> lk(c->mu); n = c->row_norm_max; }
+    return n * n <= std::ldexp(1.0, 120) && 2.0 * c->D * std::ldexp(1.0, -24) < 0.5;
+}
+
+int launch_scan_deep(Ctx *c, hipStream_t s, const DeepArgs &a, int grid)
+{
+    chip_debug_scan_launch f;
+    if (grid > c->max_grid || scan_deep_plan(c->D, c->elem, a.n_ticks, a.K, grid, &f) != CHIP_OK || a.D != c->D) return CHIP_ERR_UNSUPPORTED;
+    if (((a.seg_mask + 1) & 31) != 0 || a.n_rows < 1 || a.n_rows > INT32_MAX - 64) return CHIP_ERR_UNSUPPORTED;
+    for (int t = 0; t < a.n_ticks; t++)
+        if (a.k[t] < 0 || a.k[t] > a.n_rows) return CHIP_ERR_INVALID_ARG;
+    for (int j = 0; j < 3 * a.n_ticks; j++)
+        if (!a.q[j]) return CHIP_ERR_INVALID_ARG;
+    CHIP_HIP(c, hipFuncSetAttribute(reinterpret_cast<const void *>(db_scan_deep), hipFuncAttributeMaxDynamicSharedMemorySize, f.lds_bytes));
+    hipLaunchKernelGGL(db_scan_deep, dim3(f.grid), dim3(kDeepBlock), f.lds_bytes, s, a);
+    CHIP_HIP(c, hipGetLastError());
+    f.n_rows = a.n_rows;
+    f.launches = c->last_scan.launches + 1;
+    c->last_scan = f;
+    return CHIP_OK;
+}
+
+}
diff --git a/include/cerebro_hip.h b/include/cerebro_hip.h
--- a/include/cerebro_hip.h
+++ b/include/cerebro_hip.h
@@ -260,6 +260,18 @@
     double E;
 } chip_debug_pass_info;
 int chip_debug_last_pass(chip_ctx *ctx, chip_debug_pass_info *info, chip_topk_entry *cand, chip_topk_entry *exact, uint32_t *cert);
+#define CHIP_SCAN_FAMILY_DEEP    7
+#define CHIP_DEEP_MAX_TICKS 10
+typedef struct {
+    int32_t family, ticks, grid, wpb, K;
+    int32_t reserved;
+    int64_t k[CHIP_DEEP_MAX_TICKS];
+    double E;
+} chip_debug_deep_info;
+int chip_debug_deep_plan(int32_t D, int32_t elem, int32_t n_ticks, int32_t K, int32_t n_cus, chip_debug_scan_launch *out);
+int chip_debug_coalesce_depth(int32_t run, int32_t n_parked, int32_t t_max);
+int chip_debug_last_deep_pass(chip_ctx *ctx, chip_debug_deep_info *info, chip_topk_entry *cand, chip_topk_entry *exact, uint32_t *cert);
+int chip_debug_deep_stats(chip_ctx *ctx, int64_t *passes, int64_t *ticks);
 
 typedef struct {
     double  error_thresh;
```

After: 1217. 11.4% lower.
